# pelinski/TransformerGrooveInfilling

Hardware: AMD Instinct MI355X
Metric: HVO sequences/sec (32-step, d_model=128) per train step (higher is better)
Workload: dtype f32; 1 GPU; BASELINE configs[1]: InfillingClosedHH_training.yaml + overrides d_model=128/4 heads/3 layers, dim_feedforward=512, bs=64 per GPU, dropout=0.24, SGD lr=0.07, hit_loss_penalty=0.38, S=16, encoder-only; global_batch=64, parallelism=dp1, hipgraph=False

## Files before the change

transformergrooveinfilling_amd/csrc/groove_hip.hip:

```cpp
#include <stdarg.h>
#include <stdio.h>
#include <stdlib.h>
#include <string.h>

#include <string>
#include <vector>

#include "gt_attn.h"
#include "gt_common.h"
#include "gt_gemm.h"
#include "gt_misc.h"
#include "gt_seq_api.h"

static thread_local char g_err[512] = "";
static int gt_fail(const char* fmt, ...) {
  va_list ap;
  va_start(ap, fmt);
  vsnprintf(g_err, sizeof(g_err), fmt, ap);
  va_end(ap);
  return -1;
}
extern "C" const char* gt_last_error(void) { return g_err; }

GtProfile g_prof;
#ifndef GT_EMU
struct ProfRec { const char* label; double flops, bytes; hipEvent_t a, b; };
static std::vector<ProfRec> g_recs;
void gt_prof_events(hipEvent_t* start, hipEvent_t* stop) {
  ProfRec r{g_prof.label, g_prof.flops, g_prof.bytes, nullptr, nullptr};
  (void)hipEventCreate(&r.a);
  (void)hipEventCreate(&r.b);
  g_recs.push_back(r);
  *start = r.a; *stop = r.b;
  g_prof.label = "other"; g_prof.flops = 0; g_prof.bytes = 0;
}
#else
void gt_prof_events(hipEvent_t*, hipEvent_t*) {}
#endif
extern "C" int gt_profile_enable(int on) {
  g_prof.on = on != 0;
  g_prof.label = "other";
  return 0;
}
extern "C" int gt_profile_report(char* buf, size_t buf_len, int max_rows) {
  int n = 0;
#ifndef GT_EMU
  struct Acc { std::string label; long count; double ms, flops, bytes; };
  std::vector<Acc> acc;
  for (auto& r : g_recs) {
    (void)hipEventSynchronize(r.b);
    float ms = 0.f;
    (void)hipEventElapsedTime(&ms, r.a, r.b);
    (void)hipEventDestroy(r.a);
    (void)hipEventDestroy(r.b);
    size_t i = 0;
    for (; i < acc.size(); ++i) if (acc[i].label == r.label) break;
    if (i == acc.size()) acc.push_back(Acc{r.label, 0, 0, 0, 0});
    acc[i].count++; acc[i].ms += ms; acc[i].flops += r.flops; acc[i].bytes += r.bytes;
  }
  g_recs.clear();
  std::string out;
  for (auto& a : acc) {
    if (n >= max_rows) break;
    char line[256];
    snprintf(line, sizeof(line), "%s %ld %.6f %.6e %.6e\n", a.label.c_str(), a.count, a.ms, a.flops, a.bytes);
    out += line;
    ++n;
  }
  if (buf && buf_len) { strncpy(buf, out.c_str(), buf_len - 1); buf[buf_len - 1] = 0; }
#else
  if (buf && buf_len) buf[0] = 0;
#endif
  return n;
}
extern "C" int gt_version(void) { return 1; }

static int check_cfg(const gt_config* c) {
  if (!c) return gt_fail("gt_config is NULL");
  if (c->batch <= 0) return gt_fail("batch must be > 0 (got %d)", c->batch);
  if (c->d_model <= 0 || c->d_model > GT_MAX_D) return gt_fail("d_model %d outside 1..%d", c->d_model, GT_MAX_D);
  if (c->n_heads <= 0 || c->d_model % c->n_heads != 0)
    return gt_fail("embed_dim %d not divisible by num_heads %d", c->d_model, c->n_heads);
  if (c->d_model % 2 != 0) return gt_fail("d_model %d must be even (sin/cos positional encoding)", c->d_model);
  if (c->dim_ff <= 0 || c->src_dim <= 0) return gt_fail("dim_ff / src_dim must be > 0");
  if (c->n_enc_layers <= 0 || c->n_enc_layers > 64 || c->n_dec_layers < 0 || c->n_dec_layers > 64)
    return gt_fail("layer counts out of range (enc %d, dec %d)", c->n_enc_layers, c->n_dec_layers);
  if (!(c->dropout >= 0.f && c->dropout < 1.f)) return gt_fail("dropout %f outside [0,1)", (double)c->dropout);
  if (c->flags & ~(GT_CFG_NO_QUAD | GT_CFG_NO_LN_XCHG)) return gt_fail("gt_config.flags %d has unknown bits", c->flags);
  if (c->precision < 0 || c->precision > 2) return gt_fail("precision %d unknown (0 = fp32, 1 = bf16 GEMM operands, 2 = ... and bf16 storage of the Linear outputs)", c->precision);
  if ((int64_t)c->batch * 32 * (c->dim_ff > 3 * c->d_model ? c->dim_ff : 3 * c->d_model) >= (1ll << 31))
    return gt_fail("batch %d too large for 32-bit element indices", c->batch);
  const int n_ln = 2 * c->n_enc_layers + 3 * c->n_dec_layers + (c->n_dec_layers > 0 ? 2 : 1);
  if (n_ln > GT_LN_JOBS_MAX)
    return gt_fail("%d LayerNorm instances (enc %d, dec %d layers) exceed the %d the backward's partials table holds",
                   n_ln, c->n_enc_layers, c->n_dec_layers, GT_LN_JOBS_MAX);
  return 0;
}

struct AttnP { int64_t in_w, in_b, out_w, out_b; };
struct LayerP { AttnP sa, xa; int64_t w1, b1, w2, b2, n1w, n1b, n2w, n2b, n3w, n3b; };
struct PEntry { int64_t off, size; int rows, cols; };
struct PLayout {
  int64_t in_w, in_b, encn_w, encn_b, din_w, din_b, decn_w, decn_b, out_w, out_b, total;
  std::vector<LayerP> enc, dec;
  std::vector<PEntry> entries;
};
static PLayout param_layout(const gt_config& c) {
  PLayout L;
  int64_t cur = 0;
  auto add = [&](int rows, int cols) {
    const int64_t size = (int64_t)rows * (cols ? cols : 1);
    const int64_t off = cur;
    L.entries.push_back(PEntry{off, size, rows, cols});
    cur += (size + 63) / 64 * 64;
    return off;
  };
  const int d = c.d_model, F = c.dim_ff;
  auto attn = [&](AttnP& a) { a.in_w = add(3 * d, d); a.in_b = add(3 * d, 0); a.out_w = add(d, d); a.out_b = add(d, 0); };
  L.in_w = add(d, c.src_dim); L.in_b = add(d, 0);
  L.enc.resize(c.n_enc_layers);
  for (auto& l : L.enc) {
    attn(l.sa);
    l.w1 = add(F, d); l.b1 = add(F, 0); l.w2 = add(d, F); l.b2 = add(d, 0);
    l.n1w = add(d, 0); l.n1b = add(d, 0); l.n2w = add(d, 0); l.n2b = add(d, 0);
  }
  L.encn_w = add(d, 0); L.encn_b = add(d, 0);
  L.dec.resize(c.n_dec_layers);
  if (c.n_dec_layers > 0) {
    L.din_w = add(d, GT_TGT); L.din_b = add(d, 0);
    for (auto& l : L.dec) {
      attn(l.sa); attn(l.xa);
      l.w1 = add(F, d); l.b1 = add(F, 0); l.w2 = add(d, F); l.b2 = add(d, 0);
      l.n1w = add(d, 0); l.n1b = add(d, 0); l.n2w = add(d, 0); l.n2b = add(d, 0); l.n3w = add(d, 0); l.n3b = add(d, 0);
    }
    L.decn_w = add(d, 0); L.decn_b = add(d, 0);
  }
  L.out_w = add(GT_TGT, d); L.out_b = add(GT_TGT, 0);
  L.total = cur;
  return L;
}

extern "C" int gt_param_count(const gt_config* cfg, int64_t* n_tensors, int64_t* n_floats) {
  if (check_cfg(cfg)) return -1;
  PLayout L = param_layout(*cfg);
  if (n_tensors) *n_tensors = (int64_t)L.entries.size();
  if (n_floats) *n_floats = L.total;
  return 0;
}
extern "C" int gt_param_layout(const gt_config* cfg, int64_t* offsets, int64_t* sizes, int32_t* rows, int32_t* cols) {
  if (check_cfg(cfg)) return -1;
  PLayout L = param_layout(*cfg);
  for (size_t i = 0; i < L.entries.size(); ++i) {
    if (offsets) offsets[i] = L.entries[i].off;
    if (sizes) sizes[i] = L.entries[i].size;
    if (rows) rows[i] = L.entries[i].rows;
    if (cols) cols[i] = L.entries[i].cols;
  }
  return 0;
}

struct LayerW {
  int64_t qkv, P, ctx, xhat1, rstd1, x1;
  int64_t qx, kvx, Px, ctxx, xhatx, rstdx, x2;
  int64_t hact, xhat2, rstd2, xout;
};
struct WLayout {
  int64_t x0, a0, enc_xhat, enc_rstd, memory, y0, b0, dec_xhat, dec_rstd, dec_final;
  std::vector<LayerW> layers;
  int64_t hvo_tmp, dlogits, loss_part, dctx, dmem, da0_dec, ln_part, ln_part_stride, total, stamps = 0;
  int64_t pack_f = -1, pack_b = -1, pack_stride = 0;
  int64_t seq_dctx = -1;
  int64_t seq_xchg = -1, seq_xchg_n = 0;
  int64_t rowx = -1, rowx_n = 0;
  int64_t seq_amask = -1, seq_amask_stride = 0;
  std::vector<std::pair<int64_t, int64_t>> sh;
  std::vector<int64_t> sh_only;
  int64_t w16 = -1, w16t = -1, w16_stride = 0;
  int64_t kbits = -1, kbits_stride = 0;
  int64_t wT = -1, wT_stride = 0;
  struct TmpSet { int64_t dzA, dzAm, dzB, dzBm, dzC, dzCm, dhid, dqkv, dqkvx; };
  std::vector<TmpSet> set;
};
#ifndef GT_WGRAD_DEFER_MAX_M
#define GT_WGRAD_DEFER_MAX_M (1ll << 40)
#endif
static bool wgrad_deferred(const gt_config& c) { return (int64_t)c.batch * 32 <= GT_WGRAD_DEFER_MAX_M; }
static bool seq_supported(const gt_config& c);
#ifndef GT_T128_BIG_MIN
#define GT_T128_BIG_MIN 192
#endif
static int g_bf16_shadows = -1;
static int g_layout_epoch = 0;
extern "C" int gt_layout_epoch() { return g_layout_epoch; }
extern "C" int gt_set_operand_shadows(int level) {
  const int nv = level < 0 ? -1 : level > 2 ? 2 : level;
  if (nv != g_bf16_shadows) ++g_layout_epoch;
  g_bf16_shadows = nv;
  return 0;
}
static int bf16_shadow_level() {
  if (g_bf16_shadows < 0) { const char* e = getenv("GT_BF16_SHADOWS"); g_bf16_shadows = (e && e[0] >= '0' && e[0] <= '2') ? e[0] - '0' : 2; }
  return g_bf16_shadows;
}
static bool bf16_shadows(const gt_config& c);
static bool bf16_wt(const gt_config& c) {
  static const int on = [] { const char* e = getenv("GT_BF16_WT"); return (e && e[0] == '0') ? 0 : 1; }();
  return on && c.precision >= 1 && c.n_enc_layers > 0 && c.d_model % 32 == 0 && c.dim_ff % 32 == 0 && !bf16_shadows(c);
}
static bool bf16_shadows(const gt_config& c) {
  const int on = bf16_shadow_level() > 0;
  const int64_t M = (int64_t)c.batch * 32;
  const int hd = c.n_heads > 0 ? c.d_model / c.n_heads : 0;
  static const int attn_mfma = [] { const char* e = getenv("GT_ATTN_MFMA"); return (e && e[0] == '0') ? 0 : 1; }();
  const int nmin = c.d_model < c.dim_ff ? c.d_model : c.dim_ff;
  return on && attn_mfma && wgrad_deferred(c) && c.precision >= 1 && c.n_enc_layers > 0 && (c.d_model == 256 || c.d_model == 512) && c.dim_ff % 128 == 0 &&
         M % 128 == 0 && (hd == 16 || hd == 32 || hd == 64 || hd == 128) && (M / 128) * (nmin / 128) >= GT_T128H_MIN;
}
static bool p2(const gt_config& c) {
  const int hd = c.n_heads > 0 ? c.d_model / c.n_heads : 0;
  return c.precision == 2 && bf16_shadows(c) && bf16_shadow_level() >= 2 && (hd == 64 || hd == 128);
}
extern "C" int gt_precision_in_force(const gt_config* cfg) {
  if (check_cfg(cfg)) return -1;
  return p2(*cfg) ? 2 : (cfg->precision ? 1 : 0);
}
#ifndef GT_WS_SKEW
#define GT_WS_SKEW 0
#endif
static WLayout ws_layout(const gt_config& c) {
  WLayout W;
  int64_t cur = 0;
  static const int64_t skew = [] { const char* e = getenv("GT_WS_SKEW"); return e ? (int64_t)atoll(e) / 64 * 64 : (int64_t)GT_WS_SKEW; }();
  auto add = [&](int64_t n) { int64_t o = cur; cur += (n + 63) / 64 * 64 + skew; return o; };
  const int64_t M = (int64_t)c.batch * 32, d = c.d_model, F = c.dim_ff, BH = (int64_t)c.batch * c.n_heads;
  W.x0 = add(M * d); W.a0 = add(M * d);
  const int nl = c.n_enc_layers + c.n_dec_layers;
  W.layers.resize(nl);
  for (int l = 0; l < nl; ++l) {
    LayerW& w = W.layers[l];
    w.qkv = add(M * 3 * d); w.P = add(BH * 1024); w.ctx = add(M * d);
    w.xhat1 = add(M * d); w.rstd1 = add(M); w.x1 = add(M * d);
    if (l >= c.n_enc_layers) {
      w.qx = add(M * d); w.kvx = add(M * 2 * d); w.Px = add(BH * 1024); w.ctxx = add(M * d);
      w.xhatx = add(M * d); w.rstdx = add(M); w.x2 = add(M * d);
    } else {
      w.qx = w.kvx = w.Px = w.ctxx = w.xhatx = w.rstdx = w.x2 = -1;
    }
    w.hact = add(M * F); w.xhat2 = add(M * d); w.rstd2 = add(M); w.xout = add(M * d);
  }
  W.enc_xhat = add(M * d); W.enc_rstd = add(M); W.memory = add(M * d);
  if (c.n_dec_layers > 0) {
    W.y0 = add(M * d); W.b0 = add(M * d); W.dec_xhat = add(M * d); W.dec_rstd = add(M); W.dec_final = add(M * d);
    W.dmem = add(M * d); W.hvo_tmp = add(M * GT_TGT);
  } else {
    W.y0 = W.b0 = W.dec_xhat = W.dec_rstd = W.dec_final = W.dmem = W.hvo_tmp = -1;
  }
  W.dlogits = add(M * GT_TGT);
  W.loss_part = add(std::max<int64_t>(((M * GT_VOICES + 255) / 256) * 4, 8 * (int64_t)c.batch));
  W.ln_part_stride = ((M + 7) / 8) * 2 * d;
  W.ln_part = add(W.ln_part_stride * (2 * c.n_enc_layers + 3 * c.n_dec_layers + 2));
  W.dctx = add(M * d);
  W.da0_dec = c.n_dec_layers > 0 ? add(M * d) : -1;
  W.set.resize(wgrad_deferred(c) ? nl : 2);
  for (size_t k = 0; k < W.set.size(); ++k) {
    WLayout::TmpSet& t = W.set[k];
    t.dzA = add(M * d); t.dzAm = add(M * d); t.dzB = add(M * d); t.dzBm = add(M * d);
    t.dhid = add(M * F); t.dqkv = add(M * 3 * d);
    if (c.n_dec_layers > 0) { t.dzC = add(M * d); t.dzCm = add(M * d); t.dqkvx = add(M * 3 * d); }
    else { t.dzC = t.dzCm = t.dqkvx = -1; }
  }
  if (seq_supported(c)) {
    W.pack_stride = (int64_t)4 * d * d + (int64_t)2 * d * F;
    W.pack_f = add(W.pack_stride * c.n_enc_layers); W.pack_b = add(W.pack_stride * c.n_enc_layers);
    W.seq_dctx = add(2 * M * d);
    if (d == 128) { W.seq_xchg_n = 2 * gt_seq_xchg_floats(c.batch); W.seq_xchg = add(W.seq_xchg_n); }
    if ((d == 32 || d == 64) && c.n_heads == 16) { W.seq_amask_stride = BH * 32; W.seq_amask = add(W.seq_amask_stride * c.n_enc_layers); }
  }
  if (!seq_supported(c) && (d == 256 || d == 512) && M % 64 == 0) { W.rowx_n = gt_rowx_floats(M, (int)d); W.rowx = add(W.rowx_n); }
  if (bf16_shadows(c)) {
    auto sh = [&](int64_t off, int64_t n) { W.sh.emplace_back(off, add((n + 1) / 2)); };
    const bool only = bf16_shadow_level() >= 2;
    sh(W.x0, M * d);
    for (int l = 0; l < c.n_enc_layers; ++l) {
      const LayerW& w = W.layers[l];
      sh(w.ctx, M * d); sh(w.x1, M * d); sh(w.hact, M * F);
      if (only) { W.sh_only.push_back(w.ctx); W.sh_only.push_back(w.hact); }
      if (l + 1 < c.n_enc_layers) sh(w.xout, M * d);
    }
    for (size_t k = 0; k < W.set.size() && (int)k < c.n_enc_layers; ++k) {
      const WLayout::TmpSet& t = W.set[k];
      const int64_t a = add((M * d + 1) / 2), b = add((M * d + 1) / 2);
      W.sh.emplace_back(t.dzA, a); W.sh.emplace_back(t.dzAm, a); W.sh.emplace_back(t.dzB, b); W.sh.emplace_back(t.dzBm, b);
      sh(t.dhid, M * F); sh(t.dqkv, M * 3 * d);
      if (only) { W.sh_only.push_back(t.dhid); W.sh_only.push_back(t.dqkv); W.sh_only.push_back(t.dzAm); W.sh_only.push_back(t.dzBm); }
    }
    W.w16_stride = ((int64_t)4 * d * d + (int64_t)2 * d * F + 1) / 2;
    W.w16 = add(W.w16_stride * c.n_enc_layers); W.w16t = add(W.w16_stride * c.n_enc_layers);
  } else if (bf16_wt(c)) {
    W.wT_stride = (int64_t)4 * d * d + (int64_t)2 * d * F;
    W.wT = add(W.wT_stride * c.n_enc_layers);
  }
  if (!seq_supported(c) && F % 32 == 0) { W.kbits_stride = (M * F / 32 + 63) / 64 * 64; W.kbits = add(W.kbits_stride * nl); }
#ifdef GT_SEQ_STAMPS
  W.stamps = add(2048 + 2 * 4 * 512);
#endif
  W.total = cur;
  return W;
}
extern "C" size_t gt_workspace_bytes(const gt_config* cfg) {
  if (check_cfg(cfg)) return 0;
  return (size_t)ws_layout(*cfg).total * sizeof(float);
}
static int launch_status(const char* what);
extern "C" int gt_workspace_init(const gt_config* cfg, float* ws, gt_stream_t stream) {
  if (check_cfg(cfg)) return -1;
  if (!ws) return gt_fail("gt_workspace_init: ws must not be NULL");
  const WLayout W = ws_layout(*cfg);
  if (W.seq_xchg >= 0) (void)hipMemsetAsync(ws + W.seq_xchg, 0, (size_t)W.seq_xchg_n * sizeof(float), (hipStream_t)stream);
  if (W.rowx >= 0) (void)hipMemsetAsync(ws + W.rowx, 0, (size_t)W.rowx_n * sizeof(float), (hipStream_t)stream);
  return launch_status("gt_workspace_init");
}
extern "C" int gt_operand_shadow_level(const gt_config* cfg) {
  if (check_cfg(cfg)) return -1;
  return bf16_shadows(*cfg) ? bf16_shadow_level() : 0;
}
extern "C" int gt_ws_find(const gt_config* cfg, const char* name, int layer, int64_t* offset, int64_t* count) {
  if (check_cfg(cfg)) return -1;
  const gt_config& c = *cfg;
  WLayout W = ws_layout(c);
  const int64_t M = (int64_t)c.batch * 32, d = c.d_model, F = c.dim_ff, BH = (int64_t)c.batch * c.n_heads;
  std::string n(name);
  int64_t off = -1, cnt = 0;
  auto set = [&](int64_t o, int64_t k) { off = o; cnt = k; };
  if (n == "w16" || n == "w16t") {
    if (W.w16 < 0 || layer < 0 || layer >= c.n_enc_layers) return gt_fail("gt_ws_find: no weight shadows for this configuration / layer");
    *offset = (n == "w16" ? W.w16 : W.w16t) + W.w16_stride * layer; *count = W.w16_stride;
    return 0;
  }
  if ((n == "qkv16" || n == "dctx16") && p2(c)) {
    if (n == "qkv16") { if (layer < 0 || layer >= c.n_enc_layers) return gt_fail("gt_ws_find: qkv16: layer %d is not an encoder layer", layer); *offset = W.layers[layer].qkv; *count = (M * 3 * d + 1) / 2; }
    else { *offset = W.dctx; *count = (M * d + 1) / 2; }
    return 0;
  }
  const bool want16 = n.size() > 2 && n.compare(n.size() - 2, 2, "16") == 0;
  if (want16) n.resize(n.size() - 2);
  if (n == "x0") set(W.x0, M * d); else if (n == "a0") set(W.a0, M * d);
  else if (n == "enc_xhat") set(W.enc_xhat, M * d); else if (n == "enc_rstd") set(W.enc_rstd, M);
  else if (n == "memory") set(W.memory, M * d); else if (n == "y0") set(W.y0, M * d); else if (n == "b0") set(W.b0, M * d);
  else if (n == "dec_final") set(W.dec_final, M * d); else if (n == "dlogits") set(W.dlogits, M * GT_TGT);
  else if (n == "dmem") set(W.dmem, M * d); else if (n == "dctx") set(W.dctx, M * d);
  else if (n == "seq_xchg") set(W.seq_xchg, W.seq_xchg_n);
  else if (n == "rowx") set(W.rowx, W.rowx_n);
  else if (n == "xchg_err") { if (W.seq_xchg >= 0) set(W.seq_xchg, 2); else if (W.rowx >= 0) set(W.rowx, 2); }
  else if (n == "amask" && W.seq_amask >= 0) set(W.seq_amask, W.seq_amask_stride * c.n_enc_layers);
  else if (n == "pack_f" && W.pack_f >= 0) set(W.pack_f, W.pack_stride * c.n_enc_layers);
  else if (n == "pack_b" && W.pack_b >= 0) set(W.pack_b, W.pack_stride * c.n_enc_layers);
#ifdef GT_SEQ_STAMPS
  else if (n == "stamps") set(W.stamps, 2048 + 2 * 4 * 512);
#endif
  else if (n == "dzA" || n == "dzAm" || n == "dzB" || n == "dzBm" || n == "dzC" || n == "dzCm" || n == "dhid" || n == "dqkv" || n == "dqkvx") {
    if (layer < 0 || layer >= (int)W.layers.size()) return gt_fail("gt_ws_find: layer %d out of range", layer);
    const WLayout::TmpSet& t = W.set[(size_t)layer % W.set.size()];
    if (n == "dzA") set(t.dzA, M * d); else if (n == "dzAm") set(t.dzAm, M * d); else if (n == "dzB") set(t.dzB, M * d);
    else if (n == "dzBm") set(t.dzBm, M * d); else if (n == "dzC") set(t.dzC, M * d); else if (n == "dzCm") set(t.dzCm, M * d);
    else if (n == "dhid") set(t.dhid, M * F); else if (n == "dqkv") set(t.dqkv, M * 3 * d); else set(t.dqkvx, M * 3 * d);
  } else {
    if (layer < 0 || layer >= (int)W.layers.size()) return gt_fail("gt_ws_find: layer %d out of range", layer);
    const LayerW& w = W.layers[layer];
    if (n == "qkv") set(w.qkv, M * 3 * d); else if (n == "P") set(w.P, BH * 1024); else if (n == "ctx") set(w.ctx, M * d);
    else if (n == "xhat1") set(w.xhat1, M * d); else if (n == "rstd1") set(w.rstd1, M); else if (n == "x1") set(w.x1, M * d);
    else if (n == "qx") set(w.qx, M * d); else if (n == "kvx") set(w.kvx, M * 2 * d); else if (n == "Px") set(w.Px, BH * 1024);
    else if (n == "ctxx") set(w.ctxx, M * d); else if (n == "xhatx") set(w.xhatx, M * d); else if (n == "x2") set(w.x2, M * d);
    else if (n == "rstdx") set(w.rstdx, M);
    else if (n == "hact") set(w.hact, M * F); else if (n == "xhat2") set(w.xhat2, M * d); else if (n == "rstd2") set(w.rstd2, M);
    else if (n == "xout") set(w.xout, M * d);
  }
  if (off < 0) return gt_fail("gt_ws_find: unknown or absent buffer '%s'", name);
  if (want16) {
    for (const auto& e : W.sh) if (e.first == off) { *offset = e.second; *count = (cnt + 1) / 2; return 0; }
    return gt_fail("gt_ws_find: '%s' has no bf16 shadow in this configuration", name);
  }
  *offset = off; *count = cnt;
  return 0;
}

static thread_local int g_bf16 = 0;

struct Ctx {
  gt_config c;
  PLayout P;
  WLayout W;
  int M, d, F, H, hd;
  const float* prm;
  float* grd;
  float* ws;
  const gt_step_state* st;
  bool drop;
  hipStream_t s;
  WgradBatch* wb;
  hipStream_t side;
  hipEvent_t pending[2];
  LnJobs* ln;
};
static float* ln_job(const Ctx& x, int64_t gamma_off, int nwg) {
  if (!x.ln || x.ln->n >= GT_LN_JOBS_MAX) return nullptr;
  float* part = x.ws + x.W.ln_part + x.W.ln_part_stride * x.ln->n;
  LnJob& j = x.ln->j[x.ln->n++];
  j.part = part; j.dgamma = x.grd + gamma_off; j.dbeta = x.grd + gamma_off + (x.d + 63) / 64 * 64; j.nwg = nwg;
  return part;
}
static uint16_t* sh_act(const Ctx& x, const float* p) {
  if (x.W.sh.empty() || p == nullptr) return nullptr;
  const int64_t off = p - x.ws;
  for (const auto& e : x.W.sh) if (e.first == off) return reinterpret_cast<uint16_t*>(x.ws + e.second);
  return nullptr;
}
static const float* wT_of(const Ctx& x, const float* W) {
  if (x.W.wT < 0) return nullptr;
  const int64_t off = W - x.prm, d = x.d, F = x.F;
  for (int l = 0; l < x.c.n_enc_layers; ++l) {
    const LayerP& p = x.P.enc[l];
    const float* base = x.ws + x.W.wT + x.W.wT_stride * l;
    if (off == p.sa.in_w) return base;
    if (off == p.sa.out_w) return base + 3 * d * d;
    if (off == p.w1) return base + 4 * d * d;
    if (off == p.w2) return base + 4 * d * d + d * F;
  }
  return nullptr;
}
static bool only16(const Ctx& x, const float* p) {
  if (x.W.sh_only.empty() || p == nullptr) return false;
  const int64_t off = p - x.ws;
  for (const int64_t o : x.W.sh_only) if (o == off) return true;
  return false;
}
static thread_local const char* g_store_error = nullptr;
static void need16(bool ok, const char* what) { if (!ok && g_store_error == nullptr) g_store_error = what; }
static const uint16_t* sh_w(const Ctx& x, const float* W, bool transposed) {
  if (x.W.w16 < 0) return nullptr;
  const int64_t off = W - x.prm, d = x.d, F = x.F;
  for (int l = 0; l < x.c.n_enc_layers; ++l) {
    const LayerP& p = x.P.enc[l];
    const uint16_t* base = reinterpret_cast<const uint16_t*>(x.ws + (transposed ? x.W.w16t : x.W.w16) + x.W.w16_stride * l);
    if (off == p.sa.in_w) return base;
    if (off == p.sa.out_w) return base + 3 * d * d;
    if (off == p.w1) return base + 4 * d * d;
    if (off == p.w2) return base + 4 * d * d + d * F;
  }
  return nullptr;
}
struct Tmp { float *dzA, *dzAm, *dzB, *dzBm, *dzC, *dzCm, *dhid, *dqkv, *dqkvx; };
static Tmp tmp_set(const Ctx& x, int gl) {
  const WLayout::TmpSet& t = x.W.set[(size_t)gl % x.W.set.size()];
  float* ws = x.ws;
  Tmp r;
  r.dzA = ws + t.dzA; r.dzAm = x.drop ? ws + t.dzAm : r.dzA;
  r.dzB = ws + t.dzB; r.dzBm = x.drop ? ws + t.dzBm : r.dzB;
  r.dzC = t.dzC >= 0 ? ws + t.dzC : nullptr; r.dzCm = t.dzC >= 0 ? (x.drop ? ws + t.dzCm : r.dzC) : nullptr;
  r.dhid = ws + t.dhid; r.dqkv = ws + t.dqkv; r.dqkvx = t.dqkvx >= 0 ? ws + t.dqkvx : nullptr;
  return r;
}
static DropArgs mk_drop(const Ctx& x, int site) {
  DropArgs da;
  da.st = x.drop ? x.st : nullptr;
  da.site = (uint32_t)site;
  da.thr = x.drop ? (uint32_t)(x.c.dropout * 16777216.0f) : 0u;
  da.scale = x.drop ? 1.0f / (1.0f - x.c.dropout) : 1.0f;
  return da;
}
static DropArgs no_drop() { DropArgs da; da.st = nullptr; da.site = 0u; da.thr = 0u; da.scale = 1.0f; return da; }
static int lsite(int gl, int kind) { return GT_SITE_LAYER0 + 8 * gl + kind; }
static GemmArgs mk_gemm(const float* A, int lda, const float* B, int ldb, float* C, int ldc, int M, int N, int K) {
// ... 426 lines not shown
}

static void input_layer_fwd(const Ctx& x, const float* in, int S, int64_t w, int64_t b, const float* pe, float* a0, float* out,
                            int site) {
  GemmArgs g = mk_gemm(in, S, x.prm + w, S, out, x.d, x.M, x.d, S);
  g.bias = x.prm + b; g.aux = a0; g.pe = pe; g.drop = mk_drop(x, site);
  g.C16 = sh_act(x, out); g.ldc16 = x.d;
  gemm_launch<false, false, EPI_RELU_PE>(g, x.s);
}
static GemmArgs ffn1_args(const Ctx& x, const LayerP& p, const LayerW& w, const float* xin, int gl, bool* ok) {
  float* ws = x.ws;
  GemmArgs g = mk_gemm(xin, x.d, x.prm + p.w1, x.d, ws + w.hact, x.F, x.M, x.F, x.d);
  g.bias = x.prm + p.b1; g.drop = mk_drop(x, lsite(gl, GT_SITE_FFN));
  g.A16 = sh_act(x, xin); g.B16 = sh_w(x, x.prm + p.w1, false); g.lda16 = g.ldb16 = x.d;
  if (g.A16 && g.B16) { g.C16 = sh_act(x, ws + w.hact); g.ldc16 = x.F; }
  *ok = true;
  if (only16(x, ws + w.hact)) { *ok = g.C16 && gemm32h_ok(g, EPI_RELU_DROP); if (g.C16) g.C = nullptr; }
  return g;
}
static GemmArgs ffn2d_args(const Ctx& x, const LayerP& p, const LayerW& w, const Tmp& t, const float* dzm, bool* nt, bool* ok) {
  float* ws = x.ws;
  const float* w2t = wT_of(x, x.prm + p.w2);
  GemmArgs g = w2t ? mk_gemm(dzm, x.d, w2t, x.d, t.dhid, x.F, x.M, x.F, x.d) : mk_gemm(dzm, x.d, x.prm + p.w2, x.F, t.dhid, x.F, x.M, x.F, x.d);
  g.res = ws + w.hact; g.ldres = x.F;
  g.mask_scale = x.drop ? 1.0f / (1.0f - x.c.dropout) : 1.0f;
  *nt = w2t != nullptr; *ok = true;
  if (w2t) return g;
  g.A16 = sh_act(x, dzm); g.B16 = sh_w(x, x.prm + p.w2, true); g.lda16 = g.ldb16 = x.d;
  if (g.A16 && g.B16) { g.C16 = sh_act(x, t.dhid); g.ldc16 = x.F; }
  if (only16(x, ws + w.hact)) g.res16 = sh_act(x, ws + w.hact);
  if (only16(x, t.dhid) || only16(x, dzm) || g.res16) {
    *ok = g.C16 && gemm32h_ok(g, EPI_MASK_NZ);
    if (g.C16 && only16(x, t.dhid)) g.C = nullptr;
  }
  return g;
}
static uint16_t* ffn_kbits(const Ctx& x, const LayerP& p, const LayerW& w, const float* xin, int gl) {
  static const bool on = [] { const char* e = getenv("GT_FFN_KBITS"); return !(e && e[0] == '0'); }();
  if (!on || x.W.kbits < 0 || x.M % 32 != 0) return nullptr;
  bool ok1, ok2, nt;
  const GemmArgs a = ffn1_args(x, p, w, xin, gl, &ok1);
  const Tmp t = tmp_set(x, gl);
  const GemmArgs b = ffn2d_args(x, p, w, t, t.dzAm, &nt, &ok2);
  if (!ok1 || !ok2 || !gemm_on_big_kernel<false, EPI_RELU_DROP>(a)) return nullptr;
  if (!(nt ? gemm_on_big_kernel<false, EPI_MASK_NZ>(b) : gemm_on_big_kernel<true, EPI_MASK_NZ>(b))) return nullptr;
  return reinterpret_cast<uint16_t*>(x.ws + x.W.kbits + x.W.kbits_stride * gl);
}
static int ffn_fwd(const Ctx& x, const LayerP& p, const LayerW& w, const float* xin, int64_t norm_w, int gl,
                   const SecondNorm* second = nullptr) {
  float* ws = x.ws;
  bool ok;
  GemmArgs g = ffn1_args(x, p, w, xin, gl, &ok);
  need16(ok, "FFN activation stored in bf16 alone");
  g.kbits = ffn_kbits(x, p, w, xin, gl);
  if (g.kbits) gemm64_trace("kbits write", g, false, EPI_RELU_DROP);
  gemm_launch<false, false, EPI_RELU_DROP>(g, x.s);
  return linear_res_ln(x, ws + w.hact, x.F, p.w2, p.b2, xin, norm_w, ws + w.xout, ws + w.xhat2, ws + w.rstd2,
                       lsite(gl, GT_SITE_DROPF), second);
}
static int self_attn_fwd(const Ctx& x, const LayerP& p, const LayerW& w, const float* xin, int causal, int gl) {
  float* ws = x.ws;
  const int d = x.d;
  const bool s16 = p2(x.c) && gl < x.c.n_enc_layers;
  linear_fwd(x, xin, d, x.prm + p.sa.in_w, x.prm + p.sa.in_b, ws + w.qkv, 3 * d, 3 * d, d, s16 ? reinterpret_cast<uint16_t*>(ws + w.qkv) : nullptr);
  attention_fwd(x, ws + w.qkv, 3 * d, ws + w.qkv + d, ws + w.qkv + 2 * d, 3 * d, ws + w.P, ws + w.ctx, causal,
                lsite(gl, GT_SITE_ATTN), s16);
  return linear_res_ln(x, ws + w.ctx, d, p.sa.out_w, p.sa.out_b, xin, p.n1w, ws + w.x1, ws + w.xhat1, ws + w.rstd1,
                       lsite(gl, GT_SITE_DROP1));
}

static bool use_seq(const gt_config& c);
static int g_seq = -1;
extern "C" int gt_set_seq(int on) { g_seq = on != 0; return 0; }
static int g_seq_split = -1;
extern "C" int gt_set_seq_split(int on) { g_seq_split = on < 0 ? -1 : on != 0; return 0; }
static int seq_cu_count() {
#ifdef GT_EMU
  return 256;
#else
  static int cached[64] = {0};
  int dev = 0;
  if (hipGetDevice(&dev) != hipSuccess || dev < 0 || dev >= 64) return 256;
  if (cached[dev] == 0) {
    hipDeviceProp_t prop;
    cached[dev] = (hipGetDeviceProperties(&prop, dev) == hipSuccess && prop.multiProcessorCount > 0) ? prop.multiProcessorCount : 256;
  }
  return cached[dev];
#endif
}
static int xchg_cus() {
  static const bool masked = [] {
    const char* a = getenv("HSA_CU_MASK"); const char* b = getenv("ROC_GLOBAL_CU_MASK");
    const bool m = (a && a[0]) || (b && b[0]);
    if (m) fprintf(stderr, "[groove_hip] a CU mask is set (HSA_CU_MASK / ROC_GLOBAL_CU_MASK): the in-launch exchange schedules stay off\n");
    return m;
  }();
  return masked ? 0 : seq_cu_count();
}
static bool seq_split(const gt_config& c) {
  if (c.d_model != 128 && c.d_model != 32 && c.d_model != 64) return false;
  if (g_seq_split < 0) { const char* e = getenv("GT_SEQ_SPLIT"); if (e) g_seq_split = e[0] != '0'; }
  if (g_seq_split >= 0) return g_seq_split != 0;
  if (c.d_model <= 64 && c.dim_ff < 256 && c.n_heads != 16) return false;
  return 2 * c.batch <= seq_cu_count();
}
static int g_seq_ride = -1;
extern "C" int gt_set_seq_ride(int on) { g_seq_ride = on < 0 ? -1 : on != 0; return 0; }
#ifndef GT_SEQ_RIDE_MIN_IDLE
#define GT_SEQ_RIDE_MIN_IDLE 96
#endif
#ifndef GT_SEQ_RIDE_LAST_PCT
#define GT_SEQ_RIDE_LAST_PCT 50
#endif
static bool seq_ride(const gt_config& c) {
  if (c.d_model != 128 || c.dim_ff % 16 != 0 || !seq_split(c)) return false;
  if (g_seq_ride < 0) { const char* e = getenv("GT_SEQ_RIDE"); if (e) g_seq_ride = e[0] != '0'; }
  const int idle = seq_cu_count() - 2 * c.batch;
  if (g_seq_ride >= 0) return g_seq_ride != 0 && idle >= 1;
  return idle >= GT_SEQ_RIDE_MIN_IDLE;
}
static int g_seq_quad = -1;
extern "C" int gt_set_seq_quad(int on) { g_seq_quad = on < 0 ? -1 : on != 0; return 0; }
static bool seq_quad(const gt_config& c) {
  if (c.d_model != 128 || c.dim_ff % 32 != 0 || !seq_split(c) || 4 * c.batch > xchg_cus() || (c.flags & GT_CFG_NO_QUAD)) return false;
  if (g_seq_quad < 0) { const char* e = getenv("GT_SEQ_QUAD"); if (e) g_seq_quad = e[0] != '0'; }
  return g_seq_quad != 0;
}
extern "C" int gt_set_xchg_spin_max(int polls) { g_xchg_spin_max = polls; return 0; }
static bool seq_supported(const gt_config& c) {
  const int hd = c.d_model / c.n_heads;
  return c.n_dec_layers == 0 && c.precision == 0 && c.d_model % 16 == 0 && c.d_model <= 128 && c.dim_ff % 16 == 0 &&
         c.dim_ff <= GT_SEQ_FMAX && c.src_dim <= 32 && (hd < 16 || hd == 16 || hd == 32 || hd == 64);
}
static bool use_seq(const gt_config& c) {
  if (g_seq < 0) { const char* e = getenv("GT_SEQ"); g_seq = !e ? 2 : e[0] == '0' ? 0 : 1; }
  if (g_seq == 2 && c.d_model > 64 && c.d_model != 128 && c.batch < 64) return false;
  return g_seq && seq_supported(c);
}
struct SeqLoss { const float* y; float penalty; float* stats; unsigned* ticket; };
static thread_local SeqLoss g_seq_loss = {nullptr, 0.f, nullptr, nullptr};
static thread_local bool g_heads_loss_done = false;
static double seq_b0_flops(const Ctx& x) { return 2.0 * x.M * (27.0 * x.d + 2.0 * x.d * x.F + (double)x.d * x.d); }
static thread_local bool g_seq_b0_fused = false;
static thread_local bool g_seq_packs_current = false;
static bool seq_fuse_b0(const gt_config& c) {
  static const int fuse_env = [] { const char* e = getenv("GT_SEQ_FUSE_B0"); return (e && e[0] == '0') ? 0 : 1; }();
  static const int quad_bwd0 = [] { const char* e = getenv("GT_SEQ_QUAD_BWD0"); return (e && e[0] == '0') ? 0 : 1; }();
  return fuse_env && quad_bwd0 && seq_split(c) && seq_quad(c) && seq_ride(c) && c.d_model / c.n_heads == 32;
}
extern "C" int gt_step_launches(const gt_config* cfg) {
  if (check_cfg(cfg)) return -1;
  if (!use_seq(*cfg)) return 0;
  if (!seq_split(*cfg)) return 7;
  return 2 * cfg->n_enc_layers + 1 + (seq_ride(*cfg) ? 3 : 5) - (seq_fuse_b0(*cfg) ? 1 : 0);
}
static SeqArgs mk_seq(const Ctx& x, const float* pe, const float* src, float* hvo) {
  SeqArgs a;
  memset(&a, 0, sizeof(a));
  a.prm = x.prm; a.ws = x.ws; a.pe = pe; a.xin = src; a.hvo = hvo;
  a.B = x.c.batch; a.S = x.c.src_dim; a.d = x.d; a.F = x.F; a.H = x.H; a.L = x.c.n_enc_layers; a.hd = x.hd;
  a.st = x.drop ? x.st : nullptr; a.thr = x.drop ? (uint32_t)(x.c.dropout * 16777216.0f) : 0u;
  a.dscale = x.drop ? 1.0f / (1.0f - x.c.dropout) : 1.0f;
  const LayerP& p = x.P.enc[0];
  a.p0 = SeqLayerP{p.sa.in_w, p.sa.in_b, p.sa.out_w, p.sa.out_b, p.w1, p.b1, p.w2, p.b2, p.n1w, p.n1b, p.n2w, p.n2b};
  a.pstride = x.c.n_enc_layers > 1 ? x.P.enc[1].sa.in_w - p.sa.in_w : x.P.encn_w - p.sa.in_w;
  const LayerW& w = x.W.layers[0];
  a.w0 = SeqLayerW{w.qkv, w.P, w.ctx, w.xhat1, w.rstd1, w.x1, w.hact, w.xhat2, w.rstd2, w.xout};
  a.wstride = x.c.n_enc_layers > 1 ? x.W.layers[1].qkv - w.qkv : 0;
  const WLayout::TmpSet& t = x.W.set[0];
  a.t0 = SeqTmp{t.dzA, t.dzAm, t.dzB, t.dzBm, t.dhid, t.dqkv};
  a.tstride = x.W.set.size() > 1 ? x.W.set[1].dzA - t.dzA : 0;
  a.in_w = x.P.in_w; a.in_b = x.P.in_b; a.encn_w = x.P.encn_w; a.encn_b = x.P.encn_b; a.out_w = x.P.out_w; a.out_b = x.P.out_b;
  a.x0 = x.W.x0; a.a0 = x.W.a0; a.memory = x.W.memory; a.enc_xhat = x.W.enc_xhat; a.enc_rstd = x.W.enc_rstd;
  a.dlogits = x.W.dlogits; a.da0 = x.W.dctx; a.ln_part = x.W.ln_part; a.ln_part_stride = x.W.ln_part_stride;
  a.stamps = x.W.stamps;
  a.pack_f = x.W.pack_f; a.pack_b = x.W.pack_b; a.kstride = x.W.pack_stride;
  a.dctx = x.W.seq_dctx; a.xchg = x.W.seq_xchg; a.xchg_b = x.W.seq_xchg >= 0 ? x.W.seq_xchg + gt_seq_xchg_floats(x.c.batch) : -1; a.fuse_b0 = 0; a.spin_max = g_xchg_spin_max > 0 ? g_xchg_spin_max : GT_XCHG_SPIN_MAX; a.amask = x.W.seq_amask; a.amask_stride = x.W.seq_amask_stride; a.phase = 0;
  a.loss_y = nullptr; a.loss_penalty = 0.f; a.loss_stats = nullptr; a.loss_part = nullptr; a.loss_ticket = nullptr;
  a.grd = nullptr; a.nseq = 0; a.wg_accumulate = 0; a.ride_last_k = x.M; a.out_early = 0; a.tail_phase = 0; a.tail_ksplit = 1; a.ln_nwg = 0; a.bump = nullptr;
  return a;
}
static int seq_forward(const Ctx& x, const float* pe, const float* src, float* hvo_out) {
  SeqArgs a = mk_seq(x, pe, src, hvo_out);
  if (g_seq_loss.y != nullptr) {
    a.loss_y = g_seq_loss.y; a.loss_penalty = g_seq_loss.penalty; a.loss_stats = g_seq_loss.stats; a.loss_ticket = g_seq_loss.ticket;
    a.loss_part = x.ws + x.W.loss_part;
  }
  const double fl = 2.0 * x.M * ((double)x.c.src_dim * x.d + x.c.n_enc_layers * (4.0 * x.d * x.d + 64.0 * x.d + 2.0 * x.d * x.F) + 27.0 * x.d);
  if (!g_seq_packs_current) {
    const int64_t frags = 2 * (int64_t)x.c.n_enc_layers * x.W.pack_stride / 256;
    gt_prof_tag("seq_pack", 0.0, 12.0 * x.c.n_enc_layers * x.W.pack_stride);
    gt_seq_launch_pack(a, (unsigned)((frags + 3) / 4), x.s);
  }
  const int hc = x.hd < 16 ? 0 : x.hd;
  const bool fuse_b0 = seq_fuse_b0(x.c) && a.loss_y != nullptr;
  gt_prof_tag("seq_fwd", fl + (fuse_b0 ? seq_b0_flops(x) : 0.0), 4.0 * x.M * (x.c.src_dim + x.c.n_enc_layers * (9.0 * x.d + x.F) + 27.0));
  if (seq_split(x.c)) {
    const bool quad = seq_quad(x.c);
    static const int quad_pro = [] { const char* e = getenv("GT_SEQ_QUAD_PRO"); return (e && e[0] == '1') ? 1 : 0; }();
    a.quad_pro = quad ? quad_pro : 0;
    g_seq_b0_fused = false;
    for (int p = a.quad_pro ? -1 : 0; p < x.c.n_enc_layers; ++p) {
      SeqArgs ap = a;
      ap.phase = p;
      if (p > (a.quad_pro ? -1 : 0)) gt_prof_tag("seq_fwd", 0.0, 0.0);
      if (fuse_b0 && p == x.c.n_enc_layers - 1) {
        ap.fuse_b0 = 1;
        gt_seq_launch_fb(ap, 4 * x.c.batch, x.s);
        g_seq_b0_fused = true;
      } else {
        gt_seq_launch_fwd(ap, x.d, hc, true, (quad ? 4 : 2) * x.c.batch, x.s, quad);
      }
    }
    return 0;
  }
  const dim3 grid(x.c.batch);
  gt_seq_launch_fwd(a, x.d, hc, false, x.c.batch, x.s);
  return 0;
}

static int encoder_fwd(const Ctx& x, const float* pe, const float* src) {
  float* ws = x.ws;
  if (x.W.wT >= 0) {
    const LayerP& p0 = x.P.enc[0];
    WShadowArgs a;
    a.prm = x.prm; a.w16 = nullptr; a.w16t = nullptr;
    a.in_w = p0.sa.in_w; a.out_w = p0.sa.out_w; a.w1 = p0.w1; a.w2 = p0.w2;
    a.pstride = x.c.n_enc_layers > 1 ? x.P.enc[1].sa.in_w - p0.sa.in_w : 0; a.sstride = x.W.wT_stride;
    a.d = x.d; a.F = x.F; a.L = x.c.n_enc_layers;
    const int tiles = (4 * x.d * x.d + 2 * x.d * x.F) / 1024;
    gt_prof_tag("weight_shadow", 0.0, 8.0 * x.c.n_enc_layers * tiles * 1024.0);
    gt_launch(weight_transpose_kernel, dim3((unsigned)(tiles * x.c.n_enc_layers)), dim3(256), x.s, a, ws + x.W.wT);
  }
  if (x.W.w16 >= 0) {
    const LayerP& p0 = x.P.enc[0];
    WShadowArgs a;
    a.prm = x.prm; a.w16 = reinterpret_cast<uint16_t*>(ws + x.W.w16); a.w16t = reinterpret_cast<uint16_t*>(ws + x.W.w16t);
    a.in_w = p0.sa.in_w; a.out_w = p0.sa.out_w; a.w1 = p0.w1; a.w2 = p0.w2;
    a.pstride = x.c.n_enc_layers > 1 ? x.P.enc[1].sa.in_w - p0.sa.in_w : 0; a.sstride = 2 * x.W.w16_stride;
    a.d = x.d; a.F = x.F; a.L = x.c.n_enc_layers;
    const int tiles = (4 * x.d * x.d + 2 * x.d * x.F) / 1024;
    gt_prof_tag("weight_shadow", 0.0, 8.0 * x.c.n_enc_layers * tiles * 1024.0);
    gt_launch(weight_shadow_kernel, dim3((unsigned)(tiles * x.c.n_enc_layers)), dim3(256), x.s, a);
  }
  input_layer_fwd(x, src, x.c.src_dim, x.P.in_w, x.P.in_b, pe, ws + x.W.a0, ws + x.W.x0, GT_SITE_PE_ENC);
  const float* cur = ws + x.W.x0;
  for (int l = 0; l < x.c.n_enc_layers; ++l) {
    const LayerP& p = x.P.enc[l];
    const LayerW& w = x.W.layers[l];
    if (self_attn_fwd(x, p, w, cur, 0, l)) return gt_fail("d_model %d unsupported by the row-LayerNorm kernels", x.d);
    const SecondNorm fin = {x.P.encn_w, ws + x.W.memory, ws + x.W.enc_xhat, ws + x.W.enc_rstd};
    if (ffn_fwd(x, p, w, ws + w.x1, p.n2w, l, l == x.c.n_enc_layers - 1 ? &fin : nullptr)) return -1;
    cur = ws + w.xout;
  }
  return 0;
}
static int decoder_fwd(const Ctx& x, const float* pe, const float* tgt_in) {
  float* ws = x.ws;
  const int d = x.d, L = x.c.n_enc_layers;
  input_layer_fwd(x, tgt_in, GT_TGT, x.P.din_w, x.P.din_b, pe, ws + x.W.b0, ws + x.W.y0, GT_SITE_PE_DEC);
  const float* cur = ws + x.W.y0;
  for (int l = 0; l < x.c.n_dec_layers; ++l) {
    const LayerP& p = x.P.dec[l];
    const LayerW& w = x.W.layers[L + l];
    const int gl = L + l;
    if (self_attn_fwd(x, p, w, cur, 1, gl)) return -1;
    linear_fwd(x, ws + w.x1, d, x.prm + p.xa.in_w, x.prm + p.xa.in_b, ws + w.qx, d, d, d);
    linear_fwd(x, ws + x.W.memory, d, x.prm + p.xa.in_w + (int64_t)d * d, x.prm + p.xa.in_b + d, ws + w.kvx, 2 * d, 2 * d, d);
    attention_fwd(x, ws + w.qx, d, ws + w.kvx, ws + w.kvx + d, 2 * d, ws + w.Px, ws + w.ctxx, 0, lsite(gl, GT_SITE_XATTN));
    if (linear_res_ln(x, ws + w.ctxx, d, p.xa.out_w, p.xa.out_b, ws + w.x1, p.n2w, ws + w.x2, ws + w.xhatx, ws + w.rstdx,
                      lsite(gl, GT_SITE_DROP2))) return -1;
    const SecondNorm fin = {x.P.decn_w, ws + x.W.dec_final, ws + x.W.dec_xhat, ws + x.W.dec_rstd};
    if (ffn_fwd(x, p, w, ws + w.x2, p.n3w, gl, l == x.c.n_dec_layers - 1 ? &fin : nullptr)) return -1;
    cur = ws + w.xout;
  }
  return 0;
}
static void step_linear(const Ctx& x, int B, const float* in, int ldin, const float* W, const float* b, float* out, int ldout, int N, int K) {
  GemmArgs g = mk_gemm(in, 32 * ldin, W, K, out, 32 * ldout, B, N, K);
  g.bias = b;
  gemm_launch<false, false, EPI_STORE>(g, x.s);
}
static void step_linear_res_ln(const Ctx& x, int B, const float* in, int ldin, int K, int64_t w_off, int64_t b_off, const float* res,
                               int64_t gamma_off, float* out, float* xhat, float* rstd) {
  step_linear(x, B, in, ldin, x.prm + w_off, x.prm + b_off, out, x.d, x.d, K);
  gt_launch(ln_fwd_kernel, dim3((B + 3) / 4), dim3(256), x.s, (const float*)out, res, no_drop(), x.prm + gamma_off,
            x.prm + gamma_off + (x.d + 63) / 64 * 64, out, xhat, rstd, B, x.d, 32 * x.d, 32 * x.d, 32 * x.d, (uint16_t*)nullptr, (const uint16_t*)nullptr);
}
static void step_attention(const Ctx& x, int B, const float* q, int ldq, const float* k, const float* v, int ldkv, float* ctx, int nkeys) {
  AttnArgs a;
  memset(&a, 0, sizeof(a));
  a.q = q; a.k = k; a.v = v; a.ldq = ldq; a.ldk = ldkv; a.ldv = ldkv; a.ctx = ctx; a.ldc = x.d;
  a.H = x.H; a.hd = x.hd; a.scale = 1.0f / sqrtf((float)x.hd); a.drop = no_drop();
  gt_launch(attn_decode_kernel, dim3(B * x.H), dim3(64), x.s, a, nkeys);
}
static void decoder_step(const Ctx& x, const float* pe, const float* tgt, int t, float* hvo_tmp) {
  float* ws = x.ws;
  const int d = x.d, F = x.F, L = x.c.n_enc_layers, B = x.c.batch;
  const size_t r = (size_t)t;
  {
    GemmArgs g = mk_gemm(tgt + r * GT_TGT, 32 * GT_TGT, x.prm + x.P.din_w, GT_TGT, ws + x.W.y0 + r * d, 32 * d, B, d, GT_TGT);
    g.bias = x.prm + x.P.din_b; g.aux = ws + x.W.b0; g.pe = pe + r * d; g.pe_fixed = 1; g.drop = no_drop();
    gemm_launch<false, false, EPI_RELU_PE>(g, x.s);
  }
  const float* cur = ws + x.W.y0;
  for (int l = 0; l < x.c.n_dec_layers; ++l) {
    const LayerP& p = x.P.dec[l];
    const LayerW& w = x.W.layers[L + l];
    step_linear(x, B, cur + r * d, d, x.prm + p.sa.in_w, x.prm + p.sa.in_b, ws + w.qkv + r * 3 * d, 3 * d, 3 * d, d);
    step_attention(x, B, ws + w.qkv + r * 3 * d, 3 * d, ws + w.qkv + d, ws + w.qkv + 2 * d, 3 * d, ws + w.ctx + r * d, t + 1);
    step_linear_res_ln(x, B, ws + w.ctx + r * d, d, d, p.sa.out_w, p.sa.out_b, cur + r * d, p.n1w, ws + w.x1 + r * d, ws + w.xhat1, ws + w.rstd1);
    step_linear(x, B, ws + w.x1 + r * d, d, x.prm + p.xa.in_w, x.prm + p.xa.in_b, ws + w.qx + r * d, d, d, d);
    step_attention(x, B, ws + w.qx + r * d, d, ws + w.kvx, ws + w.kvx + d, 2 * d, ws + w.ctxx + r * d, 32);
    step_linear_res_ln(x, B, ws + w.ctxx + r * d, d, d, p.xa.out_w, p.xa.out_b, ws + w.x1 + r * d, p.n2w, ws + w.x2 + r * d, ws + w.xhatx, ws + w.rstdx);
    {
      GemmArgs g = mk_gemm(ws + w.x2 + r * d, 32 * d, x.prm + p.w1, d, ws + w.hact + r * F, 32 * F, B, F, d);
      g.bias = x.prm + p.b1; g.drop = no_drop();
      gemm_launch<false, false, EPI_RELU_DROP>(g, x.s);
    }
    step_linear_res_ln(x, B, ws + w.hact + r * F, F, F, p.w2, p.b2, ws + w.x2 + r * d, p.n3w, ws + w.xout + r * d, ws + w.xhat2, ws + w.rstd2);
    cur = ws + w.xout;
  }
  gt_launch(ln_fwd_kernel, dim3((B + 3) / 4), dim3(256), x.s, cur + r * d, (const float*)nullptr, no_drop(), x.prm + x.P.decn_w,
            x.prm + x.P.decn_b, ws + x.W.dec_final + r * d, ws + x.W.dec_xhat, ws + x.W.dec_rstd, B, d, 32 * d, 32 * d, 32 * d, (uint16_t*)nullptr, (const uint16_t*)nullptr);
  GemmArgs g = mk_gemm(ws + x.W.dec_final + r * d, 32 * d, x.prm + x.P.out_w, d, hvo_tmp + r * GT_TGT, 32 * GT_TGT, B, GT_TGT, d);
  g.bias = x.prm + x.P.out_b;
  gemm_launch<false, false, EPI_HEADS>(g, x.s);
}
static void output_layer_fwd(const Ctx& x, float* hvo_out) {
  const float* fin = x.ws + (x.c.n_dec_layers > 0 ? x.W.dec_final : x.W.memory);
  static const bool skinny = [] { const char* e = getenv("GT_HEADS_KERNEL"); return !(e && e[0] == '0'); }();
  if (skinny && heads_fwd_ok(x.M, x.d, x.d, fin, x.prm + x.P.out_w)) {
    HeadsLoss hl = {nullptr, 0.f, nullptr, nullptr, nullptr, nullptr};
    if (g_seq_loss.y != nullptr) {
      hl = HeadsLoss{g_seq_loss.y, g_seq_loss.penalty, g_seq_loss.stats, x.ws + x.W.loss_part, g_seq_loss.ticket, x.ws + x.W.dlogits};
      g_heads_loss_done = true;
    }
    static const bool trace = [] { const char* e = getenv("GT_TRACE_HEADS"); return e && e[0] == '1'; }();
    if (trace) fprintf(stderr, "[heads] M %d d %d precision %d loss %d\n", x.M, x.d, x.c.precision, hl.y != nullptr);
    gt_prof_tag("gemm_fwd_heads", 2.0 * x.M * GT_TGT * x.d, 4.0 * ((double)x.M * x.d + (double)GT_TGT * x.d + (double)x.M * GT_TGT));
    if (x.c.precision) gt_launch(heads_fwd_kernel<1>, dim3(x.M / 16), dim3(256), x.s, fin, (const float*)(x.prm + x.P.out_w), (const float*)(x.prm + x.P.out_b), hvo_out, x.M, x.d, hl);
    else               gt_launch(heads_fwd_kernel<0>, dim3(x.M / 16), dim3(256), x.s, fin, (const float*)(x.prm + x.P.out_w), (const float*)(x.prm + x.P.out_b), hvo_out, x.M, x.d, hl);
    return;
  }
  GemmArgs g = mk_gemm(fin, x.d, x.prm + x.P.out_w, x.d, hvo_out, GT_TGT, x.M, GT_TGT, x.d);
  g.bias = x.prm + x.P.out_b;
  gemm_launch<false, false, EPI_HEADS>(g, x.s);
}

extern "C" int gt_forward(const gt_config* cfg, const float* params, const float* pe, const float* xin, const float* tgt_in,
                          float* hvo_out, float* ws, const gt_step_state* state, int train, gt_stream_t stream) {
  Ctx x;
  if (make_ctx(x, cfg, params, nullptr, ws, state, train, stream)) return -1;
  if (!pe || !xin || !hvo_out) return gt_fail("gt_forward: pe / x / hvo_out must not be NULL");
  if (cfg->n_dec_layers > 0 && !tgt_in) return gt_fail("gt_forward: encoder-decoder model needs tgt_in");
  if (use_seq(*cfg)) {
    seq_forward(x, pe, xin, hvo_out);
    return launch_status("gt_forward");
  }
  if (encoder_fwd(x, pe, xin)) return -1;
  if (cfg->n_dec_layers > 0 && decoder_fwd(x, pe, tgt_in)) return -1;
  output_layer_fwd(x, hvo_out);
  return launch_status("gt_forward");
}

extern "C" int gt_loss(const gt_config* cfg, const float* hvo, const float* y, float hit_loss_penalty, float* stats, float* d_hvo,
                       gt_stream_t stream) {
  if (check_cfg(cfg)) return -1;
  if (!hvo || !y || !stats) return gt_fail("gt_loss: hvo / y / stats must not be NULL");
  const int M = cfg->batch * 32;
  hipStream_t s = (hipStream_t)stream;
  (void)hipMemsetAsync(stats, 0, 8 * sizeof(float), s);
  gt_prof_tag("loss", 0, 12.0 * M * GT_TGT);
  gt_launch(loss_kernel<false, false>, dim3((M * GT_VOICES + 255) / 256), dim3(256), s, hvo, y, hit_loss_penalty, stats, d_hvo, M,
            (float*)nullptr, (unsigned*)nullptr);
  return launch_status("gt_loss");
}

static int ffn_bwd(const Ctx& x, const LayerP& p, const LayerW& w, const Tmp& t, const float* xin, const float* dz, const float* dzm,
                   const float* xhat_prev, const float* rstd_prev, int64_t gamma_prev, float* dzo, float* dzom, int site_prev) {
  float* ws = x.ws;
  wgrad(x, dzm, x.d, ws + w.hact, x.F, x.grd + p.w2, x.grd + p.b2, x.d, x.F);
  bool nt, ok;
  GemmArgs g = ffn2d_args(x, p, w, t, dzm, &nt, &ok);
  need16(ok, "FFN2 dgrad over bf16-only tensors");
  int gl = 0;
  while (gl + 1 < (int)x.W.layers.size() && x.W.layers[gl].hact != w.hact) ++gl;
  if (dzm == tmp_set(x, gl).dzAm) g.kbits = ffn_kbits(x, p, w, xin, gl);
  if (g.kbits) gemm64_trace("kbits read", g, !nt, EPI_MASK_NZ);
  if (nt) gemm_launch<false, false, EPI_MASK_NZ>(g, x.s);
  else    gemm_launch<false, true, EPI_MASK_NZ>(g, x.s);
  wgrad(x, t.dhid, x.F, xin, x.d, x.grd + p.w1, x.grd + p.b1, x.F, x.d);
  return dgrad_lnbwd(x, t.dhid, x.F, x.prm + p.w1, x.F, dz, xhat_prev, rstd_prev, gamma_prev, dzo, dzom, site_prev);
}
static void self_attn_bwd(const Ctx& x, const LayerP& p, const LayerW& w, const Tmp& t, const float* xin, const float* dz1m, int gl) {
  float* ws = x.ws;
  const int d = x.d;
  wgrad(x, dz1m, d, ws + w.ctx, d, x.grd + p.sa.out_w, x.grd + p.sa.out_b, d, d);
  const bool s16 = p2(x.c) && gl < x.c.n_enc_layers;
  dgrad_store(x, dz1m, d, x.prm + p.sa.out_w, d, ws + x.W.dctx, d, d, 0, s16 ? reinterpret_cast<uint16_t*>(ws + x.W.dctx) : nullptr);
  attention_bwd(x, ws + w.qkv, 3 * d, ws + w.qkv + d, ws + w.qkv + 2 * d, 3 * d, ws + w.P, ws + x.W.dctx, t.dqkv, 3 * d,
                t.dqkv + d, t.dqkv + 2 * d, 3 * d, lsite(gl, GT_SITE_ATTN), s16);
  wgrad(x, t.dqkv, 3 * d, xin, d, x.grd + p.sa.in_w, x.grd + p.sa.in_b, 3 * d, d);
}
static void input_layer_bwd(const Ctx& x, const LayerP& first, const Tmp& t, const float* dz1, const float* a0, const float* in, int S,
                            int64_t w, int64_t b, int site, float* da_out) {
  if (const float* wt = wT_of(x, x.prm + first.sa.in_w)) {
    GemmArgs g = mk_gemm(t.dqkv, 3 * x.d, wt, 3 * x.d, da_out, x.d, x.M, x.d, 3 * x.d);
    g.res = dz1; g.ldres = x.d; g.aux_in = a0; g.drop = mk_drop(x, site);
    gemm_launch<false, false, EPI_ADD_RELUMASK_DROP>(g, x.s);
    wgrad(x, da_out, x.d, in, S, x.grd + w, x.grd + b, x.d, S);
    return;
  }
  GemmArgs g = mk_gemm(t.dqkv, 3 * x.d, x.prm + first.sa.in_w, x.d, da_out, x.d, x.M, x.d, 3 * x.d);
  g.res = dz1; g.ldres = x.d; g.aux_in = a0; g.drop = mk_drop(x, site);
  g.A16 = sh_act(x, t.dqkv); g.B16 = sh_w(x, x.prm + first.sa.in_w, true); g.lda16 = g.ldb16 = 3 * x.d;
  if (only16(x, t.dqkv)) need16(g.A16 && g.B16 && gemm32h_ok(g, EPI_ADD_RELUMASK_DROP), "InputLayer dgrad of a bf16-only tensor");
  gemm_launch<false, true, EPI_ADD_RELUMASK_DROP>(g, x.s);
  wgrad(x, da_out, x.d, in, S, x.grd + w, x.grd + b, x.d, S);
}

struct GradSplit { int nb; int split_layer; int64_t off[2], cnt[2]; };
static bool seq_ride(const gt_config& c);
static GradSplit grad_split(const gt_config& c, const PLayout& P) {
  GradSplit g;
  g.nb = 1; g.split_layer = 0; g.off[0] = 0; g.cnt[0] = P.total; g.off[1] = g.cnt[1] = 0;
  int64_t cut = 0;
  if (c.n_dec_layers > 0) { cut = P.din_w; g.split_layer = c.n_enc_layers; }
  else if (c.n_enc_layers >= 2) { g.split_layer = c.n_enc_layers / 2; cut = P.enc[g.split_layer].sa.in_w; }
  if (use_seq(c)) {
    const int L = c.n_enc_layers;
    int pcut = (L + 2) / 2;
    if (pcut > L - 1) pcut = L - 1;
    if (pcut >= 1 && seq_ride(c)) { g.split_layer = L - pcut + 1; cut = g.split_layer < L ? P.enc[g.split_layer].sa.in_w : P.encn_w; }
    else cut = 0;
  }
  if (cut > 0) {
    g.nb = 2; g.off[0] = cut; g.cnt[0] = P.total - cut; g.off[1] = 0; g.cnt[1] = cut;
  }
  return g;
}
extern "C" int gt_grad_buckets(const gt_config* cfg, int64_t* offsets, int64_t* counts) {
  if (check_cfg(cfg)) return -1;
  if (!offsets || !counts) return gt_fail("gt_grad_buckets: offsets / counts must not be NULL");
  const PLayout P = param_layout(*cfg);
  const GradSplit g = grad_split(*cfg, P);
  for (int i = 0; i < 2; ++i) { offsets[i] = g.off[i]; counts[i] = g.cnt[i]; }
  return g.nb;
}

static int backward_impl(const gt_config* cfg, const float* params, float* grads, const float* xin, const float* tgt_in,
                         const float* hvo, const float* d_hvo, float* ws, const gt_step_state* state, int train, int accumulate,
                         gt_stream_t stream, int phase = 0, gt_step_state* bump_state = nullptr, bool grads_zero = false) {
  Ctx x;
  if (make_ctx(x, cfg, params, grads, ws, state, train, stream)) return -1;
  if (!grads || !xin) return gt_fail("gt_backward: grads / x must not be NULL");
  const int L = cfg->n_enc_layers, Ld = cfg->n_dec_layers, d = x.d, M = x.M;
  if (Ld > 0 && !tgt_in) return gt_fail("gt_backward: encoder-decoder model needs tgt_in");
  const WLayout& W = x.W;
  const PLayout& P = x.P;
  if (!accumulate) (void)hipMemsetAsync(grads, 0, (size_t)P.total * sizeof(float), x.s);
  WgradBatch wbatch;
  x.wb = &wbatch;
  x.side = side_stream();
  LnJobs lnjobs;
  lnjobs.n = 0; lnjobs.N = d; lnjobs.bump = nullptr;
  { const int64_t eo = x.W.rowx >= 0 ? x.W.rowx : x.W.seq_xchg; lnjobs.err = eo >= 0 ? reinterpret_cast<unsigned*>(ws + eo) : nullptr; }
  x.ln = &lnjobs;
  const int top = L + Ld - 1;
  const GradSplit split = grad_split(*cfg, P);
  if (split.nb < 2) {
    if (phase == 2) return 0;
    phase = 0;
  }
  auto finish = [&]() -> int {
    if (!wbatch.empty()) wgrad_flush(wbatch, x.s);
    acquire_set(x, 0);
    acquire_set(x, 1);
    if (lnjobs.n > 0) {
      lnjobs.bump = bump_state;
      gt_prof_tag("ln_param_reduce", 0, 4.0 * lnjobs.n * W.ln_part_stride);
      gt_launch(ln_param_reduce_kernel, dim3((2 * d + 63) / 64, lnjobs.n), dim3(1024), x.s, lnjobs);
    }
    return launch_status("gt_backward");
  };

  if (use_seq(*cfg)) {
    x.side = nullptr;
    if (d_hvo != nullptr) {
      gt_prof_tag("heads_bwd", 0, 12.0 * M * GT_TGT);
      gt_launch(heads_bwd_kernel, dim3((M * GT_TGT + 255) / 256), dim3(256), x.s, d_hvo, hvo, ws + W.dlogits, M * GT_TGT);
    }
    const GradSplit split_ = split;
    const bool split = seq_split(*cfg);
    const int nwg = split ? 2 * cfg->batch : cfg->batch;
    bool ok = ln_job(x, P.encn_w, nwg) != nullptr;
    for (int j = L - 1; j >= 0; --j) ok = ok && ln_job(x, P.enc[j].n2w, nwg) && ln_job(x, P.enc[j].n1w, nwg);
    if (!ok) return gt_fail("too many LayerNorm instances for the partials table");
    const bool ride = split && seq_ride(*cfg);
    {
      SeqArgs a = mk_seq(x, nullptr, xin, nullptr);
      double fl = 2.0 * M * (L * (4.0 * d * d + 128.0 * d + 2.0 * d * x.F) + 27.0 * d);
      const int hc = x.hd < 16 ? 0 : x.hd;
      if (ride) {
        a.grd = grads; a.nseq = 2 * cfg->batch; a.wg_accumulate = (accumulate && !grads_zero) ? 1 : 0;
        const int per_layer = gt_seq_wg_tiles(d, x.F) + gt_seq_wg_tiles(x.F, d) + gt_seq_wg_tiles(d, d), win = gt_seq_wg_tiles(3 * d, d);
        const int lnu = (2 * d + 63) / 64;
        const int idle = seq_cu_count() - a.nseq, busiest = per_layer + (L > 1 ? win : 0) + 2 * lnu + (L == 1 ? lnu : 0);
        const int R = idle < busiest ? (idle > 0 ? idle : 1) : busiest;
        static const int last_pct = [] { const char* e = getenv("GT_SEQ_RIDE_LAST_PCT"); const int v = e ? atoi(e) : GT_SEQ_RIDE_LAST_PCT; return v < 0 ? 0 : v > 100 ? 100 : v; }();
        a.ride_last_k = (int)((int64_t)M * last_pct / 100) / 64 * 64;
        if (last_pct == 100) a.ride_last_k = M;
        fl += 2.0 * M * ((L - 1) * 3.0 * d * d + L * ((double)d * d + 2.0 * d * x.F))
              - 2.0 * (M - a.ride_last_k) * (per_layer + (L > 1 ? win : 0)) * 2048.0;
        if (g_seq_b0_fused) fl -= seq_b0_flops(x);
        gt_prof_tag("seq_bwd", fl, 4.0 * M * (L * (14.0 * d + 2.0 * x.F) + 27.0) + 4.0 * M * L * (8.0 * d + 2.0 * x.F));
        const int pcut = L - split_.split_layer + 1;
        const int p_lo = phase == 2 ? pcut + 1 : 0, p_hi = phase == 1 ? pcut : L;
        a.ln_nwg = nwg;
        static const int quad_bwd0 = [] { const char* e = getenv("GT_SEQ_QUAD_BWD0"); return (e && e[0] == '0') ? 0 : 1; }();
        const bool quad0 = quad_bwd0 && seq_quad(*cfg);
        const bool b0_done = g_seq_b0_fused && quad0;
        g_seq_b0_fused = false;
        for (int p = p_lo; p <= p_hi; ++p) {
          if (p == 0 && b0_done) continue;
          SeqArgs ap = a;
          ap.phase = p;
          if (p > p_lo && !(b0_done && p == 1)) gt_prof_tag("seq_bwd", 0.0, 0.0);
          if (p == 0 && quad0) gt_seq_launch_bwd(ap, d, hc, true, 2 * a.nseq, x.s, true);
          else gt_seq_launch_bwd(ap, d, hc, true, a.nseq + (p == 0 ? 0 : R), x.s);
        }
        if (phase == 1) {
          a.phase = 0; a.tail_phase = 0; a.tail_ksplit = 2; a.bump = nullptr;
          gt_prof_tag("seq_tail", 2.0 * M * 27.0 * d, 4.0 * M * (27.0 + d));
          gt_seq_launch_tail(a, (unsigned)(gt_seq_wg_tiles(GT_TGT, d) * 2), x.s);
          return launch_status("gt_backward");
        }
        a.out_early = phase == 2 ? 1 : 0;
        static const int tail_ks = [] { const char* e = getenv("GT_SEQ_TAIL_KS"); const int v = e ? atoi(e) : 2; return v < 1 ? 1 : v > 16 ? 16 : v; }();
        const int tiles = win + gt_seq_wg_tiles(d, cfg->src_dim) + (a.out_early ? 0 : gt_seq_wg_tiles(GT_TGT, d));
        int ks = (gt_deterministic() && tail_ks > 2) ? 2 : tail_ks;
        if (ks > M / 8) ks = M / 8;
        a.phase = L + 1; a.tail_phase = L + 1; a.tail_ksplit = ks; a.bump = bump_state;
        const int nrest = a.ride_last_k < M ? per_layer + (L > 1 ? win : 0) : 0;
        gt_prof_tag("seq_tail", 2.0 * M * (3.0 * d * d + (a.out_early ? 0.0 : 27.0 * d) + (double)d * cfg->src_dim) + 2.0 * (M - a.ride_last_k) * nrest * 2048.0,
                    4.0 * M * (4.0 * d + cfg->src_dim));
        gt_seq_launch_tail(a, (unsigned)(nrest + tiles * ks), x.s);
        return launch_status("gt_backward");
      }
      gt_prof_tag("seq_bwd", fl, 4.0 * M * (L * (14.0 * d + 2.0 * x.F) + 27.0));
      if (split) {
        for (int p = 0; p <= L; ++p) {
          SeqArgs ap = a;
          ap.phase = p;
          if (p > 0) gt_prof_tag("seq_bwd", 0.0, 0.0);
          gt_seq_launch_bwd(ap, d, hc, true, 2 * cfg->batch, x.s);
        }
      } else {
        gt_seq_launch_bwd(a, d, hc, false, cfg->batch, x.s);
      }
    }
    wgrad(x, ws + W.dlogits, GT_TGT, ws + W.memory, d, grads + P.out_w, grads + P.out_b, GT_TGT, d);
    for (int j = L - 1; j >= 0; --j) {
      const LayerP& p = P.enc[j];
      const LayerW& w = W.layers[j];
      const Tmp t = tmp_set(x, j);
      const float* lin = (j == 0) ? ws + W.x0 : ws + W.layers[j - 1].xout;
      wgrad(x, t.dzAm, d, ws + w.hact, x.F, grads + p.w2, grads + p.b2, d, x.F);
      wgrad(x, t.dhid, x.F, ws + w.x1, d, grads + p.w1, grads + p.b1, x.F, d);
      wgrad(x, t.dzBm, d, ws + w.ctx, d, grads + p.sa.out_w, grads + p.sa.out_b, d, d);
      wgrad(x, t.dqkv, 3 * d, lin, d, grads + p.sa.in_w, grads + p.sa.in_b, 3 * d, d);
    }
    wgrad(x, ws + W.dctx, d, xin, cfg->src_dim, grads + P.in_w, grads + P.in_b, d, cfg->src_dim);
    return finish();
  }
  bool top_norm_done = false;
  if (phase != 2) {
  if (d_hvo != nullptr) {
    gt_prof_tag("heads_bwd", 0, 12.0 * M * GT_TGT);
    gt_launch(heads_bwd_kernel, dim3((M * GT_TGT + 255) / 256), dim3(256), x.s, d_hvo, hvo, ws + W.dlogits, M * GT_TGT);
  }
  const float* fin = ws + (Ld > 0 ? W.dec_final : W.memory);
  wgrad(x, ws + W.dlogits, GT_TGT, fin, d, grads + P.out_w, grads + P.out_b, GT_TGT, d);
  {
    const float* xh = ws + (Ld > 0 ? W.dec_xhat : W.enc_xhat);
    const float* rs = ws + (Ld > 0 ? W.dec_rstd : W.enc_rstd);
    const int64_t gfin = Ld > 0 ? P.decn_w : P.encn_w;
    if (!row_fused(x)) {
      const LayerW& w = W.layers[top];
      Tmp t = tmp_set(x, top);
      acquire_set(x, top);
      dgrad_store(x, ws + W.dlogits, GT_TGT, params + P.out_w, d, ws + W.dctx, d, GT_TGT, 0);
      ln_bwd2(x, ws + W.dctx, xh, rs, gfin, ws + W.dctx, ws + w.xhat2, ws + w.rstd2, Ld > 0 ? P.dec[Ld - 1].n3w : P.enc[L - 1].n2w,
              t.dzA, t.dzAm, lsite(top, GT_SITE_DROPF));
      top_norm_done = true;
    } else if (dgrad_lnbwd(x, ws + W.dlogits, GT_TGT, params + P.out_w, GT_TGT, nullptr, xh, rs, gfin, ws + W.dctx, nullptr, 0)) {
      return gt_fail("d_model %d unsupported by the row-LayerNorm kernels", d);
    }
  }
  if (Ld > 0) {
    if (!top_norm_done) {
      const LayerW& w = W.layers[top];
      Tmp t = tmp_set(x, top);
      ln_bwd(x, ws + W.dctx, nullptr, ws + w.xhat2, ws + w.rstd2, P.dec[Ld - 1].n3w, t.dzA, t.dzAm, lsite(top, GT_SITE_DROPF));
    }
    for (int l = Ld - 1; l >= 0; --l) {
      const LayerP& p = P.dec[l];
      const int gl = L + l;
      const LayerW& w = W.layers[gl];
      const Tmp t = tmp_set(x, gl);
      const float* yin = (l == 0) ? ws + W.y0 : ws + W.layers[gl - 1].xout;
      if (ffn_bwd(x, p, w, t, ws + w.x2, t.dzA, t.dzAm, ws + w.xhatx, ws + w.rstdx, p.n2w, t.dzB, t.dzBm, lsite(gl, GT_SITE_DROP2))) return -1;
      wgrad(x, t.dzBm, d, ws + w.ctxx, d, grads + p.xa.out_w, grads + p.xa.out_b, d, d);
      dgrad_store(x, t.dzBm, d, params + p.xa.out_w, d, ws + W.dctx, d, d, 0);
      float* dqx = t.dqkvx; float* dkvx = t.dqkvx + (int64_t)M * d;
      attention_bwd(x, ws + w.qx, d, ws + w.kvx, ws + w.kvx + d, 2 * d, ws + w.Px, ws + W.dctx, dqx, d, dkvx, dkvx + d, 2 * d,
                    lsite(gl, GT_SITE_XATTN));
      wgrad(x, dqx, d, ws + w.x1, d, grads + p.xa.in_w, grads + p.xa.in_b, d, d);
      wgrad(x, dkvx, 2 * d, ws + W.memory, d, grads + p.xa.in_w + (int64_t)d * d, grads + p.xa.in_b + d, 2 * d, d);
      dgrad_store(x, dkvx, 2 * d, params + p.xa.in_w + (int64_t)d * d, d, ws + W.dmem, d, 2 * d, l == Ld - 1 ? 0 : 1);
      if (dgrad_lnbwd(x, dqx, d, params + p.xa.in_w, d, t.dzB, ws + w.xhat1, ws + w.rstd1, p.n1w, t.dzC, t.dzCm, lsite(gl, GT_SITE_DROP1)))
        return -1;
      self_attn_bwd(x, p, w, t, yin, t.dzCm, gl);
      if (l > 0) {
        wgrad_sync(x, gl);
        const LayerW& wp = W.layers[gl - 1];
        const Tmp tn = tmp_set(x, gl - 1);
        acquire_set(x, gl - 1);
        if (dgrad_lnbwd(x, t.dqkv, 3 * d, params + p.sa.in_w, 3 * d, t.dzC, ws + wp.xhat2, ws + wp.rstd2, P.dec[l - 1].n3w, tn.dzA,
                        tn.dzAm, lsite(gl - 1, GT_SITE_DROPF)))
          return -1;
      } else {
        input_layer_bwd(x, p, t, t.dzC, ws + W.b0, tgt_in, GT_TGT, P.din_w, P.din_b, GT_SITE_PE_DEC, ws + W.da0_dec);
        wgrad_sync(x, gl);
      }
    }
  }
  }
  if (Ld > 0) {
    if (phase == 1) return finish();
    const LayerW& w = W.layers[L - 1];
    const Tmp t = tmp_set(x, L - 1);
    acquire_set(x, L - 1);
    ln_bwd2(x, ws + W.dmem, ws + W.enc_xhat, ws + W.enc_rstd, P.encn_w, ws + W.dctx, ws + w.xhat2, ws + w.rstd2, P.enc[L - 1].n2w,
            t.dzA, t.dzAm, lsite(L - 1, GT_SITE_DROPF));
  } else if (phase != 2 && !top_norm_done) {
    const LayerW& w = W.layers[L - 1];
    const Tmp t = tmp_set(x, L - 1);
    acquire_set(x, L - 1);
    ln_bwd(x, ws + W.dctx, nullptr, ws + w.xhat2, ws + w.rstd2, P.enc[L - 1].n2w, t.dzA, t.dzAm, lsite(L - 1, GT_SITE_DROPF));
  }
  for (int l = (phase == 2 && Ld == 0) ? split.split_layer - 1 : L - 1; l >= 0; --l) {
    const LayerP& p = P.enc[l];
    const LayerW& w = W.layers[l];
    const Tmp t = tmp_set(x, l);
    const float* lin = (l == 0) ? ws + W.x0 : ws + W.layers[l - 1].xout;
    if (ffn_bwd(x, p, w, t, ws + w.x1, t.dzA, t.dzAm, ws + w.xhat1, ws + w.rstd1, p.n1w, t.dzB, t.dzBm, lsite(l, GT_SITE_DROP1))) return -1;
    self_attn_bwd(x, p, w, t, lin, t.dzBm, l);
    if (l > 0) {
      wgrad_sync(x, l);
      const LayerW& wp = W.layers[l - 1];
      const Tmp tn = tmp_set(x, l - 1);
      acquire_set(x, l - 1);
      if (dgrad_lnbwd(x, t.dqkv, 3 * d, params + p.sa.in_w, 3 * d, t.dzB, ws + wp.xhat2, ws + wp.rstd2, P.enc[l - 1].n2w, tn.dzA, tn.dzAm,
                      lsite(l - 1, GT_SITE_DROPF)))
        return -1;
      if (phase == 1 && Ld == 0 && l == split.split_layer) return finish();
    } else {
      input_layer_bwd(x, p, t, t.dzB, ws + W.a0, xin, cfg->src_dim, P.in_w, P.in_b, GT_SITE_PE_ENC, ws + W.dctx);
      wgrad_sync(x, l);
    }
  }
  return finish();
}

extern "C" int gt_debug_seq_wg_phase(const gt_config* cfg, const float* params, float* grads, const float* xin, float* ws, int phase,
                                     int ksplit, gt_stream_t stream) {
  Ctx x;
  if (make_ctx(x, cfg, params, grads, ws, nullptr, 0, stream)) return -1;
  if (!seq_supported(*cfg) || cfg->d_model != 128) return gt_fail("gt_debug_seq_wg_phase: d_model 128 sequence-resident shapes only");
  const int L = cfg->n_enc_layers, d = x.d;
  if (phase < 0 || phase > L + 1 || ksplit < 1) return gt_fail("gt_debug_seq_wg_phase: phase / ksplit out of range");
  SeqArgs a = mk_seq(x, nullptr, xin, nullptr);
  a.grd = grads; a.nseq = 0; a.wg_accumulate = 1; a.phase = phase; a.tail_phase = phase; a.tail_ksplit = ksplit; a.ln_nwg = 0; a.bump = nullptr;
  if (phase == 0 || phase > L) return gt_fail("gt_debug_seq_wg_phase: phases 1..L carry riders");
  const int per_layer = gt_seq_wg_tiles(d, x.F) + gt_seq_wg_tiles(x.F, d) + gt_seq_wg_tiles(d, d), win = gt_seq_wg_tiles(3 * d, d);
  const int tiles = per_layer + (phase >= 2 ? win : 0);
  gt_prof_tag("seq_tail", 0.0, 0.0);
  gt_seq_launch_tail(a, (unsigned)(tiles * ksplit), x.s);
  return launch_status("gt_debug_seq_wg_phase");
}

extern "C" int gt_backward(const gt_config* cfg, const float* params, float* grads, const float* xin, const float* tgt_in,
                           const float* hvo, const float* d_hvo, float* ws, const gt_step_state* state, int train, int accumulate,
                           gt_stream_t stream) {
  if (!hvo || !d_hvo) return gt_fail("gt_backward: hvo / d_hvo must not be NULL");
  g_seq_b0_fused = false;
  return backward_impl(cfg, params, grads, xin, tgt_in, hvo, d_hvo, ws, state, train, accumulate, stream);
}

static int optimizer_step_impl(int algo, float* params, float* grads, float* m, float* v, int64_t n, gt_step_state* state,
                               int zero_grads, gt_stream_t stream, int step_advanced, unsigned* err = nullptr, int guard = 0) {
  if (!params || !grads || !state || n <= 0) return gt_fail("gt_optimizer_step: params / grads / state must not be NULL");
  hipStream_t s = (hipStream_t)stream;
  const unsigned blocks = (unsigned)((n + 1023) / 1024);
  if (algo == 0) {
    gt_prof_tag("optimizer", 0, 12.0 * n);
    gt_launch(sgd_kernel, dim3(blocks), dim3(256), s, params, grads, n, (const gt_step_state*)state, zero_grads, (const unsigned*)err, guard);
  } else if (algo == 1) {
    if (!m || !v) return gt_fail("gt_optimizer_step: adam needs m and v");
    gt_prof_tag("optimizer", 0, 28.0 * n);
    gt_launch(adam_kernel, dim3(blocks), dim3(256), s, params, grads, m, v, n, (const gt_step_state*)state, zero_grads, step_advanced, (const unsigned*)err, guard);
  } else {
    return gt_fail("optimizer algo %d unknown (0 = sgd, 1 = adam)", algo);
  }
  if (!step_advanced) gt_launch(step_inc_kernel, dim3(1), dim3(64), s, state, err, guard ? (const float*)(grads + n - 1) : (const float*)nullptr);
  return launch_status("gt_optimizer_step");
}
extern "C" int gt_optimizer_step(int algo, float* params, float* grads, float* m, float* v, int64_t n, gt_step_state* state,
                                 int zero_grads, gt_stream_t stream) {
  return optimizer_step_impl(algo, params, grads, m, v, n, state, zero_grads, stream, 0);
}

extern "C" int gt_optimizer_step_ws(const gt_config* cfg, int algo, float* params, float* grads, float* m, float* v, float* ws,
                                    gt_step_state* state, int zero_grads, gt_stream_t stream) {
  if (check_cfg(cfg)) return -1;
  PLayout P = param_layout(*cfg);
  if (!use_seq(*cfg) || !zero_grads || !ws) {
    const WLayout W0 = ws ? ws_layout(*cfg) : WLayout();
    const int64_t eo = W0.rowx >= 0 ? W0.rowx : W0.seq_xchg;
    unsigned* err = (ws && eo >= 0) ? reinterpret_cast<unsigned*>(ws + eo) : nullptr;
    return optimizer_step_impl(algo, params, grads, m, v, P.total, state, zero_grads, stream, 0, err, 1);
  }
  if (!params || !grads || !state) return gt_fail("gt_optimizer_step: params / grads / state must not be NULL");
  if (algo != 0 && algo != 1) return gt_fail("optimizer algo %d unknown (0 = sgd, 1 = adam)", algo);
  if (algo == 1 && (!m || !v)) return gt_fail("gt_optimizer_step: adam needs m and v");
  Ctx x;
  if (make_ctx(x, cfg, params, grads, ws, state, 1, stream)) return -1;
  const SeqArgs a = mk_seq(x, nullptr, nullptr, nullptr);
  gt_prof_tag("optimizer", 0, (algo ? 28.0 : 12.0) * P.total + 8.0 * cfg->n_enc_layers * x.W.pack_stride);
  gt_seq_launch_update_pack(a, algo, params, grads, m, v, P.total, state, 0, (hipStream_t)stream);
  gt_launch(step_inc_kernel, dim3(1), dim3(64), (hipStream_t)stream, state, x.W.seq_xchg >= 0 ? reinterpret_cast<unsigned*>(ws + x.W.seq_xchg) : (unsigned*)nullptr,
            (const float*)(grads + P.total - 1));
  return launch_status("gt_optimizer_step_ws");
}

extern "C" int gt_train_step(const gt_config* cfg, int algo, float* params, float* grads, float* m, float* v, const float* pe,
                             const float* xin, const float* y, float hit_loss_penalty, float* hvo_out, float* stats,
                             float* tgt_scratch, float* ws, gt_step_state* state, int skip_update, gt_stream_t stream) {
  if (check_cfg(cfg)) return -1;
  if (!y || !state) return gt_fail("gt_train_step: y / state must not be NULL");
  if (skip_update < 0 || skip_update > 7) return gt_fail("gt_train_step: skip_update %d outside 0..7", skip_update);
  const bool packs_current = (skip_update & GT_STEP_PACKS_CURRENT) != 0;
  skip_update &= 3;
  struct Handoffs { ~Handoffs() { g_seq_loss.y = nullptr; g_seq_packs_current = false; g_seq_b0_fused = false; g_heads_loss_done = false; } } handoffs_guard;
  const int M = cfg->batch * 32;
  hipStream_t s = (hipStream_t)stream;
  const float* tgt_in = nullptr;
  if (cfg->n_dec_layers > 0) {
    if (!tgt_scratch) return gt_fail("gt_train_step: encoder-decoder model needs tgt_scratch");
    tgt_in = tgt_scratch;
  }
  if (skip_update == 3)
    return backward_impl(cfg, params, grads, xin, tgt_in, hvo_out, nullptr, ws, state, 1, 1, stream, 2);
  if (tgt_in) gt_launch(shift_right_kernel, dim3((M * GT_TGT + 255) / 256), dim3(256), s, y, tgt_scratch, M * GT_TGT);
  bool fuse_loss = use_seq(*cfg) && stats != nullptr && hvo_out != nullptr;
  g_heads_loss_done = false;
  if (stats != nullptr && hvo_out != nullptr && y != nullptr) g_seq_loss = SeqLoss{y, hit_loss_penalty, stats, reinterpret_cast<unsigned*>(&state->pad2[0])};
  g_seq_packs_current = packs_current && use_seq(*cfg);
  const int frc = gt_forward(cfg, params, pe, xin, tgt_in, hvo_out, ws, state, 1, stream);
  g_seq_loss.y = nullptr;
  g_seq_packs_current = false;
  fuse_loss = fuse_loss || g_heads_loss_done;
  g_heads_loss_done = false;
  if (frc) return -1;
  WLayout W = ws_layout(*cfg);
  if (!stats || !hvo_out) return gt_fail("gt_train_step: hvo_out / stats must not be NULL");
  if (!fuse_loss) {
    gt_prof_tag("loss", 0, 12.0 * M * GT_TGT);
    gt_launch(loss_kernel<true, true>, dim3((M * GT_VOICES + 255) / 256), dim3(256), s, (const float*)hvo_out, y, hit_loss_penalty, stats,
              ws + W.dlogits, M, ws + W.loss_part, reinterpret_cast<unsigned*>(&state->pad2[0]));
  }
  const int brc = backward_impl(cfg, params, grads, xin, tgt_in, hvo_out, nullptr, ws, state, 1, 1, stream, skip_update == 2 ? 1 : 0,
                                skip_update == 0 ? state : nullptr, true);
  g_seq_b0_fused = false;
  if (brc) return -1;
  if (!skip_update) {
    PLayout P = param_layout(*cfg);
    if (use_seq(*cfg)) {
      if (algo != 0 && algo != 1) return gt_fail("optimizer algo %d unknown (0 = sgd, 1 = adam)", algo);
      if (algo == 1 && (!m || !v)) return gt_fail("gt_optimizer_step: adam needs m and v");
      Ctx x;
      if (make_ctx(x, cfg, params, grads, ws, state, 1, stream)) return -1;
      const SeqArgs a = mk_seq(x, pe, xin, hvo_out);
      gt_prof_tag("optimizer", 0, (algo ? 28.0 : 12.0) * P.total + 8.0 * cfg->n_enc_layers * x.W.pack_stride);
      gt_seq_launch_update_pack(a, algo, params, grads, m, v, P.total, state, 1, (hipStream_t)stream);
      return launch_status("gt_train_step");
    }
    const int64_t eo = W.rowx >= 0 ? W.rowx : W.seq_xchg;
    if (optimizer_step_impl(algo, params, grads, m, v, P.total, state, 1, stream, 1,
                            eo >= 0 ? reinterpret_cast<unsigned*>(ws + eo) : nullptr, 1)) return -1;
  }
  return 0;
}

__global__ __launch_bounds__(64) void dp_guard_kernel(float* guard, const unsigned* err) { if (threadIdx.x == 0) *guard = (*err != 0u) ? 1.0f : 0.0f; }
extern "C" int gt_dp_guard(const gt_config* cfg, float* grads, const float* ws, gt_stream_t stream) {
  if (check_cfg(cfg)) return -1;
  if (!grads || !ws) return gt_fail("gt_dp_guard: grads / ws must not be NULL");
  const WLayout W = ws_layout(*cfg);
  const int64_t eo = W.rowx >= 0 ? W.rowx : W.seq_xchg;
  if (eo < 0) return 0;
  const PLayout P = param_layout(*cfg);
  gt_launch(dp_guard_kernel, dim3(1), dim3(64), (hipStream_t)stream, grads + P.total - 1, reinterpret_cast<const unsigned*>(ws + eo));
  return launch_status("gt_dp_guard");
}

__global__ __launch_bounds__(64) void occupy_cus_kernel(int usec, unsigned* sink) {
  __shared__ unsigned hold[24 * 1024];
  hold[threadIdx.x] = threadIdx.x;
  __syncthreads();
#ifndef GT_EMU
  const unsigned long long t0 = __builtin_amdgcn_s_memrealtime();
  while (__builtin_amdgcn_s_memrealtime() - t0 < (unsigned long long)usec * 100ull) __builtin_amdgcn_s_sleep(32);
#endif
  if (hold[(threadIdx.x + 1) & 63] == 0xFFFFFFFFu && sink) *sink = 1u;
}
extern "C" int gt_debug_occupy_cus(int nblocks, int usec, gt_stream_t stream) {
  if (nblocks <= 0 || usec < 0) return gt_fail("gt_debug_occupy_cus: nblocks %d / usec %d", nblocks, usec);
  gt_launch(occupy_cus_kernel, dim3(nblocks), dim3(64), (hipStream_t)stream, usec, (unsigned*)nullptr);
  return launch_status("gt_debug_occupy_cus");
}

extern "C" int64_t gt_voice_metrics_scratch_floats(int64_t n_rows) {
  return n_rows <= 0 ? 0 : ((n_rows + GT_VM_ROWS - 1) / GT_VM_ROWS) * GT_TGT;
}
extern "C" int gt_voice_metrics(const float* hvo_pred, const float* hvo_gt, int64_t n_rows, float* out30, float* scratch,
                                gt_stream_t stream) {
  if (!hvo_pred || !hvo_gt || !out30 || !scratch) return gt_fail("gt_voice_metrics: pointers must not be NULL");
  if (n_rows <= 0 || n_rows >= (1ll << 31)) return gt_fail("gt_voice_metrics: n_rows %lld out of range", (long long)n_rows);
  const int M = (int)n_rows, nwg = (M + GT_VM_ROWS - 1) / GT_VM_ROWS;
  hipStream_t s = (hipStream_t)stream;
  gt_launch(voice_metrics_partial_kernel, dim3(nwg), dim3(256), s, hvo_pred, hvo_gt, scratch, M);
  gt_launch(voice_metrics_final_kernel, dim3(1), dim3(64), s, (const float*)scratch, out30, nwg, M);
  return launch_status("gt_voice_metrics");
}
extern "C" int gt_gather_batch(const float* xs, const float* ys, const int64_t* idx, int64_t n_seq, int32_t batch, int32_t src_dim,
                               float* x, float* y, gt_stream_t stream) {
  if (!xs || !ys || !idx || !x || !y) return gt_fail("gt_gather_batch: pointers must not be NULL");
  if (batch <= 0 || src_dim <= 0 || n_seq <= 0) return gt_fail("gt_gather_batch: batch / src_dim / n_seq must be > 0");
  const int64_t n4 = (int64_t)batch * (32 * src_dim / 4 + 32 * GT_TGT / 4);
  gt_launch(gather_batch_kernel, dim3((unsigned)((n4 + 255) / 256)), dim3(256), (hipStream_t)stream, xs, ys, idx, x, y, (int)batch,
            (int)src_dim, n_seq);
  return launch_status("gt_gather_batch");
}

static int predict_impl(const gt_config* cfg, const float* params, const float* pe, const float* xin, float* hvo_out, float thres,
                        int use_thres, uint32_t seed, float* tgt_scratch, float* ws, gt_stream_t stream, uint32_t idx0 = 0u);
extern "C" int gt_predict(const gt_config* cfg, const float* params, const float* pe, const float* xin, float* hvo_out, float thres,
                          int use_thres, float* tgt_scratch, float* ws, gt_stream_t stream) {
  return predict_impl(cfg, params, pe, xin, hvo_out, thres, use_thres != 0, 0u, tgt_scratch, ws, stream);
}
extern "C" int gt_predict_pd(const gt_config* cfg, const float* params, const float* pe, const float* xin, float* hvo_out, uint32_t seed,
                             float* tgt_scratch, float* ws, gt_stream_t stream) {
  return predict_impl(cfg, params, pe, xin, hvo_out, 0.5f, 2, seed, tgt_scratch, ws, stream);
}
extern "C" int gt_predict_pd_at(const gt_config* cfg, const float* params, const float* pe, const float* xin, float* hvo_out, uint32_t seed,
                                int64_t first_seq, float* tgt_scratch, float* ws, gt_stream_t stream) {
  if (first_seq < 0) return gt_fail("gt_predict_pd_at: first_seq must be >= 0");
  return predict_impl(cfg, params, pe, xin, hvo_out, 0.5f, 2, seed, tgt_scratch, ws, stream, (uint32_t)((uint64_t)first_seq * 32u * GT_TGT));
}
static int predict_impl(const gt_config* cfg, const float* params, const float* pe, const float* xin, float* hvo_out, float thres,
                        int use_thres, uint32_t seed, float* tgt_scratch, float* ws, gt_stream_t stream, uint32_t idx0) {
  Ctx x;
  if (make_ctx(x, cfg, params, nullptr, ws, nullptr, 0, stream)) return -1;
  if (!pe || !xin || !hvo_out) return gt_fail("gt_predict: pe / x / hvo_out must not be NULL");
  const int M = x.M, B = cfg->batch;
  if (encoder_fwd(x, pe, xin)) return -1;
  if (cfg->n_dec_layers == 0) {
    output_layer_fwd(x, hvo_out);
    gt_launch(predict_head_kernel, dim3((M * GT_TGT + 255) / 256), dim3(256), x.s, (const float*)hvo_out, hvo_out, (float*)nullptr,
              thres, use_thres, -1, B, seed, idx0);
    return launch_status("gt_predict");
  }
  if (!tgt_scratch) return gt_fail("gt_predict: encoder-decoder model needs tgt_scratch");
  float* tmp = ws + x.W.hvo_tmp;
  (void)hipMemsetAsync(tgt_scratch, 0, (size_t)M * GT_TGT * sizeof(float), x.s);
  static const int full = [] { const char* e = getenv("GT_PREDICT_FULL"); return (e && e[0] == '1') ? 1 : 0; }();
  if (!full) {
    const int d = x.d, L = cfg->n_enc_layers;
    for (int l = 0; l < cfg->n_dec_layers; ++l) {
      const LayerP& p = x.P.dec[l];
      const LayerW& w = x.W.layers[L + l];
      linear_fwd(x, ws + x.W.memory, d, x.prm + p.xa.in_w + (int64_t)d * d, x.prm + p.xa.in_b + d, ws + w.kvx, 2 * d, 2 * d, d);
    }
  }
  for (int t = 0; t < 32; ++t) {
    if (full) {
      if (decoder_fwd(x, pe, tgt_scratch)) return -1;
      output_layer_fwd(x, tmp);
    } else {
      decoder_step(x, pe, tgt_scratch, t, tmp);
    }
    gt_launch(predict_head_kernel, dim3((B * GT_TGT + 255) / 256), dim3(256), x.s, (const float*)tmp, hvo_out, tgt_scratch, thres,
              use_thres, t, B, seed, idx0);
  }
  return launch_status("gt_predict");
}
```

transformergrooveinfilling_amd/csrc/gt_common.h:

```cpp
#pragma once
#include <stddef.h>
#include <stdint.h>

#ifdef GT_EMU
#include "hip_emu.h"
#else
#include <hip/hip_runtime.h>
#include <hip/hip_ext.h>
typedef float f32x4 __attribute__((ext_vector_type(4)));
typedef float f32x16 __attribute__((ext_vector_type(16)));
#define GT_MFMA32(a, b, c) __builtin_amdgcn_mfma_f32_32x32x2f32((a), (b), (c), 0, 0, 0)
#define GT_MFMA16(a, b, c) __builtin_amdgcn_mfma_f32_16x16x4f32((a), (b), (c), 0, 0, 0)
typedef __bf16 bf16x8 __attribute__((ext_vector_type(8)));
#define GT_MFMA16_BF16(a, b, c) __builtin_amdgcn_mfma_f32_16x16x32_bf16((a), (b), (c), 0, 0, 0)
#define GT_MFMA32_BF16(a, b, c) __builtin_amdgcn_mfma_f32_32x32x16_bf16((a), (b), (c), 0, 0, 0)
#define GT_BF16X8_SET(vec, j, x) (vec)[j] = (__bf16)(x)
__device__ __forceinline__ uint16_t gt_f2bf(float f) { return __builtin_bit_cast(uint16_t, (__bf16)f); }
#endif
#ifdef GT_EMU
static inline uint32_t gt_f2u(float f) { uint32_t u; memcpy(&u, &f, 4); return u; }
static inline float gt_u2f(uint32_t u) { float f; memcpy(&f, &u, 4); return f; }
#else
__device__ __forceinline__ uint32_t gt_f2u(float f) { return __builtin_bit_cast(uint32_t, f); }
__device__ __forceinline__ float gt_u2f(uint32_t u) { return __builtin_bit_cast(float, u); }
#endif
__host__ __device__ static inline float gt_bf2f(uint16_t h) {
  union { uint32_t u; float f; } c;
  c.u = (uint32_t)h << 16;
  return c.f;
}

#include "../../include/groove_hip.h"

#ifdef GT_EMU
#define GT_BARRIER() __syncthreads()
#else
#define GT_BARRIER() asm volatile("s_waitcnt lgkmcnt(0)\n\ts_barrier" ::: "memory")
#endif

#ifdef GT_EMU
#define GT_WAVE_SYNC() emu::wave_rendezvous()
#else
#define GT_WAVE_SYNC() __builtin_amdgcn_wave_barrier()
#endif

#define GT_LN_EPS 1e-5f

__device__ __attribute__((aligned(16))) static float gt_zero_page[4] = {0.f, 0.f, 0.f, 0.f};
__device__ __forceinline__ const float* gt_zero_ptr() { return gt_zero_page; }

struct GtProfile {
  bool on = false;
  const char* label = "";
  double flops = 0, bytes = 0;
};
extern GtProfile g_prof;
void gt_prof_events(hipEvent_t* start, hipEvent_t* stop);
static inline void gt_prof_tag(const char* label, double flops, double bytes) {
  if (g_prof.on) { g_prof.label = label; g_prof.flops = flops; g_prof.bytes = bytes; }
}

template <typename... KArgs, typename... Args>
static inline void gt_launch(void (*kern)(KArgs...), dim3 grid, dim3 block, hipStream_t s, Args... args) {
#ifdef GT_EMU
  (void)s;
  emu::launch(grid, block, 0, [=]() { kern(args...); });
#else
  if (g_prof.on) {
    hipEvent_t a, b;
    gt_prof_events(&a, &b);
    hipExtLaunchKernelGGL<KArgs...>(kern, grid, block, 0u, s, a, b, 0u, static_cast<KArgs>(args)...);
  } else {
    kern<<<grid, block, 0, s>>>(args...);
  }
#endif
}

__host__ __device__ static inline uint32_t gt_fmix32(uint32_t h) {
  h ^= h >> 16; h *= 0x85EBCA6Bu; h ^= h >> 13; h *= 0xC2B2AE35u; h ^= h >> 16;
  return h;
}
struct DropArgs {
  const gt_step_state* st;
  uint32_t site;
  uint32_t thr;
  float scale;
};
__device__ static inline uint32_t gt_drop_key(const DropArgs& d) {
  if (d.thr == 0u || d.st == nullptr) return 0u;
  uint32_t s = d.st->seed_lo ^ gt_fmix32(d.st->step);
  uint32_t k = s ^ (d.site * 0x9E3779B9u);
  k = gt_fmix32(k) ^ d.st->seed_hi;
  return gt_fmix32(k + 0x7F4A7C15u);
}
__device__ static inline float gt_drop_mul(const DropArgs& d, uint32_t key, uint32_t idx) {
  if (d.thr == 0u || d.st == nullptr) return 1.0f;
#if defined(GT_ACCT_NOHASH)
  return (idx ^ key) == 0x12345u ? 0.0f : d.scale;
#endif
  return ((gt_fmix32((idx * 0x9E3779B1u) ^ key) >> 8) >= d.thr) ? d.scale : 0.0f;
}

__device__ static inline float gt_wave_sum(float v) {
  v += __shfl_xor(v, 32); v += __shfl_xor(v, 16); v += __shfl_xor(v, 8);
  v += __shfl_xor(v, 4);  v += __shfl_xor(v, 2);  v += __shfl_xor(v, 1);
  return v;
}
__device__ static inline float gt_sigmoid(float x) { return 1.0f / (1.0f + expf(-x)); }

__device__ __forceinline__ void gt_pub_store(float* p, const float v) {
#ifdef GT_EMU
  *p = v;
#else
  __hip_atomic_store(p, v, __ATOMIC_RELAXED, __HIP_MEMORY_SCOPE_AGENT);
#endif
}
__device__ __forceinline__ float gt_pub_load(const float* p) {
#ifdef GT_EMU
  return *p;
#else
  return __hip_atomic_load(p, __ATOMIC_RELAXED, __HIP_MEMORY_SCOPE_AGENT);
#endif
}
__device__ __forceinline__ unsigned gt_pub_ticket(unsigned* counter) {
#ifdef GT_EMU
  return atomicAdd(counter, 1u);
#else
  asm volatile("s_waitcnt vmcnt(0)" ::: "memory");
  return __hip_atomic_fetch_add(counter, 1u, __ATOMIC_RELAXED, __HIP_MEMORY_SCOPE_AGENT);
#endif
}

#ifdef GT_EMU
#define GT_SGB(mask, n)
#define GT_SCHED_FENCE()
#else
#define GT_SGB(mask, n) __builtin_amdgcn_sched_group_barrier(mask, n, 0);
#define GT_SCHED_FENCE() __builtin_amdgcn_sched_barrier(0);
#endif

template <bool WRT_LOGITS>
__device__ __forceinline__ void gt_loss_elem(const float h, const float v, const float o, const float yh, const float yv, const float yo,
                                             const float penalty, const float invM, float& bce, float& mv, float& mo, float& ok, float& dh,
                                             float& dv, float& dO) {
  const float pen = (yh == 1.0f) ? 1.0f : penalty;
  bce = (fmaxf(h, 0.f) - h * yh + log1pf(expf(-fabsf(h)))) * pen;
  mv = (v - yv) * (v - yv) * pen;
  mo = (o - yo) * (o - yo) * pen;
  ok = (((h > 0.f) ? 1.0f : 0.0f) == yh) ? 1.0f : 0.0f;
  dv = 2.0f * (v - yv) * pen * invM; dO = 2.0f * (o - yo) * pen * invM;
  if (WRT_LOGITS) { dv *= v * (1.0f - v); dO *= (0.5f - 2.0f * o * o); }
  dh = (gt_sigmoid(h) - yh) * pen * invM;
}

__device__ __forceinline__ void gt_bump_counters(gt_step_state* st, unsigned* err, const float* guard) {
  const bool skip = (err != nullptr && err[0] != 0u) || (guard != nullptr && *guard != 0.f);
  st->step += 1u;
  if (!skip) st->opt_step += 1u;
  else if (err != nullptr) err[1] += 1u;
}
```

transformergrooveinfilling_amd/csrc/gt_seq.h:

```cpp
#pragma once
#include "gt_seq_api.h"
#include <type_traits>

#ifdef GT_SEQ_STAMPS
#define GT_STAMP(i) do { if (blockIdx.x == 0 && threadIdx.x == 0) reinterpret_cast<long long*>(a.ws + a.stamps)[(i)] = (long long)__builtin_amdgcn_s_memtime(); } while (0)
__shared__ long long* gt_sub_ptr;
#define GT_SUBSTAMP(i) do { if (threadIdx.x == 0 && gt_sub_ptr) gt_sub_ptr[(i)] = (long long)__builtin_amdgcn_s_memtime(); } while (0)
#define GT_SUBWAIT() asm volatile("s_waitcnt vmcnt(0) lgkmcnt(0)" ::: "memory")
#define GT_SUBSET(on) do { if (threadIdx.x == 0) gt_sub_ptr = ((on) && blockIdx.x == 0) ? reinterpret_cast<long long*>(a.ws + a.stamps) + 200 : nullptr; } while (0)
#define GT_WGSTAMP(k) do { if (threadIdx.x == 0 && a.phase == 1 && blockIdx.x < 512) { long long* q_ = reinterpret_cast<long long*>(a.ws + a.stamps) + 1024 + 4 * blockIdx.x + 2 * (k); \
    q_[0] = (long long)__builtin_amdgcn_s_memtime(); q_[1] = (long long)__builtin_amdgcn_s_memrealtime(); } } while (0)
#else
#define GT_WGSTAMP(k) do { } while (0)
#define GT_STAMP(i) do { } while (0)
#define GT_SUBSTAMP(i) do { } while (0)
#define GT_SUBWAIT() do { } while (0)
#define GT_SUBSET(on) do { } while (0)
#endif

#ifndef GT_SEQ_ACCT
#define GT_SEQ_ACCT 0
#endif
#ifndef GT_SEQ_PFB_LN
#define GT_SEQ_PFB_LN 1
// ... 17 lines not shown
  SeqDropK k;
  k.thr = (a.st != nullptr) ? a.thr : 0u; k.scale = a.dscale; k.s_lo = 0u; k.s_hi = 0u;
  if (k.thr) { k.s_lo = a.st->seed_lo ^ gt_fmix32(a.st->step); k.s_hi = a.st->seed_hi; }
  return k;
}
__device__ __forceinline__ uint32_t seq_key(const SeqDropK& k, const int site) {
  if (!k.thr) return 0u;
  uint32_t x = k.s_lo ^ ((uint32_t)site * 0x9E3779B9u);
  x = gt_fmix32(x) ^ k.s_hi;
  return gt_fmix32(x + 0x7F4A7C15u);
}
__device__ __forceinline__ float seq_dmul(const SeqDropK& k, const uint32_t key, const uint32_t idx) {
  if (!k.thr) return 1.0f;
  return ((gt_fmix32((idx * 0x9E3779B1u) ^ key) >> 8) >= k.thr) ? k.scale : 0.0f;
}
__device__ __forceinline__ bool seq_dkeep(const SeqDropK& k, const uint32_t key, const uint32_t idx) {
  return (gt_fmix32((idx * 0x9E3779B1u) ^ key) >> 8) >= k.thr;
}

__device__ __forceinline__ float seq_row16_sum(float v) {
#ifdef GT_EMU
  v += __shfl_xor(v, 1); v += __shfl_xor(v, 2); v += __shfl_xor(v, 4); v += __shfl_xor(v, 8);
#else
  v += __builtin_bit_cast(float, __builtin_amdgcn_update_dpp(0, __builtin_bit_cast(int, v), 0xB1, 0xF, 0xF, true));
  v += __builtin_bit_cast(float, __builtin_amdgcn_update_dpp(0, __builtin_bit_cast(int, v), 0x4E, 0xF, 0xF, true));
  v += __builtin_bit_cast(float, __builtin_amdgcn_update_dpp(0, __builtin_bit_cast(int, v), 0x141, 0xF, 0xF, true));
  v += __builtin_bit_cast(float, __builtin_amdgcn_update_dpp(0, __builtin_bit_cast(int, v), 0x140, 0xF, 0xF, true));
#endif
  return v;
}

#define GT_XTAG 0x5EC0DE01u
#define GT_XCHG_WG_GRANULES (4 * GT_SEQ_NT)
#ifdef GT_EMU
#define GT_XTAG_NOW (GT_XTAG + emu::launch_serial)
#else
#define GT_XTAG_NOW GT_XTAG
#endif
__device__ __forceinline__ void seq_xchg_put(unsigned long long* slot, const f32x4& v, const int tid) {
#pragma unroll
  for (int j = 0; j < 4; ++j) {
    const unsigned long long w = ((unsigned long long)GT_XTAG_NOW << 32) | (unsigned long long)gt_f2u(v[j]);
#ifdef GT_EMU
    slot[j * GT_SEQ_NT + tid] = w;
#else
    if (!(GT_SEQ_ACCT & 4)) __hip_atomic_store(slot + j * GT_SEQ_NT + tid, w, __ATOMIC_RELAXED, __HIP_MEMORY_SCOPE_AGENT);
#endif
  }
}
__device__ __forceinline__ f32x4 seq_xchg_get(unsigned long long* slot, const int tid, unsigned* err, const int spin_max = GT_XCHG_SPIN_MAX) {
  unsigned long long w[4];
#ifdef GT_EMU
  bool ok = true;
  for (int j = 0; j < 4; ++j) { w[j] = slot[j * GT_SEQ_NT + tid]; ok = ok && (uint32_t)(w[j] >> 32) == GT_XTAG_NOW; }
  if (!ok) emu::block_retry();
#else
  int spins = 0;
  for (;;) {
    bool ok = true;
#pragma unroll
    for (int j = 0; j < 4; ++j) {
      w[j] = __hip_atomic_load(slot + j * GT_SEQ_NT + tid, __ATOMIC_RELAXED, __HIP_MEMORY_SCOPE_AGENT);
      ok = ok && (uint32_t)(w[j] >> 32) == GT_XTAG;
    }
    if (__all(ok) || (GT_SEQ_ACCT & 4)) break;
    if (spins == 0 && __hip_atomic_load(err, __ATOMIC_RELAXED, __HIP_MEMORY_SCOPE_AGENT) != 0u) spins = spin_max;
    if (++spins > spin_max) { if ((tid & 63) == 0) __hip_atomic_store(err, 1u, __ATOMIC_RELAXED, __HIP_MEMORY_SCOPE_AGENT); break; }
    __builtin_amdgcn_s_sleep(1);
  }
  if (!(GT_SEQ_ACCT & 6)) {
#pragma unroll
    for (int j = 0; j < 4; ++j) __hip_atomic_store(slot + j * GT_SEQ_NT + tid, 0ull, __ATOMIC_RELAXED, __HIP_MEMORY_SCOPE_AGENT);
  }
#endif
  return f32x4{gt_u2f((uint32_t)w[0]), gt_u2f((uint32_t)w[1]), gt_u2f((uint32_t)w[2]), gt_u2f((uint32_t)w[3])};
}


template <bool BKM, bool VEC>
__device__ __forceinline__ void seq_ldb(float (&b)[4], const float* __restrict__ W, const int ldw, const int n, const int N, const int k,
                                        const int K, const float* zp) {
  if (!BKM && VEC) {
    const float4 v = *reinterpret_cast<const float4*>((n < N && k < K) ? W + (size_t)n * ldw + k : zp);
    b[0] = v.x; b[1] = v.y; b[2] = v.z; b[3] = v.w;
  } else if (!BKM) {
#pragma unroll
    for (int j = 0; j < 4; ++j) b[j] = *((n < N && k + j < K) ? W + (size_t)n * ldw + k + j : zp);
  } else {
#pragma unroll
    for (int j = 0; j < 4; ++j) b[j] = *((n < N && k + j < K) ? W + (size_t)(k + j) * ldw + n : zp);
  }
}
template <bool HALF>
__device__ __forceinline__ void seq_mma(f32x4& acc0, f32x4& acc1, const float (&b)[4], const float* sA, const int lda, const int l16, const int k) {
  const float4 a0 = *reinterpret_cast<const float4*>(sA + l16 * lda + k);
  acc0 = GT_MFMA16(b[0], a0.x, acc0); acc0 = GT_MFMA16(b[1], a0.y, acc0); acc0 = GT_MFMA16(b[2], a0.z, acc0); acc0 = GT_MFMA16(b[3], a0.w, acc0);
  if (!HALF) {
    const float4 a1 = *reinterpret_cast<const float4*>(sA + (16 + l16) * lda + k);
    acc1 = GT_MFMA16(b[0], a1.x, acc1); acc1 = GT_MFMA16(b[1], a1.y, acc1); acc1 = GT_MFMA16(b[2], a1.z, acc1); acc1 = GT_MFMA16(b[3], a1.w, acc1);
  }
}
template <bool BKM, bool VEC, int NK, bool HALF, typename Epi>
__device__ __forceinline__ void seq_mm_edge(const float* sA, const int lda, const int K, const float* __restrict__ W, const int ldw, const int N,
                                            const float* __restrict__ bias, const int wave, const int lane, const float* zp, Epi epi) {
  const int l16 = lane & 15, lg = lane >> 4;
  const int n0 = wave * 16;
  if (n0 >= N) return;
  float b[NK][4], bi[4];
#pragma unroll
  for (int u = 0; u < NK; ++u) { if (16 * u < K) seq_ldb<BKM, VEC>(b[u], W, ldw, n0 + l16, N, 16 * u + 4 * lg, K, zp); }
#pragma unroll
  for (int r = 0; r < 4; ++r) bi[r] = *((bias != nullptr && n0 + 4 * lg + r < N) ? bias + n0 + 4 * lg + r : zp);
  f32x4 acc0 = f32x4{0.f, 0.f, 0.f, 0.f}, acc1 = f32x4{0.f, 0.f, 0.f, 0.f};
#pragma unroll
  for (int u = 0; u < NK; ++u) { if (16 * u < K) seq_mma<HALF>(acc0, acc1, b[u], sA, lda, l16, 16 * u + 4 * lg); }
  epi(n0, acc0, acc1, bi);
}

template <int NK> struct SeqB { float4 v[NK]; };
template <int NK, bool FULL = false>
__device__ __forceinline__ void seq_b_load(SeqB<NK>& b, const float* __restrict__ Wp, const int nkt, const int t, const int u0, const int nk,
                                           const int lane) {
  const float* p = Wp + (unsigned)(((t * nkt + u0) * 64 + lane) * 4);
#pragma unroll
  for (int u = 0; u < NK; ++u) { if (FULL || u < nk) b.v[u] = *reinterpret_cast<const float4*>(p + 256 * u); }
}
#ifdef GT_SEQ_TU_FWD
__global__ __launch_bounds__(256) void seq_pack_kernel(SeqArgs a) {
  const int lane = threadIdx.x & 63, l16 = lane & 15, lg = lane >> 4;
  const int d = a.d, F = a.F, d16 = d >> 4, f16 = F >> 4;
  const int nf0 = 3 * d16 * d16, nf1 = d16 * d16, nf2 = f16 * d16, T = nf0 + nf1 + 2 * nf2;
  const int g = blockIdx.x * 4 + (threadIdx.x >> 6);
  if (g >= 2 * a.L * T) return;
  const int pack = g / (a.L * T), r = g % (a.L * T), l = r / T;
  int f = r % T, R, C;
  int64_t src, moff;
  if (f < nf0) { src = a.p0.in_w; R = 3 * d; C = d; moff = 0; }
  else if (f < nf0 + nf1) { f -= nf0; src = a.p0.out_w; R = d; C = d; moff = (int64_t)3 * d * d; }
  else if (f < nf0 + nf1 + nf2) { f -= nf0 + nf1; src = a.p0.w1; R = F; C = d; moff = (int64_t)4 * d * d; }
  else { f -= nf0 + nf1 + nf2; src = a.p0.w2; R = d; C = F; moff = (int64_t)4 * d * d + (int64_t)d * F; }
  const float* W = a.prm + src + (int64_t)l * a.pstride;
  float4 v;
  if (pack == 0) {
    const int nkt = C >> 4, t = f / nkt, u = f % nkt;
    v = *reinterpret_cast<const float4*>(W + (size_t)(16 * t + l16) * C + 16 * u + 4 * lg);
  } else {
    const int nkt = R >> 4, t = f / nkt, u = f % nkt;
    const float* p = W + (size_t)(16 * u + 4 * lg) * C + 16 * t + l16;
    v = make_float4(p[0], p[C], p[2 * (size_t)C], p[3 * (size_t)C]);
  }
  *reinterpret_cast<float4*>(a.ws + (pack ? a.pack_b : a.pack_f) + (int64_t)l * a.kstride + moff + (int64_t)f * 256 + lane * 4) = v;
}

struct SeqUpd { float* prm; float* g; float* m; float* v; int64_t n; const gt_step_state* st; int algo, step_advanced, nblk_a; const unsigned* err; };
__device__ __forceinline__ float seq_upd_elem(const SeqUpd& u, const int64_t i, const float w, const float g, const float k, const float b1,
                                              const float b2, const float step_size, const float inv_sqrt_bc2, const float gs, const float eps,
                                              const bool skip) {
  if (skip) return w;
  if (u.algo == 0) return w - k * g;
  const float gi = g * gs;
  const float mi = b1 * u.m[i] + (1.0f - b1) * gi;
  const float vi = b2 * u.v[i] + (1.0f - b2) * gi * gi;
  u.m[i] = mi; u.v[i] = vi;
  return w - step_size * mi / (sqrtf(vi) * inv_sqrt_bc2 + eps);
}
__global__ __launch_bounds__(256) void seq_update_pack_kernel(SeqArgs a, SeqUpd u) {
  __shared__ float tr[4][16][17];
  const int lane = threadIdx.x & 63, wave = threadIdx.x >> 6, l16 = lane & 15, lg = lane >> 4;
  const float k = u.st->lr * u.st->grad_scale;
  float b1 = 0.f, b2 = 0.f, step_size = 0.f, inv_sqrt_bc2 = 0.f, gs = u.st->grad_scale, eps = 0.f;
  if (u.algo == 1) {
    b1 = u.st->beta1; b2 = u.st->beta2; eps = u.st->eps;
    const float t = (float)(u.st->opt_step + (u.step_advanced ? 0u : 1u));
    const float bc1 = 1.0f - powf(b1, t), bc2 = 1.0f - powf(b2, t);
    step_size = u.st->lr / bc1; inv_sqrt_bc2 = 1.0f / sqrtf(bc2);
  }
  const bool skip = (u.err != nullptr && *u.err != 0u) || u.g[u.n - 1] != 0.f;
  const int d = a.d, F = a.F, d16 = d >> 4, f16 = F >> 4;
  const int nf0 = 3 * d16 * d16, nf1 = d16 * d16, nf2 = f16 * d16, T = nf0 + nf1 + 2 * nf2;
  if ((int)blockIdx.x < u.nblk_a) {
    const int gidx = blockIdx.x * 4 + wave;
    if (gidx >= a.L * T) return;
    const int l = gidx / T;
    int f = gidx % T, R, C;
    int64_t src, moff;
    if (f < nf0) { src = a.p0.in_w; R = 3 * d; C = d; moff = 0; }
    else if (f < nf0 + nf1) { f -= nf0; src = a.p0.out_w; R = d; C = d; moff = (int64_t)3 * d * d; }
    else if (f < nf0 + nf1 + nf2) { f -= nf0 + nf1; src = a.p0.w1; R = F; C = d; moff = (int64_t)4 * d * d; }
    else { f -= nf0 + nf1 + nf2; src = a.p0.w2; R = d; C = F; moff = (int64_t)4 * d * d + (int64_t)d * F; }
    const int nkt = C >> 4, br = f / nkt, bc = f % nkt;
    const int64_t e0 = src + (int64_t)l * a.pstride + (int64_t)(16 * br + l16) * C + 16 * bc + 4 * lg;
    const float4 w = *reinterpret_cast<const float4*>(u.prm + e0), g = *reinterpret_cast<const float4*>(u.g + e0);
    float4 nw;
    nw.x = seq_upd_elem(u, e0, w.x, g.x, k, b1, b2, step_size, inv_sqrt_bc2, gs, eps, skip);
    nw.y = seq_upd_elem(u, e0 + 1, w.y, g.y, k, b1, b2, step_size, inv_sqrt_bc2, gs, eps, skip);
    nw.z = seq_upd_elem(u, e0 + 2, w.z, g.z, k, b1, b2, step_size, inv_sqrt_bc2, gs, eps, skip);
    nw.w = seq_upd_elem(u, e0 + 3, w.w, g.w, k, b1, b2, step_size, inv_sqrt_bc2, gs, eps, skip);
    *reinterpret_cast<float4*>(u.prm + e0) = nw;
    *reinterpret_cast<float4*>(u.g + e0) = make_float4(0.f, 0.f, 0.f, 0.f);
    float* pf = a.ws + a.pack_f + (int64_t)l * a.kstride + moff;
    float* pb = a.ws + a.pack_b + (int64_t)l * a.kstride + moff;
    *reinterpret_cast<float4*>(pf + (int64_t)f * 256 + lane * 4) = nw;
    tr[wave][l16][4 * lg] = nw.x; tr[wave][l16][4 * lg + 1] = nw.y; tr[wave][l16][4 * lg + 2] = nw.z; tr[wave][l16][4 * lg + 3] = nw.w;
    GT_WAVE_SYNC();
    const float4 tv = make_float4(tr[wave][4 * lg][l16], tr[wave][4 * lg + 1][l16], tr[wave][4 * lg + 2][l16], tr[wave][4 * lg + 3][l16]);
    *reinterpret_cast<float4*>(pb + (int64_t)(bc * (R >> 4) + br) * 256 + lane * 4) = tv;
    return;
  }
  const int64_t i = ((int64_t)(blockIdx.x - u.nblk_a) * 256 + threadIdx.x) * 4;
  if (i >= u.n) return;
  const int64_t rel = i - a.p0.in_w;
  if (rel >= 0 && rel < (int64_t)a.L * a.pstride) {
    const int64_t r = rel % a.pstride;
    const int64_t o1 = a.p0.out_w - a.p0.in_w, o2 = a.p0.w1 - a.p0.in_w, o3 = a.p0.w2 - a.p0.in_w;
    if (r < (int64_t)3 * d * d || (r >= o1 && r < o1 + (int64_t)d * d) || (r >= o2 && r < o2 + (int64_t)d * F) || (r >= o3 && r < o3 + (int64_t)d * F)) return;
  }
#pragma unroll
  for (int e = 0; e < 4; ++e) {
    if (i + e < u.n - 1) {
      u.prm[i + e] = seq_upd_elem(u, i + e, u.prm[i + e], u.g[i + e], k, b1, b2, step_size, inv_sqrt_bc2, gs, eps, skip);
      u.g[i + e] = 0.f;
    }
  }
}
#endif
template <int NK, bool FULL = false, bool HALF = false>
__device__ __forceinline__ void seq_b_mma(f32x4& acc0, f32x4& acc1, const SeqB<NK>& b, const float* ap, const int lda, const int nk) {
  if (FULL && HALF) {
    float4 a0 = *reinterpret_cast<const float4*>(ap);
#pragma unroll
    for (int u = 0; u < NK; ++u) {
      float4 n0 = a0;
      if (u + 1 < NK) n0 = *reinterpret_cast<const float4*>(ap + 16 * (u + 1));
      acc0 = GT_MFMA16(b.v[u].x, a0.x, acc0); acc0 = GT_MFMA16(b.v[u].y, a0.y, acc0);
      acc0 = GT_MFMA16(b.v[u].z, a0.z, acc0); acc0 = GT_MFMA16(b.v[u].w, a0.w, acc0);
      GT_SCHED_FENCE()
      a0 = n0;
    }
    return;
  }
  if (HALF) {
#pragma unroll
    for (int u = 0; u < NK; ++u) {
      if (u < nk) {
        const float4 a0 = *reinterpret_cast<const float4*>(ap + 16 * u);
        acc0 = GT_MFMA16(b.v[u].x, a0.x, acc0); acc0 = GT_MFMA16(b.v[u].y, a0.y, acc0);
        acc0 = GT_MFMA16(b.v[u].z, a0.z, acc0); acc0 = GT_MFMA16(b.v[u].w, a0.w, acc0);
      }
    }
    return;
  }
  if (FULL) {
    float4 a0 = *reinterpret_cast<const float4*>(ap), a1 = *reinterpret_cast<const float4*>(ap + 16 * lda);
#pragma unroll
    for (int u = 0; u < NK; ++u) {
      float4 n0 = a0, n1 = a1;
      if (u + 1 < NK) { n0 = *reinterpret_cast<const float4*>(ap + 16 * (u + 1)); n1 = *reinterpret_cast<const float4*>(ap + 16 * lda + 16 * (u + 1)); }
      acc0 = GT_MFMA16(b.v[u].x, a0.x, acc0); acc1 = GT_MFMA16(b.v[u].x, a1.x, acc1);
      acc0 = GT_MFMA16(b.v[u].y, a0.y, acc0); acc1 = GT_MFMA16(b.v[u].y, a1.y, acc1);
      acc0 = GT_MFMA16(b.v[u].z, a0.z, acc0); acc1 = GT_MFMA16(b.v[u].z, a1.z, acc1);
      acc0 = GT_MFMA16(b.v[u].w, a0.w, acc0); acc1 = GT_MFMA16(b.v[u].w, a1.w, acc1);
      GT_SCHED_FENCE()
      a0 = n0; a1 = n1;
    }
    return;
  }
#pragma unroll
  for (int u = 0; u < NK; ++u) {
    if (FULL || u < nk) {
      const float4 a0 = *reinterpret_cast<const float4*>(ap + 16 * u), a1 = *reinterpret_cast<const float4*>(ap + 16 * lda + 16 * u);
      acc0 = GT_MFMA16(b.v[u].x, a0.x, acc0); acc1 = GT_MFMA16(b.v[u].x, a1.x, acc1);
      acc0 = GT_MFMA16(b.v[u].y, a0.y, acc0); acc1 = GT_MFMA16(b.v[u].y, a1.y, acc1);
      acc0 = GT_MFMA16(b.v[u].z, a0.z, acc0); acc1 = GT_MFMA16(b.v[u].z, a1.z, acc1);
      acc0 = GT_MFMA16(b.v[u].w, a0.w, acc0); acc1 = GT_MFMA16(b.v[u].w, a1.w, acc1);
    }
  }
}
template <int NK, int MAXT> struct SeqTilesAll { SeqB<NK> b[MAXT]; float4 bi[MAXT]; };
template <int NK, int MAXT, bool BIAS = true>
__device__ __forceinline__ void seq_tiles_all_load(SeqTilesAll<NK, MAXT>& f, const float* __restrict__ Wp, const int K, const int N,
                                                   const float* __restrict__ bias, const int wave, const int lane) {
  const int lg = lane >> 4, ntile = N >> 4, nk = K >> 4;
#pragma unroll
  for (int i = 0; i < MAXT; ++i) {
    const int t = wave + i * GT_SEQ_WAVES, tc = t < ntile ? t : (wave < ntile ? wave : 0);
    seq_b_load<NK, true>(f.b[i], Wp, nk, tc, 0, nk, lane);
    if constexpr (BIAS) f.bi[i] = *reinterpret_cast<const float4*>(bias + 16 * tc + 4 * lg);
    else f.bi[i] = make_float4(0.f, 0.f, 0.f, 0.f);
  }
}
template <int NK, int MAXT, bool HALF, typename Epi>
__device__ __forceinline__ void seq_mm_tiles_all(const float* sA, const int lda, const int K, const int N, const int wave, const int lane,
                                                 const SeqTilesAll<NK, MAXT>& f, Epi epi) {
  const int l16 = lane & 15, lg = lane >> 4, ntile = N >> 4, nk = K >> 4;
  if (wave >= ntile) return;
  const float* ap = sA + l16 * lda + 4 * lg;
#pragma unroll
  for (int i = 0; i < MAXT; ++i) {
    const int t = wave + i * GT_SEQ_WAVES;
    if (t < ntile) {
      f32x4 acc0 = f32x4{0.f, 0.f, 0.f, 0.f}, acc1 = f32x4{0.f, 0.f, 0.f, 0.f};
      seq_b_mma<NK, true, HALF>(acc0, acc1, f.b[i], ap, lda, nk);
      epi(16 * t, acc0, acc1, f.bi[i]);
    }
  }
}
template <int NK, int MAXT, bool FULL, bool HALF, typename Epi>
__device__ __forceinline__ void seq_mm_tiles_impl(const float* sA, const int lda, const int K, const float* __restrict__ Wp, const int N,
                                                  const float* __restrict__ bias, const int wave, const int lane, Epi& epi,
                                                  const bool have_pre = false, const SeqB<NK> pre = SeqB<NK>(), const float4* pre_bias = nullptr) {
  const int l16 = lane & 15, lg = lane >> 4, ntile = N >> 4, nk = K >> 4;
  if (wave >= ntile) return;
  const float* ap = sA + l16 * lda + 4 * lg;
  if constexpr (MAXT > 2 && NK * MAXT <= 8) {
    SeqB<NK> ball[MAXT];
    float4 biall[MAXT];
#pragma unroll
    for (int i = 0; i < MAXT; ++i) {
      const int t = wave + i * GT_SEQ_WAVES, tc = t < ntile ? t : wave;
      if (i == 0 && have_pre) ball[0] = pre;
      else seq_b_load<NK, FULL>(ball[i], Wp, nk, tc, 0, nk, lane);
      biall[i] = bias != nullptr ? *reinterpret_cast<const float4*>(bias + 16 * tc + 4 * lg) : make_float4(0.f, 0.f, 0.f, 0.f);
    }
#pragma unroll
    for (int i = 0; i < MAXT; ++i) {
      const int t = wave + i * GT_SEQ_WAVES;
      if (t < ntile) {
        f32x4 acc0 = f32x4{0.f, 0.f, 0.f, 0.f}, acc1 = f32x4{0.f, 0.f, 0.f, 0.f};
        seq_b_mma<NK, FULL, HALF>(acc0, acc1, ball[i], ap, lda, nk);
        epi(16 * t, acc0, acc1, biall[i]);
      }
    }
    return;
  }
  SeqB<NK> b[2];
  float4 bi[2];
  GT_SUBSTAMP(0);
  if (have_pre) b[0] = pre;
  else seq_b_load<NK, FULL>(b[0], Wp, nk, wave, 0, nk, lane);
  if (have_pre && pre_bias != nullptr) bi[0] = *pre_bias;
  else bi[0] = bias != nullptr ? *reinterpret_cast<const float4*>(bias + 16 * wave + 4 * lg) : make_float4(0.f, 0.f, 0.f, 0.f);
  GT_SUBSTAMP(1);
#pragma unroll
  for (int i = 0; i < MAXT; ++i) {
    const int t = wave + i * GT_SEQ_WAVES;
    if (t < ntile) {
      if (i + 1 < MAXT && t + GT_SEQ_WAVES < ntile) {
        seq_b_load<NK, FULL>(b[(i + 1) & 1], Wp, nk, t + GT_SEQ_WAVES, 0, nk, lane);
        bi[(i + 1) & 1] = bias != nullptr ? *reinterpret_cast<const float4*>(bias + 16 * (t + GT_SEQ_WAVES) + 4 * lg) : make_float4(0.f, 0.f, 0.f, 0.f);
      }
      f32x4 acc0 = f32x4{0.f, 0.f, 0.f, 0.f}, acc1 = f32x4{0.f, 0.f, 0.f, 0.f};
      GT_SUBSTAMP(2 + 3 * i);
      seq_b_mma<NK, FULL, HALF>(acc0, acc1, b[i & 1], ap, lda, nk);
#ifdef GT_SEQ_STAMPS
      asm volatile("" : "+v"(acc0), "+v"(acc1));
#endif
      GT_SUBSTAMP(3 + 3 * i);
      epi(16 * t, acc0, acc1, bi[i & 1]);
      GT_SUBSTAMP(4 + 3 * i);
    }
  }
}
template <int NK, int MAXT, bool FULL, bool HALF, typename Epi>
__device__ __forceinline__ void seq_mm_tiles(const float* sA, const int lda, const int K, const float* __restrict__ Wp, const int N,
                                             const float* __restrict__ bias, const int wave, const int lane, Epi epi,
                                             const bool have_pre = false, const SeqB<NK> pre = SeqB<NK>(), const float4* pre_bias = nullptr) {
  seq_mm_tiles_impl<NK, MAXT, FULL, HALF>(sA, lda, K, Wp, N, bias, wave, lane, epi, have_pre, pre, pre_bias);
}
template <int NK>
__device__ __forceinline__ SeqB<NK> seq_tiles_first(const float* __restrict__ Wp, const int K, const int N, const int wave, const int lane) {
  SeqB<NK> b;
  seq_b_load<NK, true>(b, Wp, K >> 4, wave < (N >> 4) ? wave : 0, 0, K >> 4, lane);
  return b;
}
__device__ __forceinline__ void seq_mma4(f32x4& acc, const float4& b, const float4& a) {
  acc = GT_MFMA16(b.x, a.x, acc); acc = GT_MFMA16(b.y, a.y, acc); acc = GT_MFMA16(b.z, a.z, acc); acc = GT_MFMA16(b.w, a.w, acc);
// ... 1493 lines not shown
```

transformergrooveinfilling_amd/csrc/gt_seq_api.h:

```cpp
#pragma once
#include "gt_common.h"

#define GT_SEQ_FMAX 512
#ifndef GT_XCHG_SPIN_MAX
#define GT_XCHG_SPIN_MAX (1 << 22)
#endif
struct SeqLayerP { int64_t in_w, in_b, out_w, out_b, w1, b1, w2, b2, n1w, n1b, n2w, n2b; };
struct SeqLayerW { int64_t qkv, P, ctx, xhat1, rstd1, x1, hact, xhat2, rstd2, xout; };
struct SeqTmp { int64_t dzA, dzAm, dzB, dzBm, dhid, dqkv; };
struct SeqArgs {
  const float* prm; float* ws; const float* pe; const float* xin; float* hvo;
  int B, S, d, F, H, L, hd;
  const gt_step_state* st; uint32_t thr; float dscale;
  SeqLayerP p0; int64_t pstride;
  SeqLayerW w0; int64_t wstride;
  SeqTmp t0; int64_t tstride;
  int64_t in_w, in_b, encn_w, encn_b, out_w, out_b;
  int64_t x0, a0, memory, enc_xhat, enc_rstd, dlogits, da0;
  int64_t ln_part, ln_part_stride;
  int64_t stamps;
  int64_t pack_f, pack_b, kstride;
  int64_t dctx;
  int64_t amask, amask_stride;
  int64_t xchg;
  int64_t xchg_b; int fuse_b0;
  int spin_max;
  int quad_pro;
  int phase;
  const float* loss_y; float loss_penalty; float* loss_stats; float* loss_part; unsigned* loss_ticket;
  float* grd;
  int nseq;
  int wg_accumulate;
  int ride_last_k;
  int out_early;
  int tail_phase;
  int tail_ksplit;
  int ln_nwg;
  gt_step_state* bump;
};
static inline int gt_seq_wg_tiles(int rows, int cols) { return ((rows + 31) / 32) * ((cols + 63) / 64); }
void gt_seq_launch_pack(const SeqArgs& a, unsigned nblocks, hipStream_t s);
void gt_seq_launch_update_pack(const SeqArgs& a, int algo, float* params, float* grads, float* m, float* v, int64_t n, const gt_step_state* st,
                               int step_advanced, hipStream_t s);
void gt_seq_launch_fwd(const SeqArgs& a, int d_model, int hc, bool split, unsigned nblocks, hipStream_t s, bool quad = false);
static inline int64_t gt_seq_xchg_floats(int batch) { return 16 + (int64_t)4 * batch * 4 * 512 * 2; }
void gt_seq_launch_fb(const SeqArgs& a, unsigned nblocks, hipStream_t s);
void gt_seq_launch_bwd(const SeqArgs& a, int d_model, int hc, bool split, unsigned nblocks, hipStream_t s, bool quad = false);
void gt_seq_launch_tail(const SeqArgs& a, unsigned nblocks, hipStream_t s);
void gt_seq_launch_fwd64(const SeqArgs& a, int hc, unsigned nblocks, hipStream_t s);
void gt_seq_launch_bwd64(const SeqArgs& a, int hc, unsigned nblocks, hipStream_t s);
```

transformergrooveinfilling_amd/csrc/gt_seq_wg.h:

```cpp
#pragma once
#include "gt_seq_api.h"

#define GT_WG_SLAB 8
#define GT_WG_TM 32
#define GT_WG_TN 64
#ifndef GT_WG_DEPTH
#define GT_WG_DEPTH 2
#endif
#define GT_WG_STAGE (2 * GT_WG_SLAB * (GT_WG_TM + GT_WG_TN))
#define GT_WG_LDS (8 * GT_WG_TM * GT_WG_TN)

struct SeqWgProb { const float* A; const float* B; float* C; float* dbias; int lda, ldb, ldc, rows, cols; };
enum { GT_WG_STORE = 0, GT_WG_ADD = 1, GT_WG_ATOMIC = 2 };

struct SeqWgRegs { float4 a, b0, b1; };
enum { GT_WGL_LINES = 0, GT_WGL_PACKED = 1, GT_WGL_SCALAR = 2 };
template <int MA, int MB>
__device__ __forceinline__ SeqWgRegs seq_wg_load(const SeqWgProb& p, const int i0, const int j0, const int t0, const int lane, const float* zp) {
  SeqWgRegs r;
  if (MA == GT_WGL_LINES) {
    r.a = *reinterpret_cast<const float4*>(p.A + (size_t)(t0 + (lane >> 3)) * p.lda + i0 + 4 * (lane & 7));
  } else if (MA == GT_WGL_PACKED) {
    r.a = *reinterpret_cast<const float4*>(lane < 2 * p.rows ? p.A + (size_t)t0 * p.lda + 4 * lane : zp);
  } else {
    const int ca = i0 + 4 * (lane & 7);
    const float* pa = p.A + (size_t)(t0 + (lane >> 3)) * p.lda + ca;
    float v[4];
#pragma unroll
    for (int e = 0; e < 4; ++e) v[e] = *((ca + e < p.rows) ? pa + e : zp);
    r.a = make_float4(v[0], v[1], v[2], v[3]);
  }
  if (MB == GT_WGL_LINES) {
    const float* pb = p.B + (size_t)(t0 + (lane >> 4)) * p.ldb + j0 + 4 * (lane & 15);
    r.b0 = *reinterpret_cast<const float4*>(pb);
    r.b1 = *reinterpret_cast<const float4*>(pb + (size_t)4 * p.ldb);
  } else if (MB == GT_WGL_PACKED) {
    const float* pb = p.B + (size_t)t0 * p.ldb + 4 * lane;
    r.b0 = *reinterpret_cast<const float4*>(lane < 2 * p.cols ? pb : zp);
    r.b1 = *reinterpret_cast<const float4*>(lane + 64 < 2 * p.cols ? pb + 256 : zp);
  } else {
    const int cb = j0 + 4 * (lane & 15);
    const float* pb = p.B + (size_t)(t0 + (lane >> 4)) * p.ldb + cb;
    float v[2][4];
#pragma unroll
    for (int e = 0; e < 4; ++e) { v[0][e] = *((cb + e < p.cols) ? pb + e : zp); v[1][e] = *((cb + e < p.cols) ? pb + (size_t)4 * p.ldb + e : zp); }
    r.b0 = make_float4(v[0][0], v[0][1], v[0][2], v[0][3]);
    r.b1 = make_float4(v[1][0], v[1][1], v[1][2], v[1][3]);
  }
  return r;
}
__device__ __forceinline__ void seq_wg_packed_slots(int (&o)[4], const int f, const int width, const int tilew) {
#pragma unroll
  for (int e = 0; e < 4; ++e) { const int x = 4 * f + e; o[e] = x < GT_WG_SLAB * width ? (x / width) * tilew + x % width : -1; }
}

__device__ __forceinline__ void seq_wg_scatter(float* buf, const int (&o)[4], const float4& v) {
  if (o[0] >= 0) buf[o[0]] = v.x;
  if (o[1] >= 0) buf[o[1]] = v.y;
  if (o[2] >= 0) buf[o[2]] = v.z;
  if (o[3] >= 0) buf[o[3]] = v.w;
}

template <int MA, int MB>
__device__ __forceinline__ void seq_wg_unit(const SeqWgProb& p, const int ti, const int tj, const int k0, const int k1, const int mode,
                                            float* lds, float* sb, const int tid) {
  const int lane = tid & 63, wave = tid >> 6, r = lane & 31, h = lane >> 5;
  const int i0 = GT_WG_TM * ti, j0 = GT_WG_TN * tj;
  const float* const zp = gt_zero_ptr();
  float* const st = lds + wave * GT_WG_STAGE;
  float* const stA = st, * const stB = st + 2 * GT_WG_SLAB * GT_WG_TM;
  const int nslab = (k1 - k0) / GT_WG_SLAB;
  const int nw = nslab > wave ? (nslab - wave + 7) >> 3 : 0;
  f32x16 acc0, acc1;
#pragma unroll
  for (int e = 0; e < 16; ++e) { acc0[e] = 0.f; acc1[e] = 0.f; }
  float bsum = 0.f;
  const bool want_bias = p.dbias != nullptr && tj == 0;
  GT_BARRIER();
  if (nw > 0) {
    auto slab_t0 = [&](int i) { const int ii = i < nw ? i : nw - 1; return k0 + (wave + 8 * ii) * GT_WG_SLAB; };
    SeqWgRegs q[GT_WG_DEPTH];
#pragma unroll
    for (int u = 0; u < GT_WG_DEPTH; ++u) q[u] = seq_wg_load<MA, MB>(p, i0, j0, slab_t0(u), lane, zp);
    const int wa = (lane >> 3) * GT_WG_TM + 4 * (lane & 7);
    const int wb = (lane >> 4) * GT_WG_TN + 4 * (lane & 15);
    int oa[4], ob0[4], ob1[4];
    if (MA == GT_WGL_PACKED) {
      seq_wg_packed_slots(oa, lane, p.rows, GT_WG_TM);
      for (int e = lane; e < 2 * GT_WG_SLAB * GT_WG_TM; e += 64) stA[e] = 0.f;
    }
    if (MB == GT_WGL_PACKED) {
      seq_wg_packed_slots(ob0, lane, p.cols, GT_WG_TN); seq_wg_packed_slots(ob1, lane + 64, p.cols, GT_WG_TN);
      for (int e = lane; e < 2 * GT_WG_SLAB * GT_WG_TN; e += 64) stB[e] = 0.f;
    }
    GT_WAVE_SYNC();
    auto slab = [&](const SeqWgRegs qq, const int i) -> SeqWgRegs {
      float* const bA = stA + (i & 1) * GT_WG_SLAB * GT_WG_TM;
      float* const bB = stB + (i & 1) * GT_WG_SLAB * GT_WG_TN;
      if (MA == GT_WGL_PACKED) {
        seq_wg_scatter(bA, oa, qq.a);
      } else {
        *reinterpret_cast<float4*>(bA + wa) = qq.a;
      }
      if (MB == GT_WGL_PACKED) {
        seq_wg_scatter(bB, ob0, qq.b0);
        seq_wg_scatter(bB, ob1, qq.b1);
      } else {
        *reinterpret_cast<float4*>(bB + wb) = qq.b0;
        *reinterpret_cast<float4*>(bB + wb + 4 * GT_WG_TN) = qq.b1;
      }
      GT_WAVE_SYNC();
      const SeqWgRegs nq = seq_wg_load<MA, MB>(p, i0, j0, slab_t0(i + GT_WG_DEPTH), lane, zp);
      const float live = i < nw ? 1.0f : 0.0f;
#pragma unroll
      for (int kk = 0; kk < GT_WG_SLAB / 2; ++kk) {
        const float av = bA[(2 * kk + h) * GT_WG_TM + r] * live;
        const float b0 = bB[(2 * kk + h) * GT_WG_TN + r], b1 = bB[(2 * kk + h) * GT_WG_TN + 32 + r];
        acc0 = GT_MFMA32(av, b0, acc0);
        acc1 = GT_MFMA32(av, b1, acc1);
        bsum += av;
      }
      GT_WAVE_SYNC();
      return nq;
    };
    for (int i = 0; i < nw; i += GT_WG_DEPTH) {
#pragma unroll
      for (int u = 0; u < GT_WG_DEPTH; ++u) q[u] = slab(q[u], i + u);
    }
  }
  GT_BARRIER();
  {
    float* const pt = lds + wave * (GT_WG_TM * GT_WG_TN);
#pragma unroll
    for (int e = 0; e < 16; ++e) {
      const int row = (e & 3) + 8 * (e >> 2) + 4 * h;
      pt[row * GT_WG_TN + r] = acc0[e];
      pt[row * GT_WG_TN + 32 + r] = acc1[e];
    }
    sb[wave * 64 + lane] = bsum;
  }
  GT_BARRIER();
  {
    const int row = tid >> 4, seg = tid & 15;
    float s[4];
#pragma unroll
    for (int e = 0; e < 4; ++e) {
      s[e] = lds[row * GT_WG_TN + seg + 16 * e];
#pragma unroll
      for (int w = 1; w < 8; ++w) s[e] += lds[w * (GT_WG_TM * GT_WG_TN) + row * GT_WG_TN + seg + 16 * e];
    }
    if (i0 + row < p.rows) {
      float* c = p.C + (size_t)(i0 + row) * p.ldc + j0 + seg;
#pragma unroll
      for (int e = 0; e < 4; ++e) {
        if (j0 + seg + 16 * e < p.cols) {
          if (mode == GT_WG_ATOMIC) atomicAdd(c + 16 * e, s[e]);
          else if (mode == GT_WG_ADD) c[16 * e] += s[e];
          else c[16 * e] = s[e];
        }
      }
    }
    if (want_bias && tid < GT_WG_TM && i0 + tid < p.rows) {
      float t = 0.f;
#pragma unroll
      for (int w = 0; w < 8; ++w) t += sb[w * 64 + tid] + sb[w * 64 + 32 + tid];
      if (mode == GT_WG_ATOMIC) atomicAdd(p.dbias + i0 + tid, t);
      else if (mode == GT_WG_ADD) p.dbias[i0 + tid] += t;
      else p.dbias[i0 + tid] = t;
    }
  }
}
__device__ __forceinline__ int seq_wg_tiles(const int rows, const int cols) { return ((rows + GT_WG_TM - 1) / GT_WG_TM) * ((cols + GT_WG_TN - 1) / GT_WG_TN); }
template <bool TAIL>
__device__ __forceinline__ void seq_wg_run(const SeqWgProb& p, const int tile, const int k0, const int k1, const int mode, float* lds, float* sb,
                                           const int tid) {
  const int ntj = (p.cols + GT_WG_TN - 1) / GT_WG_TN, ti = tile / ntj, tj = tile % ntj;
  const bool al_a = (reinterpret_cast<uintptr_t>(p.A) & 15) == 0, al_b = (reinterpret_cast<uintptr_t>(p.B) & 15) == 0;
  const bool lines_a = GT_WG_TM * (ti + 1) <= p.rows && (p.lda & 3) == 0 && al_a;
  const bool lines_b = GT_WG_TN * (tj + 1) <= p.cols && (p.ldb & 3) == 0 && al_b;
  const bool packed_a = p.rows <= GT_WG_TM && p.lda == p.rows && al_a;
  const bool packed_b = p.cols <= GT_WG_TN && p.ldb == p.cols && al_b;
  if (lines_a && lines_b) seq_wg_unit<GT_WGL_LINES, GT_WGL_LINES>(p, ti, tj, k0, k1, mode, lds, sb, tid);
  else if (TAIL && packed_a && lines_b) seq_wg_unit<GT_WGL_PACKED, GT_WGL_LINES>(p, ti, tj, k0, k1, mode, lds, sb, tid);
  else if (TAIL && lines_a && packed_b) seq_wg_unit<GT_WGL_LINES, GT_WGL_PACKED>(p, ti, tj, k0, k1, mode, lds, sb, tid);
  else seq_wg_unit<GT_WGL_SCALAR, GT_WGL_SCALAR>(p, ti, tj, k0, k1, mode, lds, sb, tid);
}

enum { GT_WGP_OUT = 0, GT_WGP_W2 = 1, GT_WGP_W1 = 2, GT_WGP_WO = 3, GT_WGP_WIN = 4, GT_WGP_IN = 5, GT_WGP_LN = 6 };
__device__ __forceinline__ SeqWgProb seq_wg_prob(const SeqArgs& a, const int kind, const int l) {
  const int d = a.d, F = a.F;
  const float* ws = a.ws;
  const float* wl = ws + (int64_t)l * a.wstride;
  const float* tl = ws + (int64_t)l * a.tstride;
  float* g = a.grd + (int64_t)l * a.pstride;
  const bool drop = a.st != nullptr && a.thr != 0u;
  SeqWgProb p;
  switch (kind) {
    case GT_WGP_OUT: p = SeqWgProb{ws + a.dlogits, ws + a.memory, a.grd + a.out_w, a.grd + a.out_b, GT_TGT, d, d, GT_TGT, d}; break;
    case GT_WGP_W2:  p = SeqWgProb{tl + (drop ? a.t0.dzAm : a.t0.dzA), wl + a.w0.hact, g + a.p0.w2, g + a.p0.b2, d, F, F, d, F}; break;
    case GT_WGP_W1:  p = SeqWgProb{tl + a.t0.dhid, wl + a.w0.x1, g + a.p0.w1, g + a.p0.b1, F, d, d, F, d}; break;
    case GT_WGP_WO:  p = SeqWgProb{tl + (drop ? a.t0.dzBm : a.t0.dzB), wl + a.w0.ctx, g + a.p0.out_w, g + a.p0.out_b, d, d, d, d, d}; break;
    case GT_WGP_WIN: p = SeqWgProb{tl + a.t0.dqkv, l == 0 ? ws + a.x0 : ws + (int64_t)(l - 1) * a.wstride + a.w0.xout, g + a.p0.in_w, g + a.p0.in_b,
                                   3 * d, d, d, 3 * d, d}; break;
    default:         p = SeqWgProb{ws + a.da0, a.xin, a.grd + a.in_w, a.grd + a.in_b, d, a.S, a.S, d, a.S}; break;
  }
  return p;
}
__device__ __forceinline__ void seq_wg_ln_job(const SeqArgs& a, const int j, const int cb, float* lds, const int tid) {
  const int d = a.d, nwg = a.ln_nwg, ncol = 2 * d;
  int64_t goff;
  if (j == 0) goff = a.encn_w;
  else { const int k = (j - 1) >> 1, l = a.L - 1 - k; goff = (int64_t)l * a.pstride + (((j - 1) & 1) ? a.p0.n1w : a.p0.n2w); }
  const float* part = a.ws + a.ln_part + (int64_t)j * a.ln_part_stride;
  float* dst = a.grd + goff;
  const int64_t bo = (d + 63) / 64 * 64;
  const float* const zp = gt_zero_ptr();
  const int c = cb * 64 + (tid & 63), grp = tid >> 6;
  const bool ok = c < ncol;
  float acc = 0.f;
  for (int g0 = grp; g0 < nwg; g0 += 64) {
    float v[8];
#pragma unroll
    for (int u = 0; u < 8; ++u) { const int g = g0 + 8 * u; v[u] = *((ok && g < nwg) ? part + (size_t)g * ncol + c : zp); }
#pragma unroll
    for (int u = 0; u < 8; ++u) acc += v[u];
  }
  GT_BARRIER();
  lds[tid] = acc;
  GT_BARRIER();
  if (grp == 0 && ok) {
    float t = lds[tid];
#pragma unroll
    for (int q = 1; q < 8; ++q) t += lds[tid + 64 * q];
    float* o = c < d ? dst + c : dst + bo + (c - d);
    if (a.wg_accumulate) *o += t; else *o = t;
  }
}
template <typename F>
__device__ __forceinline__ void seq_wg_phase_list(const SeqArgs& a, const int phase, F f) {
  const int L = a.L;
  if (phase == 0) { f(GT_WGP_OUT, 0); return; }
  if (phase >= 2) { if (f(GT_WGP_WIN, L - phase + 1)) return; }
  if (phase <= L) {
    const int l = L - phase;
    if (f(GT_WGP_W2, l)) return;
    if (f(GT_WGP_W1, l)) return;
    if (f(GT_WGP_WO, l)) return;
    if (phase == 1) { if (f(GT_WGP_LN, 0)) return; }
    if (f(GT_WGP_LN, 2 * phase - 1)) return;
    f(GT_WGP_LN, 2 * phase);
  } else {
    if (!a.out_early) { if (f(GT_WGP_OUT, 0)) return; }
    f(GT_WGP_IN, 0);
  }
}
__device__ __forceinline__ int seq_wg_kind_tiles(const SeqArgs& a, const int kind) {
  const int d = a.d, F = a.F;
  switch (kind) {
    case GT_WGP_OUT: return seq_wg_tiles(GT_TGT, d);
    case GT_WGP_W2:  return seq_wg_tiles(d, F);
    case GT_WGP_W1:  return seq_wg_tiles(F, d);
    case GT_WGP_WO:  return seq_wg_tiles(d, d);
    case GT_WGP_WIN: return seq_wg_tiles(3 * d, d);
    case GT_WGP_LN:  return (2 * d + 63) / 64;
    default:         return seq_wg_tiles(d, a.S);
  }
}
__device__ __forceinline__ int seq_wg_phase_units(const SeqArgs& a, const int phase, const int ksplit, const bool with_ln) {
  int n = 0;
  seq_wg_phase_list(a, phase, [&](int kind, int) {
    if (kind == GT_WGP_LN) { if (with_ln) n += seq_wg_kind_tiles(a, kind); }
    else n += seq_wg_kind_tiles(a, kind) * ksplit;
    return false;
  });
  return n;
}
template <bool TAIL>
__device__ __forceinline__ bool seq_wg_phase_unit(const SeqArgs& a, const int phase, int u, const int klo, const int khi, const int ksplit,
                                                  const int mode, const bool with_ln, float* lds, float* sb, const int tid) {
  bool done = false;
  seq_wg_phase_list(a, phase, [&](int kind, int layer) {
    if (kind == GT_WGP_LN) {
      if (!with_ln) return false;
      const int ncb = seq_wg_kind_tiles(a, kind);
      if (u >= ncb) { u -= ncb; return false; }
      seq_wg_ln_job(a, layer, u, lds, tid);
      done = true;
      return true;
    }
    const int nt = seq_wg_kind_tiles(a, kind) * ksplit;
    if (u >= nt) { u -= nt; return false; }
    const SeqWgProb p = seq_wg_prob(a, kind, layer);
    const int tile = u / ksplit, c = u % ksplit;
    const int per = (((khi - klo) / GT_WG_SLAB + ksplit - 1) / ksplit) * GT_WG_SLAB;
    const int k0 = klo + c * per < khi ? klo + c * per : khi, k1 = k0 + per < khi ? k0 + per : khi;
    seq_wg_run<TAIL>(p, tile, k0, k1, mode, lds, sb, tid);
    done = true;
    return true;
  });
  return done;
}
__device__ __forceinline__ void seq_wg_riders(const SeqArgs& a, const int phase, const int r, const int R, float* lds, float* sb, const int tid) {
  const int mode = a.wg_accumulate ? GT_WG_ADD : GT_WG_STORE;
  const int khi = phase == a.L ? a.ride_last_k : a.B * 32;
  for (int u = r; seq_wg_phase_unit<false>(a, phase, u, 0, khi, 1, mode, true, lds, sb, tid); u += R) { }
}

#ifdef GT_SEQ_TU_BWD
__global__ __launch_bounds__(GT_SEQ_NT_WG) void seq_tail_kernel(SeqArgs a) {
  __shared__ __attribute__((aligned(16))) float lds[GT_WG_LDS];
  __shared__ float sb[8 * 64];
  const int tid = threadIdx.x;
  if (a.bump != nullptr && blockIdx.x == 0 && tid == 0) gt_bump_counters(a.bump, a.xchg >= 0 ? reinterpret_cast<unsigned*>(a.ws + a.xchg) : nullptr, nullptr);
  const int M = a.B * 32, ks = a.tail_ksplit;
  int blk = blockIdx.x;
  if (a.tail_phase <= a.L) {
    seq_wg_phase_unit<true>(a, a.tail_phase, blk, 0, M, ks, ks > 1 ? GT_WG_ATOMIC : GT_WG_ADD, false, lds, sb, tid);
    return;
  }
  const int nrest = a.ride_last_k < M ? seq_wg_phase_units(a, a.L, 1, false) : 0;
  if (blk < nrest) { seq_wg_phase_unit<true>(a, a.L, blk, a.ride_last_k, M, 1, GT_WG_ADD, false, lds, sb, tid); return; }
  blk -= nrest;
  seq_wg_phase_unit<true>(a, a.L + 1, blk, 0, M, ks, ks > 1 ? GT_WG_ATOMIC : (a.wg_accumulate ? GT_WG_ADD : GT_WG_STORE), true, lds, sb, tid);
}
#endif
```

Baseline: 322,900 sequences/s.

## Fold optimizer update into backward tail kernel, dropping the separate update launch

```diff
diff --git a/transformergrooveinfilling_amd/csrc/groove_hip.hip b/transformergrooveinfilling_amd/csrc/groove_hip.hip
--- a/transformergrooveinfilling_amd/csrc/groove_hip.hip
+++ b/transformergrooveinfilling_amd/csrc/groove_hip.hip
@@ -173,6 +173,7 @@
   int64_t seq_xchg = -1, seq_xchg_n = 0;
   int64_t rowx = -1, rowx_n = 0;
   int64_t seq_amask = -1, seq_amask_stride = 0;
+  int64_t seq_fold = -1, seq_fold_n = 0, seq_fold_tiles = 0;
   std::vector<std::pair<int64_t, int64_t>> sh;
   std::vector<int64_t> sh_only;
   int64_t w16 = -1, w16t = -1, w16_stride = 0;
@@ -275,6 +276,8 @@
     W.seq_dctx = add(2 * M * d);
     if (d == 128) { W.seq_xchg_n = 2 * gt_seq_xchg_floats(c.batch); W.seq_xchg = add(W.seq_xchg_n); }
     if ((d == 32 || d == 64) && c.n_heads == 16) { W.seq_amask_stride = BH * 32; W.seq_amask = add(W.seq_amask_stride * c.n_enc_layers); }
+    W.seq_fold_tiles = gt_seq_wg_tiles(3 * d, d) + gt_seq_wg_tiles(d, c.src_dim) + gt_seq_wg_tiles(GT_TGT, d);
+    W.seq_fold_n = gt_seq_fold_floats((int)W.seq_fold_tiles); W.seq_fold = add(W.seq_fold_n);
   }
   if (!seq_supported(c) && (d == 256 || d == 512) && M % 64 == 0) { W.rowx_n = gt_rowx_floats(M, (int)d); W.rowx = add(W.rowx_n); }
   if (bf16_shadows(c)) {
@@ -318,6 +321,8 @@
   const WLayout W = ws_layout(*cfg);
   if (W.seq_xchg >= 0) (void)hipMemsetAsync(ws + W.seq_xchg, 0, (size_t)W.seq_xchg_n * sizeof(float), (hipStream_t)stream);
   if (W.rowx >= 0) (void)hipMemsetAsync(ws + W.rowx, 0, (size_t)W.rowx_n * sizeof(float), (hipStream_t)stream);
+  if (W.seq_fold >= 0)
+    (void)hipMemsetAsync(ws + W.seq_fold, 0, (size_t)gt_seq_fold_tick_floats((int)W.seq_fold_tiles) * sizeof(float), (hipStream_t)stream);
   return launch_status("gt_workspace_init");
 }
 extern "C" int gt_operand_shadow_level(const gt_config* cfg) {
@@ -1050,7 +1055,7 @@
   if (check_cfg(cfg)) return -1;
   if (!use_seq(*cfg)) return 0;
   if (!seq_split(*cfg)) return 7;
-  return 2 * cfg->n_enc_layers + 1 + (seq_ride(*cfg) ? 3 : 5) - (seq_fuse_b0(*cfg) ? 1 : 0);
+  return 2 * cfg->n_enc_layers + 1 + (seq_ride(*cfg) ? 2 : 5) - (seq_fuse_b0(*cfg) ? 1 : 0);
 }
 static SeqArgs mk_seq(const Ctx& x, const float* pe, const float* src, float* hvo) {
   SeqArgs a;
@@ -1076,6 +1081,8 @@
   a.dctx = x.W.seq_dctx; a.xchg = x.W.seq_xchg; a.xchg_b = x.W.seq_xchg >= 0 ? x.W.seq_xchg + gt_seq_xchg_floats(x.c.batch) : -1; a.fuse_b0 = 0; a.spin_max = g_xchg_spin_max > 0 ? g_xchg_spin_max : GT_XCHG_SPIN_MAX; a.amask = x.W.seq_amask; a.amask_stride = x.W.seq_amask_stride; a.phase = 0;
   a.loss_y = nullptr; a.loss_penalty = 0.f; a.loss_stats = nullptr; a.loss_part = nullptr; a.loss_ticket = nullptr;
   a.grd = nullptr; a.nseq = 0; a.wg_accumulate = 0; a.ride_last_k = x.M; a.out_early = 0; a.tail_phase = 0; a.tail_ksplit = 1; a.ln_nwg = 0; a.bump = nullptr;
+  a.fold = 0; a.upd_algo = 0; a.upd_prm = nullptr; a.upd_m = nullptr; a.upd_v = nullptr; a.upd_n = 0;
+  a.fold_tick = x.W.seq_fold; a.fold_plane = x.W.seq_fold >= 0 ? x.W.seq_fold + gt_seq_fold_tick_floats((int)x.W.seq_fold_tiles) : -1;
   return a;
 }
 static int seq_forward(const Ctx& x, const float* pe, const float* src, float* hvo_out) {
@@ -1347,9 +1354,11 @@
   return g.nb;
 }
 
+struct SeqFoldReq { int algo; float* params; float* m; float* v; bool done; };
 static int backward_impl(const gt_config* cfg, const float* params, float* grads, const float* xin, const float* tgt_in,
                          const float* hvo, const float* d_hvo, float* ws, const gt_step_state* state, int train, int accumulate,
-                         gt_stream_t stream, int phase = 0, gt_step_state* bump_state = nullptr, bool grads_zero = false) {
+                         gt_stream_t stream, int phase = 0, gt_step_state* bump_state = nullptr, bool grads_zero = false,
+                         SeqFoldReq* fold = nullptr) {
   Ctx x;
   if (make_ctx(x, cfg, params, grads, ws, state, train, stream)) return -1;
   if (!grads || !xin) return gt_fail("gt_backward: grads / x must not be NULL");
@@ -1435,15 +1444,25 @@
           return launch_status("gt_backward");
         }
         a.out_early = phase == 2 ? 1 : 0;
-        static const int tail_ks = [] { const char* e = getenv("GT_SEQ_TAIL_KS"); const int v = e ? atoi(e) : 2; return v < 1 ? 1 : v > 16 ? 16 : v; }();
+        static const int tail_ks = [] { const char* e = getenv("GT_SEQ_TAIL_KS"); const int v = e ? atoi(e) : 0; return v < 0 ? 0 : v > 16 ? 16 : v; }();
         const int tiles = win + gt_seq_wg_tiles(d, cfg->src_dim) + (a.out_early ? 0 : gt_seq_wg_tiles(GT_TGT, d));
-        int ks = (gt_deterministic() && tail_ks > 2) ? 2 : tail_ks;
+        const bool fold_here = fold != nullptr && bump_state != nullptr && phase == 0 && x.W.seq_fold >= 0 && !a.out_early;
+        int ks = tail_ks > 0 ? tail_ks : 2;
+        if (!fold_here && gt_deterministic() && ks > 2) ks = 2;
+        if (fold_here && ks > GT_SEQ_FOLD_KS_MAX) ks = GT_SEQ_FOLD_KS_MAX;
         if (ks > M / 8) ks = M / 8;
         a.phase = L + 1; a.tail_phase = L + 1; a.tail_ksplit = ks; a.bump = bump_state;
         const int nrest = a.ride_last_k < M ? per_layer + (L > 1 ? win : 0) : 0;
+        unsigned nupd = 0;
+        if (fold_here) {
+          a.fold = 1; a.upd_algo = fold->algo; a.upd_prm = fold->params; a.upd_m = fold->m; a.upd_v = fold->v; a.upd_n = P.total;
+          const int64_t frags = (int64_t)L * x.W.pack_stride / 256;
+          nupd = (unsigned)((frags + 7) / 8 + (P.total + 2047) / 2048);
+          fold->done = true;
+        }
         gt_prof_tag("seq_tail", 2.0 * M * (3.0 * d * d + (a.out_early ? 0.0 : 27.0 * d) + (double)d * cfg->src_dim) + 2.0 * (M - a.ride_last_k) * nrest * 2048.0,
-                    4.0 * M * (4.0 * d + cfg->src_dim));
-        gt_seq_launch_tail(a, (unsigned)(nrest + tiles * ks), x.s);
+                    4.0 * M * (4.0 * d + cfg->src_dim) + (fold_here ? (fold->algo ? 28.0 : 12.0) * P.total + 8.0 * L * x.W.pack_stride : 0.0));
+        gt_seq_launch_tail(a, (unsigned)(nrest + tiles * ks) + nupd, x.s);
         return launch_status("gt_backward");
       }
       gt_prof_tag("seq_bwd", fl, 4.0 * M * (L * (14.0 * d + 2.0 * x.F) + 27.0));
@@ -1679,10 +1698,13 @@
     gt_launch(loss_kernel<true, true>, dim3((M * GT_VOICES + 255) / 256), dim3(256), s, (const float*)hvo_out, y, hit_loss_penalty, stats,
               ws + W.dlogits, M, ws + W.loss_part, reinterpret_cast<unsigned*>(&state->pad2[0]));
   }
+  if (!skip_update && algo == 1 && (!m || !v)) return gt_fail("gt_optimizer_step: adam needs m and v");
+  SeqFoldReq fold{algo, params, m, v, false};
   const int brc = backward_impl(cfg, params, grads, xin, tgt_in, hvo_out, nullptr, ws, state, 1, 1, stream, skip_update == 2 ? 1 : 0,
-                                skip_update == 0 ? state : nullptr, true);
+                                skip_update == 0 ? state : nullptr, true, (!skip_update && (algo == 0 || algo == 1)) ? &fold : nullptr);
   g_seq_b0_fused = false;
   if (brc) return -1;
+  if (fold.done) return 0;
   if (!skip_update) {
     PLayout P = param_layout(*cfg);
     if (use_seq(*cfg)) {
diff --git a/transformergrooveinfilling_amd/csrc/gt_common.h b/transformergrooveinfilling_amd/csrc/gt_common.h
--- a/transformergrooveinfilling_amd/csrc/gt_common.h
+++ b/transformergrooveinfilling_amd/csrc/gt_common.h
@@ -122,6 +122,11 @@
   return __hip_atomic_load(p, __ATOMIC_RELAXED, __HIP_MEMORY_SCOPE_AGENT);
 #endif
 }
+__device__ __forceinline__ void gt_pub_drain() {
+#ifndef GT_EMU
+  asm volatile("s_waitcnt vmcnt(0)" ::: "memory");
+#endif
+}
 __device__ __forceinline__ unsigned gt_pub_ticket(unsigned* counter) {
 #ifdef GT_EMU
   return atomicAdd(counter, 1u);
diff --git a/transformergrooveinfilling_amd/csrc/gt_seq.h b/transformergrooveinfilling_amd/csrc/gt_seq.h
--- a/transformergrooveinfilling_amd/csrc/gt_seq.h
+++ b/transformergrooveinfilling_amd/csrc/gt_seq.h
@@ -193,76 +193,17 @@
   *reinterpret_cast<float4*>(a.ws + (pack ? a.pack_b : a.pack_f) + (int64_t)l * a.kstride + moff + (int64_t)f * 256 + lane * 4) = v;
 }
 
-struct SeqUpd { float* prm; float* g; float* m; float* v; int64_t n; const gt_step_state* st; int algo, step_advanced, nblk_a; const unsigned* err; };
-__device__ __forceinline__ float seq_upd_elem(const SeqUpd& u, const int64_t i, const float w, const float g, const float k, const float b1,
-                                              const float b2, const float step_size, const float inv_sqrt_bc2, const float gs, const float eps,
-                                              const bool skip) {
-  if (skip) return w;
-  if (u.algo == 0) return w - k * g;
-  const float gi = g * gs;
-  const float mi = b1 * u.m[i] + (1.0f - b1) * gi;
-  const float vi = b2 * u.v[i] + (1.0f - b2) * gi * gi;
-  u.m[i] = mi; u.v[i] = vi;
-  return w - step_size * mi / (sqrtf(vi) * inv_sqrt_bc2 + eps);
-}
 __global__ __launch_bounds__(256) void seq_update_pack_kernel(SeqArgs a, SeqUpd u) {
   __shared__ float tr[4][16][17];
-  const int lane = threadIdx.x & 63, wave = threadIdx.x >> 6, l16 = lane & 15, lg = lane >> 4;
-  const float k = u.st->lr * u.st->grad_scale;
-  float b1 = 0.f, b2 = 0.f, step_size = 0.f, inv_sqrt_bc2 = 0.f, gs = u.st->grad_scale, eps = 0.f;
-  if (u.algo == 1) {
-    b1 = u.st->beta1; b2 = u.st->beta2; eps = u.st->eps;
-    const float t = (float)(u.st->opt_step + (u.step_advanced ? 0u : 1u));
-    const float bc1 = 1.0f - powf(b1, t), bc2 = 1.0f - powf(b2, t);
-    step_size = u.st->lr / bc1; inv_sqrt_bc2 = 1.0f / sqrtf(bc2);
-  }
-  const bool skip = (u.err != nullptr && *u.err != 0u) || u.g[u.n - 1] != 0.f;
-  const int d = a.d, F = a.F, d16 = d >> 4, f16 = F >> 4;
-  const int nf0 = 3 * d16 * d16, nf1 = d16 * d16, nf2 = f16 * d16, T = nf0 + nf1 + 2 * nf2;
+  const int wave = threadIdx.x >> 6;
+  const SeqUpdK c = seq_upd_coef(u, u.step_advanced);
   if ((int)blockIdx.x < u.nblk_a) {
     const int gidx = blockIdx.x * 4 + wave;
-    if (gidx >= a.L * T) return;
-    const int l = gidx / T;
-    int f = gidx % T, R, C;
-    int64_t src, moff;
-    if (f < nf0) { src = a.p0.in_w; R = 3 * d; C = d; moff = 0; }
-    else if (f < nf0 + nf1) { f -= nf0; src = a.p0.out_w; R = d; C = d; moff = (int64_t)3 * d * d; }
-    else if (f < nf0 + nf1 + nf2) { f -= nf0 + nf1; src = a.p0.w1; R = F; C = d; moff = (int64_t)4 * d * d; }
-    else { f -= nf0 + nf1 + nf2; src = a.p0.w2; R = d; C = F; moff = (int64_t)4 * d * d + (int64_t)d * F; }
-    const int nkt = C >> 4, br = f / nkt, bc = f % nkt;
-    const int64_t e0 = src + (int64_t)l * a.pstride + (int64_t)(16 * br + l16) * C + 16 * bc + 4 * lg;
-    const float4 w = *reinterpret_cast<const float4*>(u.prm + e0), g = *reinterpret_cast<const float4*>(u.g + e0);
-    float4 nw;
-    nw.x = seq_upd_elem(u, e0, w.x, g.x, k, b1, b2, step_size, inv_sqrt_bc2, gs, eps, skip);
-    nw.y = seq_upd_elem(u, e0 + 1, w.y, g.y, k, b1, b2, step_size, inv_sqrt_bc2, gs, eps, skip);
-    nw.z = seq_upd_elem(u, e0 + 2, w.z, g.z, k, b1, b2, step_size, inv_sqrt_bc2, gs, eps, skip);
-    nw.w = seq_upd_elem(u, e0 + 3, w.w, g.w, k, b1, b2, step_size, inv_sqrt_bc2, gs, eps, skip);
-    *reinterpret_cast<float4*>(u.prm + e0) = nw;
-    *reinterpret_cast<float4*>(u.g + e0) = make_float4(0.f, 0.f, 0.f, 0.f);
-    float* pf = a.ws + a.pack_f + (int64_t)l * a.kstride + moff;
-    float* pb = a.ws + a.pack_b + (int64_t)l * a.kstride + moff;
-    *reinterpret_cast<float4*>(pf + (int64_t)f * 256 + lane * 4) = nw;
-    tr[wave][l16][4 * lg] = nw.x; tr[wave][l16][4 * lg + 1] = nw.y; tr[wave][l16][4 * lg + 2] = nw.z; tr[wave][l16][4 * lg + 3] = nw.w;
-    GT_WAVE_SYNC();
-    const float4 tv = make_float4(tr[wave][4 * lg][l16], tr[wave][4 * lg + 1][l16], tr[wave][4 * lg + 2][l16], tr[wave][4 * lg + 3][l16]);
-    *reinterpret_cast<float4*>(pb + (int64_t)(bc * (R >> 4) + br) * 256 + lane * 4) = tv;
+    if (gidx >= a.L * seq_upd_frags_per_layer(a)) return;
+    seq_upd_frag(a, u, c, gidx, &tr[wave][0][0], threadIdx.x & 63);
     return;
   }
-  const int64_t i = ((int64_t)(blockIdx.x - u.nblk_a) * 256 + threadIdx.x) * 4;
-  if (i >= u.n) return;
-  const int64_t rel = i - a.p0.in_w;
-  if (rel >= 0 && rel < (int64_t)a.L * a.pstride) {
-    const int64_t r = rel % a.pstride;
-    const int64_t o1 = a.p0.out_w - a.p0.in_w, o2 = a.p0.w1 - a.p0.in_w, o3 = a.p0.w2 - a.p0.in_w;
-    if (r < (int64_t)3 * d * d || (r >= o1 && r < o1 + (int64_t)d * d) || (r >= o2 && r < o2 + (int64_t)d * F) || (r >= o3 && r < o3 + (int64_t)d * F)) return;
-  }
-#pragma unroll
-  for (int e = 0; e < 4; ++e) {
-    if (i + e < u.n - 1) {
-      u.prm[i + e] = seq_upd_elem(u, i + e, u.prm[i + e], u.g[i + e], k, b1, b2, step_size, inv_sqrt_bc2, gs, eps, skip);
-      u.g[i + e] = 0.f;
-    }
-  }
+  seq_upd_flat(a, u, c, ((int64_t)(blockIdx.x - u.nblk_a) * 256 + threadIdx.x) * 4, [](int64_t) { return true; });
 }
 #endif
 template <int NK, bool FULL = false, bool HALF = false>
diff --git a/transformergrooveinfilling_amd/csrc/gt_seq_api.h b/transformergrooveinfilling_amd/csrc/gt_seq_api.h
--- a/transformergrooveinfilling_amd/csrc/gt_seq_api.h
+++ b/transformergrooveinfilling_amd/csrc/gt_seq_api.h
@@ -37,7 +37,13 @@
   int tail_ksplit;
   int ln_nwg;
   gt_step_state* bump;
+  int fold, upd_algo;
+  float* upd_prm; float* upd_m; float* upd_v; int64_t upd_n;
+  int64_t fold_tick, fold_plane;
 };
+#define GT_SEQ_FOLD_KS_MAX 4
+static inline int64_t gt_seq_fold_tick_floats(int tiles) { return (tiles + 1 + 63) / 64 * 64; }
+static inline int64_t gt_seq_fold_floats(int tiles) { return gt_seq_fold_tick_floats(tiles) + (int64_t)tiles * GT_SEQ_FOLD_KS_MAX * (32 * 64 + 64); }
 static inline int gt_seq_wg_tiles(int rows, int cols) { return ((rows + 31) / 32) * ((cols + 63) / 64); }
 void gt_seq_launch_pack(const SeqArgs& a, unsigned nblocks, hipStream_t s);
 void gt_seq_launch_update_pack(const SeqArgs& a, int algo, float* params, float* grads, float* m, float* v, int64_t n, const gt_step_state* st,
diff --git a/transformergrooveinfilling_amd/csrc/gt_seq_wg.h b/transformergrooveinfilling_amd/csrc/gt_seq_wg.h
--- a/transformergrooveinfilling_amd/csrc/gt_seq_wg.h
+++ b/transformergrooveinfilling_amd/csrc/gt_seq_wg.h
@@ -61,9 +61,100 @@
   if (o[3] >= 0) buf[o[3]] = v.w;
 }
 
-template <int MA, int MB>
+enum { GT_WGP_OUT = 0, GT_WGP_W2 = 1, GT_WGP_W1 = 2, GT_WGP_WO = 3, GT_WGP_WIN = 4, GT_WGP_IN = 5, GT_WGP_LN = 6 };
+
+struct SeqUpd { float* prm; float* g; float* m; float* v; int64_t n; const gt_step_state* st; int algo, step_advanced, nblk_a; const unsigned* err; };
+__device__ __forceinline__ float seq_upd_elem(const SeqUpd& u, const int64_t i, const float w, const float g, const float k, const float b1,
+                                              const float b2, const float step_size, const float inv_sqrt_bc2, const float gs, const float eps,
+                                              const bool skip) {
+  if (skip) return w;
+  if (u.algo == 0) return w - k * g;
+  const float gi = g * gs;
+  const float mi = b1 * u.m[i] + (1.0f - b1) * gi;
+  const float vi = b2 * u.v[i] + (1.0f - b2) * gi * gi;
+  u.m[i] = mi; u.v[i] = vi;
+  return w - step_size * mi / (sqrtf(vi) * inv_sqrt_bc2 + eps);
+}
+struct SeqUpdK { float k, b1, b2, step_size, inv_sqrt_bc2, gs, eps; bool skip; };
+__device__ __forceinline__ SeqUpdK seq_upd_coef(const SeqUpd& u, const int step_advanced) {
+  SeqUpdK c;
+  c.k = u.st->lr * u.st->grad_scale;
+  c.b1 = 0.f; c.b2 = 0.f; c.step_size = 0.f; c.inv_sqrt_bc2 = 0.f; c.gs = u.st->grad_scale; c.eps = 0.f;
+  if (u.algo == 1) {
+    c.b1 = u.st->beta1; c.b2 = u.st->beta2; c.eps = u.st->eps;
+    const float t = (float)(u.st->opt_step + (step_advanced ? 0u : 1u));
+    const float bc1 = 1.0f - powf(c.b1, t), bc2 = 1.0f - powf(c.b2, t);
+    c.step_size = u.st->lr / bc1; c.inv_sqrt_bc2 = 1.0f / sqrtf(bc2);
+  }
+  c.skip = (u.err != nullptr && *u.err != 0u) || u.g[u.n - 1] != 0.f;
+  return c;
+}
+__device__ __forceinline__ float seq_upd_one(const SeqUpd& u, const SeqUpdK& c, const int64_t i, const float w, const float g) {
+  return seq_upd_elem(u, i, w, g, c.k, c.b1, c.b2, c.step_size, c.inv_sqrt_bc2, c.gs, c.eps, c.skip);
+}
+__device__ __forceinline__ int seq_upd_frags_per_layer(const SeqArgs& a) {
+  const int d16 = a.d >> 4, f16 = a.F >> 4;
+  return 3 * d16 * d16 + d16 * d16 + 2 * f16 * d16;
+}
+__device__ __forceinline__ void seq_upd_frag_locate(const SeqArgs& a, const int gidx, int& l, int& f, int& R, int& C, int64_t& src, int64_t& moff,
+                                                    int& kind) {
+  const int d = a.d, F = a.F, d16 = d >> 4, f16 = F >> 4;
+  const int nf0 = 3 * d16 * d16, nf1 = d16 * d16, nf2 = f16 * d16, T = nf0 + nf1 + 2 * nf2;
+  l = gidx / T;
+  f = gidx % T;
+  if (f < nf0) { src = a.p0.in_w; R = 3 * d; C = d; moff = 0; kind = GT_WGP_WIN; }
+  else if (f < nf0 + nf1) { f -= nf0; src = a.p0.out_w; R = d; C = d; moff = (int64_t)3 * d * d; kind = GT_WGP_WO; }
+  else if (f < nf0 + nf1 + nf2) { f -= nf0 + nf1; src = a.p0.w1; R = F; C = d; moff = (int64_t)4 * d * d; kind = GT_WGP_W1; }
+  else { f -= nf0 + nf1 + nf2; src = a.p0.w2; R = d; C = F; moff = (int64_t)4 * d * d + (int64_t)d * F; kind = GT_WGP_W2; }
+}
+__device__ __forceinline__ void seq_upd_frag(const SeqArgs& a, const SeqUpd& u, const SeqUpdK& c, const int gidx, float* tr, const int lane) {
+  const int l16 = lane & 15, lg = lane >> 4;
+  int l, f, R, C, kind;
+  int64_t src, moff;
+  seq_upd_frag_locate(a, gidx, l, f, R, C, src, moff, kind);
+  const int nkt = C >> 4, br = f / nkt, bc = f % nkt;
+  const int64_t e0 = src + (int64_t)l * a.pstride + (int64_t)(16 * br + l16) * C + 16 * bc + 4 * lg;
+  const float4 w = *reinterpret_cast<const float4*>(u.prm + e0), g = *reinterpret_cast<const float4*>(u.g + e0);
+  float4 nw;
+  nw.x = seq_upd_one(u, c, e0, w.x, g.x);
+  nw.y = seq_upd_one(u, c, e0 + 1, w.y, g.y);
+  nw.z = seq_upd_one(u, c, e0 + 2, w.z, g.z);
+  nw.w = seq_upd_one(u, c, e0 + 3, w.w, g.w);
+  *reinterpret_cast<float4*>(u.prm + e0) = nw;
+  *reinterpret_cast<float4*>(u.g + e0) = make_float4(0.f, 0.f, 0.f, 0.f);
+  float* pf = a.ws + a.pack_f + (int64_t)l * a.kstride + moff;
+  float* pb = a.ws + a.pack_b + (int64_t)l * a.kstride + moff;
+  *reinterpret_cast<float4*>(pf + (int64_t)f * 256 + lane * 4) = nw;
+  tr[l16 * 17 + 4 * lg] = nw.x; tr[l16 * 17 + 4 * lg + 1] = nw.y; tr[l16 * 17 + 4 * lg + 2] = nw.z; tr[l16 * 17 + 4 * lg + 3] = nw.w;
+  GT_WAVE_SYNC();
+  const float4 tv = make_float4(tr[(4 * lg) * 17 + l16], tr[(4 * lg + 1) * 17 + l16], tr[(4 * lg + 2) * 17 + l16], tr[(4 * lg + 3) * 17 + l16]);
+  *reinterpret_cast<float4*>(pb + (int64_t)(bc * (R >> 4) + br) * 256 + lane * 4) = tv;
+}
+template <typename Own>
+__device__ __forceinline__ void seq_upd_flat(const SeqArgs& a, const SeqUpd& u, const SeqUpdK& c, const int64_t i, Own own) {
+  if (i >= u.n) return;
+  const int d = a.d, F = a.F;
+  const int64_t rel = i - a.p0.in_w;
+  if (rel >= 0 && rel < (int64_t)a.L * a.pstride) {
+    const int64_t r = rel % a.pstride;
+    const int64_t o1 = a.p0.out_w - a.p0.in_w, o2 = a.p0.w1 - a.p0.in_w, o3 = a.p0.w2 - a.p0.in_w;
+    if (r < (int64_t)3 * d * d || (r >= o1 && r < o1 + (int64_t)d * d) || (r >= o2 && r < o2 + (int64_t)d * F) || (r >= o3 && r < o3 + (int64_t)d * F)) return;
+  }
+#pragma unroll
+  for (int e = 0; e < 4; ++e) {
+    if (i + e < u.n - 1 && own(i + e)) {
+      u.prm[i + e] = seq_upd_one(u, c, i + e, u.prm[i + e], u.g[i + e]);
+      u.g[i + e] = 0.f;
+    }
+  }
+}
+
+struct SeqWgFold { const SeqArgs* a; int kind, layer, slot, chunk, nchunk; };
+__device__ __forceinline__ void seq_wg_fold(const SeqWgProb& p, const SeqWgFold& fo, const int i0, const int j0, const float (&s)[4], const float tb,
+                                            const bool want_bias, const int mode, float* lds, float* sb, const int tid);
+template <int MA, int MB, bool FOLD = false>
 __device__ __forceinline__ void seq_wg_unit(const SeqWgProb& p, const int ti, const int tj, const int k0, const int k1, const int mode,
-                                            float* lds, float* sb, const int tid) {
+                                            float* lds, float* sb, const int tid, const SeqWgFold& fo = SeqWgFold{}) {
   const int lane = tid & 63, wave = tid >> 6, r = lane & 31, h = lane >> 5;
   const int i0 = GT_WG_TM * ti, j0 = GT_WG_TN * tj;
   const float* const zp = gt_zero_ptr();
@@ -149,6 +240,15 @@
 #pragma unroll
       for (int w = 1; w < 8; ++w) s[e] += lds[w * (GT_WG_TM * GT_WG_TN) + row * GT_WG_TN + seg + 16 * e];
     }
+    if (FOLD && fo.a->fold) {
+      float tb = 0.f;
+      if (want_bias && tid < GT_WG_TM) {
+#pragma unroll
+        for (int w = 0; w < 8; ++w) tb += sb[w * 64 + tid] + sb[w * 64 + 32 + tid];
+      }
+      seq_wg_fold(p, fo, i0, j0, s, tb, want_bias, mode, lds, sb, tid);
+      return;
+    }
     if (i0 + row < p.rows) {
       float* c = p.C + (size_t)(i0 + row) * p.ldc + j0 + seg;
 #pragma unroll
@@ -170,23 +270,102 @@
     }
   }
 }
+__device__ __forceinline__ void seq_wg_fold(const SeqWgProb& p, const SeqWgFold& fo, const int i0, const int j0, const float (&s)[4], const float tb,
+                                            const bool want_bias, const int mode, float* lds, float* sb, const int tid) {
+  const SeqArgs& a = *fo.a;
+  const int row = tid >> 4, seg = tid & 15, lane = tid & 63, wave = tid >> 6;
+  const bool rok = i0 + row < p.rows, bok = want_bias && tid < GT_WG_TM && i0 + tid < p.rows;
+  float fv[4] = {s[0], s[1], s[2], s[3]}, fb = tb;
+  if (mode == GT_WG_ATOMIC) {
+    unsigned* const tick = reinterpret_cast<unsigned*>(a.ws + a.fold_tick) + 1 + fo.slot;
+    float* const pl0 = a.ws + a.fold_plane + (int64_t)fo.slot * GT_SEQ_FOLD_KS_MAX * (GT_WG_TM * GT_WG_TN + 64);
+    float* const pl = pl0 + (int64_t)fo.chunk * (GT_WG_TM * GT_WG_TN + 64);
+#pragma unroll
+    for (int e = 0; e < 4; ++e) gt_pub_store(pl + row * GT_WG_TN + seg + 16 * e, s[e]);
+    if (tid < GT_WG_TM) gt_pub_store(pl + GT_WG_TM * GT_WG_TN + tid, tb);
+    gt_pub_drain();
+    GT_BARRIER();
+    if (tid == 0) {
+      const unsigned t = gt_pub_ticket(tick);
+      const bool last = t == (unsigned)fo.nchunk - 1u;
+      if (last) *tick = 0u;
+      sb[0] = last ? 1.0f : 0.0f;
+    }
+    GT_BARRIER();
+    if (sb[0] == 0.0f) return;
+#pragma unroll
+    for (int e = 0; e < 4; ++e) fv[e] = gt_pub_load(pl0 + row * GT_WG_TN + seg + 16 * e);
+    if (bok) fb = gt_pub_load(pl0 + GT_WG_TM * GT_WG_TN + tid);
+    for (int c = 1; c < fo.nchunk; ++c) {
+      const float* q = pl0 + (int64_t)c * (GT_WG_TM * GT_WG_TN + 64);
+#pragma unroll
+      for (int e = 0; e < 4; ++e) fv[e] += gt_pub_load(q + row * GT_WG_TN + seg + 16 * e);
+      if (bok) fb += gt_pub_load(q + GT_WG_TM * GT_WG_TN + tid);
+    }
+  } else if (mode == GT_WG_ADD) {
+    if (rok) {
+      const float* c = p.C + (size_t)(i0 + row) * p.ldc + j0 + seg;
+#pragma unroll
+      for (int e = 0; e < 4; ++e) { if (j0 + seg + 16 * e < p.cols) fv[e] = c[16 * e] + s[e]; }
+    }
+    if (bok) fb = p.dbias[i0 + tid] + tb;
+  }
+  const SeqUpd u{a.upd_prm, a.grd, a.upd_m, a.upd_v, a.upd_n, a.bump, a.upd_algo, 0, 0,
+                 a.xchg >= 0 ? reinterpret_cast<const unsigned*>(a.ws + a.xchg) : nullptr};
+  const SeqUpdK k = seq_upd_coef(u, 0);
+  const bool pack = fo.kind == GT_WGP_W2 || fo.kind == GT_WGP_W1 || fo.kind == GT_WGP_WO || fo.kind == GT_WGP_WIN;
+  GT_BARRIER();
+  if (rok) {
+    const int64_t o = (p.C - a.grd) + (int64_t)(i0 + row) * p.ldc + j0 + seg;
+#pragma unroll
+    for (int e = 0; e < 4; ++e) {
+      if (j0 + seg + 16 * e < p.cols) {
+        const float nw = seq_upd_one(u, k, o + 16 * e, u.prm[o + 16 * e], fv[e]);
+        u.prm[o + 16 * e] = nw;
+        u.g[o + 16 * e] = 0.f;
+        lds[row * (GT_WG_TN + 1) + seg + 16 * e] = nw;
+      }
+    }
+  }
+  if (bok) {
+    const int64_t o = (p.dbias - a.grd) + i0 + tid;
+    u.prm[o] = seq_upd_one(u, k, o, u.prm[o], fb);
+    u.g[o] = 0.f;
+  }
+  if (!pack) return;
+  GT_BARRIER();
+  const int r0 = 16 * (wave >> 2), c0 = 16 * (wave & 3), l16 = lane & 15, lg = lane >> 4;
+  if (i0 + r0 >= p.rows || j0 + c0 >= p.cols) return;
+  const int d = a.d, F = a.F;
+  const int64_t moff = fo.kind == GT_WGP_WIN ? 0 : fo.kind == GT_WGP_WO ? (int64_t)3 * d * d : fo.kind == GT_WGP_W1 ? (int64_t)4 * d * d
+                                                 : (int64_t)4 * d * d + (int64_t)d * F;
+  const int br = (i0 + r0) >> 4, bc = (j0 + c0) >> 4, nkt = p.cols >> 4;
+  float* pf = a.ws + a.pack_f + (int64_t)fo.layer * a.kstride + moff;
+  float* pb = a.ws + a.pack_b + (int64_t)fo.layer * a.kstride + moff;
+  const float* t = lds + r0 * (GT_WG_TN + 1) + c0;
+  const float4 nw = make_float4(t[l16 * (GT_WG_TN + 1) + 4 * lg], t[l16 * (GT_WG_TN + 1) + 4 * lg + 1], t[l16 * (GT_WG_TN + 1) + 4 * lg + 2],
+                                t[l16 * (GT_WG_TN + 1) + 4 * lg + 3]);
+  const float4 tv = make_float4(t[(4 * lg) * (GT_WG_TN + 1) + l16], t[(4 * lg + 1) * (GT_WG_TN + 1) + l16], t[(4 * lg + 2) * (GT_WG_TN + 1) + l16],
+                                t[(4 * lg + 3) * (GT_WG_TN + 1) + l16]);
+  *reinterpret_cast<float4*>(pf + (int64_t)(br * nkt + bc) * 256 + lane * 4) = nw;
+  *reinterpret_cast<float4*>(pb + (int64_t)(bc * (p.rows >> 4) + br) * 256 + lane * 4) = tv;
+}
 __device__ __forceinline__ int seq_wg_tiles(const int rows, const int cols) { return ((rows + GT_WG_TM - 1) / GT_WG_TM) * ((cols + GT_WG_TN - 1) / GT_WG_TN); }
 template <bool TAIL>
 __device__ __forceinline__ void seq_wg_run(const SeqWgProb& p, const int tile, const int k0, const int k1, const int mode, float* lds, float* sb,
-                                           const int tid) {
+                                           const int tid, const SeqWgFold& fo = SeqWgFold{}) {
   const int ntj = (p.cols + GT_WG_TN - 1) / GT_WG_TN, ti = tile / ntj, tj = tile % ntj;
   const bool al_a = (reinterpret_cast<uintptr_t>(p.A) & 15) == 0, al_b = (reinterpret_cast<uintptr_t>(p.B) & 15) == 0;
   const bool lines_a = GT_WG_TM * (ti + 1) <= p.rows && (p.lda & 3) == 0 && al_a;
   const bool lines_b = GT_WG_TN * (tj + 1) <= p.cols && (p.ldb & 3) == 0 && al_b;
   const bool packed_a = p.rows <= GT_WG_TM && p.lda == p.rows && al_a;
   const bool packed_b = p.cols <= GT_WG_TN && p.ldb == p.cols && al_b;
-  if (lines_a && lines_b) seq_wg_unit<GT_WGL_LINES, GT_WGL_LINES>(p, ti, tj, k0, k1, mode, lds, sb, tid);
-  else if (TAIL && packed_a && lines_b) seq_wg_unit<GT_WGL_PACKED, GT_WGL_LINES>(p, ti, tj, k0, k1, mode, lds, sb, tid);
-  else if (TAIL && lines_a && packed_b) seq_wg_unit<GT_WGL_LINES, GT_WGL_PACKED>(p, ti, tj, k0, k1, mode, lds, sb, tid);
-  else seq_wg_unit<GT_WGL_SCALAR, GT_WGL_SCALAR>(p, ti, tj, k0, k1, mode, lds, sb, tid);
-}
-
-enum { GT_WGP_OUT = 0, GT_WGP_W2 = 1, GT_WGP_W1 = 2, GT_WGP_WO = 3, GT_WGP_WIN = 4, GT_WGP_IN = 5, GT_WGP_LN = 6 };
+  if (lines_a && lines_b) seq_wg_unit<GT_WGL_LINES, GT_WGL_LINES, TAIL>(p, ti, tj, k0, k1, mode, lds, sb, tid, fo);
+  else if (TAIL && packed_a && lines_b) seq_wg_unit<GT_WGL_PACKED, GT_WGL_LINES, TAIL>(p, ti, tj, k0, k1, mode, lds, sb, tid, fo);
+  else if (TAIL && lines_a && packed_b) seq_wg_unit<GT_WGL_LINES, GT_WGL_PACKED, TAIL>(p, ti, tj, k0, k1, mode, lds, sb, tid, fo);
+  else seq_wg_unit<GT_WGL_SCALAR, GT_WGL_SCALAR, TAIL>(p, ti, tj, k0, k1, mode, lds, sb, tid, fo);
+}
+
 __device__ __forceinline__ SeqWgProb seq_wg_prob(const SeqArgs& a, const int kind, const int l) {
   const int d = a.d, F = a.F;
   const float* ws = a.ws;
@@ -279,6 +458,7 @@
 __device__ __forceinline__ bool seq_wg_phase_unit(const SeqArgs& a, const int phase, int u, const int klo, const int khi, const int ksplit,
                                                   const int mode, const bool with_ln, float* lds, float* sb, const int tid) {
   bool done = false;
+  int slot = 0;
   seq_wg_phase_list(a, phase, [&](int kind, int layer) {
     if (kind == GT_WGP_LN) {
       if (!with_ln) return false;
@@ -289,12 +469,12 @@
       return true;
     }
     const int nt = seq_wg_kind_tiles(a, kind) * ksplit;
-    if (u >= nt) { u -= nt; return false; }
+    if (u >= nt) { u -= nt; slot += nt / ksplit; return false; }
     const SeqWgProb p = seq_wg_prob(a, kind, layer);
     const int tile = u / ksplit, c = u % ksplit;
     const int per = (((khi - klo) / GT_WG_SLAB + ksplit - 1) / ksplit) * GT_WG_SLAB;
     const int k0 = klo + c * per < khi ? klo + c * per : khi, k1 = k0 + per < khi ? k0 + per : khi;
-    seq_wg_run<TAIL>(p, tile, k0, k1, mode, lds, sb, tid);
+    seq_wg_run<TAIL>(p, tile, k0, k1, mode, lds, sb, tid, SeqWgFold{&a, kind, layer, slot + tile, c, ksplit});
     done = true;
     return true;
   });
@@ -307,11 +487,18 @@
 }
 
 #ifdef GT_SEQ_TU_BWD
+__device__ __forceinline__ bool seq_wg_tail_final(const SeqArgs& a, const int kind, const int layer) {
+  bool hit = false;
+  auto f = [&](int k, int l) { if (k != GT_WGP_LN && k == kind && l == layer) hit = true; return hit; };
+  if (a.ride_last_k < a.B * 32) seq_wg_phase_list(a, a.L, f);
+  if (!hit) seq_wg_phase_list(a, a.L + 1, f);
+  return hit;
+}
 __global__ __launch_bounds__(GT_SEQ_NT_WG) void seq_tail_kernel(SeqArgs a) {
   __shared__ __attribute__((aligned(16))) float lds[GT_WG_LDS];
   __shared__ float sb[8 * 64];
   const int tid = threadIdx.x;
-  if (a.bump != nullptr && blockIdx.x == 0 && tid == 0) gt_bump_counters(a.bump, a.xchg >= 0 ? reinterpret_cast<unsigned*>(a.ws + a.xchg) : nullptr, nullptr);
+  if (a.bump != nullptr && !a.fold && blockIdx.x == 0 && tid == 0) gt_bump_counters(a.bump, a.xchg >= 0 ? reinterpret_cast<unsigned*>(a.ws + a.xchg) : nullptr, nullptr);
   const int M = a.B * 32, ks = a.tail_ksplit;
   int blk = blockIdx.x;
   if (a.tail_phase <= a.L) {
@@ -319,8 +506,49 @@
     return;
   }
   const int nrest = a.ride_last_k < M ? seq_wg_phase_units(a, a.L, 1, false) : 0;
-  if (blk < nrest) { seq_wg_phase_unit<true>(a, a.L, blk, a.ride_last_k, M, 1, GT_WG_ADD, false, lds, sb, tid); return; }
-  blk -= nrest;
-  seq_wg_phase_unit<true>(a, a.L + 1, blk, 0, M, ks, ks > 1 ? GT_WG_ATOMIC : (a.wg_accumulate ? GT_WG_ADD : GT_WG_STORE), true, lds, sb, tid);
+  const int nown = seq_wg_phase_units(a, a.L + 1, ks, true);
+  if (blk < nrest) {
+    seq_wg_phase_unit<true>(a, a.L, blk, a.ride_last_k, M, 1, GT_WG_ADD, false, lds, sb, tid);
+  } else if (blk < nrest + nown) {
+    seq_wg_phase_unit<true>(a, a.L + 1, blk - nrest, 0, M, ks, ks > 1 ? GT_WG_ATOMIC : (a.wg_accumulate ? GT_WG_ADD : GT_WG_STORE), true, lds, sb, tid);
+  } else if (a.fold) {
+    const SeqUpd u{a.upd_prm, a.grd, a.upd_m, a.upd_v, a.upd_n, a.bump, a.upd_algo, 0, 0,
+                   a.xchg >= 0 ? reinterpret_cast<const unsigned*>(a.ws + a.xchg) : nullptr};
+    const SeqUpdK c = seq_upd_coef(u, 0);
+    const int ub = blk - nrest - nown, nfrag = a.L * seq_upd_frags_per_layer(a), nblk_a = (nfrag + 7) / 8;
+    if (ub < nblk_a) {
+      const int gidx = ub * 8 + (tid >> 6);
+      if (gidx < nfrag) {
+        int l, f, R, C, kind;
+        int64_t src, moff;
+        seq_upd_frag_locate(a, gidx, l, f, R, C, src, moff, kind);
+        if (!seq_wg_tail_final(a, kind, l)) seq_upd_frag(a, u, c, gidx, lds + (tid >> 6) * (16 * 17), tid & 63);
+      }
+    } else {
+      seq_upd_flat(a, u, c, ((int64_t)(ub - nblk_a) * GT_SEQ_NT_WG + tid) * 4, [&](int64_t i) {
+        bool mine = true;
+        auto f = [&](int kind, int layer) {
+          if (kind == GT_WGP_LN) return false;
+          const SeqWgProb p = seq_wg_prob(a, kind, layer);
+          const int64_t c0 = p.C - a.grd, b0 = p.dbias - a.grd;
+          if ((i >= c0 && i < c0 + (int64_t)p.rows * p.ldc) || (i >= b0 && i < b0 + p.rows)) mine = false;
+          return !mine;
+        };
+        if (a.ride_last_k < M) seq_wg_phase_list(a, a.L, f);
+        if (mine) seq_wg_phase_list(a, a.L + 1, f);
+        return mine;
+      });
+    }
+  }
+  if (a.fold) {
+    GT_BARRIER();
+    if (tid == 0) {
+      unsigned* const tick = reinterpret_cast<unsigned*>(a.ws + a.fold_tick);
+      if (gt_pub_ticket(tick) == gridDim.x - 1u) {
+        *tick = 0u;
+        gt_bump_counters(a.bump, a.xchg >= 0 ? reinterpret_cast<unsigned*>(a.ws + a.xchg) : nullptr, nullptr);
+      }
+    }
+  }
 }
 #endif
```

New measurement: 325,100 sequences/s, median of 6. No clear change (+0.7%).
